# AnonymWriter/Iris-Style-Transfer

Hardware: NVIDIA B200
Metric: masked-NST image-steps/sec @640x400 VGG-19 (higher is better)
Workload: dtype bf16

## Files before the change

### include/isx.h

```cpp
#ifndef ISX_H_
#define ISX_H_

#include <stdint.h>

#ifdef __cplusplus
extern "C" {
#endif

#define ISX_VERSION 100

typedef uint16_t isx_bf16;
typedef void* isx_stream;

const char* isx_last_error(void);
int isx_version(void);
int isx_device_check(int device);

int isx_ipc_export(const void* ptr, void* handle64, int64_t* offset);
int isx_ipc_open(const void* handle64, void** base_out);
int isx_ipc_close(void* base);
int isx_copy_d2d_async(void* dst, const void* src, int64_t bytes, isx_stream stream);

typedef void* isx_handle;
int isx_create(int device, isx_handle* out);
int isx_destroy(isx_handle h);
int isx_make_current(isx_handle h);
int isx_sm_count(void);

int isx_pack_conv3x3_weights(const float* w_oihw, int Cout, int Cin, isx_bf16* w_fwd, isx_bf16* w_dgrad,
                             isx_stream stream);

int isx_conv1_1_fwd(const float* x, int xc, const float* mask, int mask_b, const float* w, const float* bias,
                    isx_bf16* out, int B, int H, int W, isx_stream stream);
int isx_pack_conv1_1_fwd(const float* w, isx_bf16* w0_fwd, isx_stream stream);
int isx_conv1_1_fwd_tc(const float* x, int xc, const float* mask, int mask_b, const isx_bf16* w0_fwd, const float* bias,
                       isx_bf16* out, int B, int H, int W, isx_stream stream);
int isx_conv1_1_dgrad(const isx_bf16* dy, const float* w, const float* mask, int mask_b, float* dx, int xc, int B,
                      int H, int W, isx_stream stream);

int isx_pack_conv1_1_dgrad(const float* w, isx_bf16* w0_dgrad, isx_stream stream);
int isx_conv1_1_dgrad_tc(const isx_bf16* dy, const isx_bf16* w0_dgrad, const float* mask, int mask_b, float* dx, int xc,
                         int B, int H, int W, isx_stream stream);

int isx_conv3x3_bias_relu_fwd(const isx_bf16* in, const isx_bf16* w_fwd, const float* bias, isx_bf16* out, int B,
                              int H, int W, int Cin, int Cout, int relu, int tile_cfg, isx_stream stream);

int isx_conv3x3_bias_relu_pool_fwd(const isx_bf16* in, const isx_bf16* w_fwd, const float* bias, isx_bf16* out,
                                   isx_bf16* pool_out, int B, int H, int W, int Cin, int Cout, int tile_cfg,
                                   isx_stream stream);
int isx_conv3x3_bias_relu_pool_idx_fwd(const isx_bf16* in, const isx_bf16* w_fwd, const float* bias, isx_bf16* out,
                                       isx_bf16* pool_out, uint8_t* pool_idx, int skip_out, int B, int H, int W, int Cin,
                                       int Cout, int tile_cfg, isx_stream stream);

int isx_conv3x3_dgrad(const isx_bf16* dy, const isx_bf16* w_dgrad, isx_bf16* dx, int B, int H, int W, int Cin,
                      int Cout, const isx_bf16* relu_act, const isx_bf16* add_grad, const float* aff_a,
                      const float* aff_b, int tile_cfg, isx_stream stream);

int isx_conv3x3_dgrad_gram(const isx_bf16* dy, const isx_bf16* w_dgrad, isx_bf16* dx, int B, int H, int W, int Cin,
                           int Cout, const isx_bf16* act_below, const isx_bf16* gram_D, isx_stream stream);

int isx_maxpool2x2_fwd(const isx_bf16* in, isx_bf16* out, int B, int H, int W, int C, isx_stream stream);
int isx_maxpool2x2_bwd(const isx_bf16* dy_pooled, const isx_bf16* act_prepool, isx_bf16* dx, int B, int H, int W,
                       int C, isx_stream stream);
int isx_maxpool2x2_fwd_idx(const isx_bf16* in, isx_bf16* out, uint8_t* idx, int B, int H, int W, int C, isx_stream stream);
int isx_maxpool2x2_bwd_idx(const isx_bf16* dy_pooled, const uint8_t* idx, isx_bf16* dx, int B, int H, int W, int C,
                           isx_stream stream);

int64_t isx_gram_workspace_bytes(int B, int HW, int C);
int isx_gram_fwd(const isx_bf16* feat, int B, int HW, int C, float inv_n, void* workspace, float* G_out,
                 const float* target, int target_b, double loss_scale, double* loss, float grad_scale,
                 isx_bf16* D_out, isx_stream stream);
int64_t isx_gram_mask_flags_bytes(int mask_b, int HW, int C);
int isx_gram_masked_fwd(const isx_bf16* feat, int B, int HW, int C, const float* m, int mask_b, void* flags_ws,
                        isx_bf16* fm2, float inv_n, void* workspace, float* G_out, const float* target, int target_b,
                        double loss_scale, double* loss, float grad_scale, isx_bf16* D_out, isx_stream stream);
int isx_gram_bwd(const isx_bf16* feat, const isx_bf16* D, isx_bf16* dF, int B, int H, int W, int C,
                 const isx_bf16* relu_act, isx_stream stream);

int isx_content_mse_fwd_bwd(const isx_bf16* pred, const isx_bf16* target, int target_b, isx_bf16* grad, int B,
                            int64_t per_image, double loss_scale, float grad_scale, double* loss, isx_stream stream);
int isx_mse_fwd_bwd(const isx_bf16* pred, const isx_bf16* target, int target_b, isx_bf16* grad, int B, int64_t per_image,
                    double loss_scale, float grad_scale, int relu_mask, double* loss, isx_stream stream);
int isx_channel_affine(const isx_bf16* feat, const float* a, const float* b, isx_bf16* out, int B, int64_t HW, int C,
                       int relu_mask, isx_stream stream);
int isx_bn_stats_fwd(const isx_bf16* feat, int B, int64_t HW, int C, double* sums, float* mean, float* std_,
                     const float* t_mean, const float* t_std, int target_b, double loss_scale, double grad_scale,
                     double* loss, float* aff_a, float* aff_b, isx_stream stream);
int isx_bn_stats_masked_fwd(const isx_bf16* feat, const float* m, int mask_b, int B, int64_t HW, int C, double* sums, float* mean,
                            float* std_, isx_stream stream);
int isx_mask_features(const isx_bf16* feat, const float* m, int mask_b, isx_bf16* fm, isx_bf16* fm2, int B, int64_t HW,
                      int C, isx_stream stream);
int isx_avgpool2x2_f32(const float* in, float* out, int B, int H, int W, isx_stream stream);
int isx_tap_add_mask(const isx_bf16* g, const isx_bf16* add, const float* aff_a, const float* aff_b,
                     const isx_bf16* act, isx_bf16* out, int B, int64_t HW, int C, isx_stream stream);

typedef struct {
  int32_t epochs;
  int32_t max_iter;
  int32_t max_eval;
  int32_t history;
  int32_t history_bf16;
  int32_t reserved_;
  double lr;
  double tolerance_grad;
  double tolerance_change;
  double c_weight, s_weight;
} isx_lbfgs_config;
int64_t isx_lbfgs_state_bytes(int P);
int64_t isx_lbfgs_mats_bytes(int P, int history);
int64_t isx_lbfgs_scratch_bytes(int P, int64_t N, int history);
int isx_lbfgs_init(void* state, int P, isx_stream stream);
int isx_lbfgs_tick(float* x, const float* grad, float* grad_prev, void* S, void* Y, void* state, void* mats,
                   void* scratch, const double* loss_c, const double* loss_s, int images_per_problem, int P,
                   int64_t N, const isx_lbfgs_config* cfg, double* hist_c, double* hist_s, int tick,
                   isx_stream stream);
int isx_lbfgs_done_flags(const void* state, int P, int32_t* done_out, isx_stream stream);
int isx_lbfgs_history_counts(const void* state, int P, int32_t* count_out, isx_stream stream);
int isx_clamp01(float* x, int64_t n, isx_stream stream);

#define ISX_MAX_TAPS 8
#define ISX_VGG19_CONVS 16
#define ISX_TAP_POOL0 16
#define ISX_VGG19_TAPS 21
typedef struct {
  int32_t B, H, W, xc;
  int32_t n_conv;
  int32_t style_mode;
  int32_t n_style;
  int32_t style_conv[ISX_MAX_TAPS];
  float style_w[ISX_MAX_TAPS];
  int32_t n_content;
  int32_t content_conv[ISX_MAX_TAPS];
  float content_w[ISX_MAX_TAPS];
  int32_t style_target_b;
  int32_t content_target_b;
  int32_t coupled;
  int32_t mask_b;
  int32_t style_mask_b;
  int32_t pred_unbatched;
  double c_weight, s_weight;
} isx_nst_config;

typedef struct {
  const float* w0;
  const isx_bf16* w0_fwd;
  const isx_bf16* w0_dgrad;
  const float* bias[ISX_VGG19_CONVS];
  const isx_bf16* w_fwd[ISX_VGG19_CONVS];
  const isx_bf16* w_dgrad[ISX_VGG19_CONVS];
  void* workspace;
  const isx_bf16* content_target[ISX_MAX_TAPS];
  const float* gram_target[ISX_MAX_TAPS];
  const float* bn_target_mean[ISX_MAX_TAPS];
  const float* bn_target_std[ISX_MAX_TAPS];
  const float* input_mask;
  const float* style_mask[ISX_MAX_TAPS];
} isx_nst_buffers;

int64_t isx_nst_workspace_bytes(const isx_nst_config* cfg);
int isx_nst_backward(const isx_nst_config* cfg, const isx_nst_buffers* bufs, const isx_bf16* const* feat_grads,
                     const isx_bf16* last_pool_grad, float* grad, isx_stream stream);
#define ISX_FWD_LAST_POOL 1
#define ISX_FWD_LEAN 2
int isx_nst_forward(const isx_nst_config* cfg, const isx_nst_buffers* bufs, const float* x, int flags,
                    isx_stream stream);
int isx_nst_feature(const isx_nst_config* cfg, const isx_nst_buffers* bufs, int kind, int idx, isx_bf16** ptr,
                    int32_t* h, int32_t* w, int32_t* c);
int isx_nst_prepare_style_masks(const isx_nst_config* cfg, const isx_nst_buffers* bufs, isx_stream stream);
int isx_nst_style_features(const isx_nst_config* cfg, const isx_nst_buffers* bufs, int want_stats, int want_gram,
                           float* out, int64_t ld, isx_stream stream);
int isx_nst_eval(const isx_nst_config* cfg, const isx_nst_buffers* bufs, const float* x, double* loss_c,
                 double* loss_s, float* grad, isx_stream stream);

int isx_mask_bbox(const float* x, const int64_t* seg, int label, int use_threshold, float threshold, uint8_t* mask,
                  float* xm, int32_t* bbox, int B, int H, int W, isx_stream stream);
int isx_mask_bbox_typed(const float* x, const void* seg, int seg_dtype, int label, int use_threshold, float threshold,
                        uint8_t* mask, float* xm, int32_t* bbox, int B, int H, int W, isx_stream stream);
int isx_resize_bilinear_aa(const float* src, int src_c, int SH, int SW, const int32_t* src_bbox, float* dst, int dst_c,
                           int DH, int DW, int B, isx_stream stream);
int isx_crop_resize_masked(const float* frames, const uint8_t* mask, const int32_t* bbox, float* dst, int dst_c, int DH,
                           int DW, int B, int H, int W, isx_stream stream);
int isx_composite(const float* new_iris, int src_c, int SH, int SW, float* frames, const uint8_t* mask,
                  const int32_t* bbox, int B, int H, int W, isx_stream stream);

int64_t isx_ritnet_transform_workspace_bytes(int B, int H, int W);
int isx_ritnet_transform(const float* x, const uint8_t* gamma_lut, const float* norm_lut, void* workspace, float* out, int B,
                         int H, int W, isx_stream stream);
int64_t isx_ritnet_param_floats(void);
int64_t isx_ritnet_workspace_bytes(int B, int H, int W);
int isx_ritnet_forward(const float* x, const float* params, const uint8_t* gamma_lut, const float* norm_lut, void* workspace,
                       int64_t* labels, float* logits, int B, int H, int W, isx_stream stream);
int isx_ritnet_forward_typed(const float* x, const float* params, const uint8_t* gamma_lut, const float* norm_lut,
                             void* workspace, void* labels, int label_dtype, float* logits, int B, int H, int W,
                             isx_stream stream);

int isx_linear_pack(const float* W, const float* bias, int N, int K, int Npad, isx_bf16* dst, isx_stream stream);
int isx_rows_pack(const float* src, int64_t ld_src, int M, int K, int Mpad, isx_bf16* dst, isx_stream stream);
int isx_pool7_flatten_pack(const isx_bf16* pool5, int B, int h, int w, int C, int Mpad, isx_bf16* dst, isx_stream stream);
int isx_linear_fwd(const isx_bf16* Xp, const isx_bf16* Wp, isx_bf16* outT, int Mpad, int Npad, int Kp, int relu, isx_stream stream);
int isx_transpose_pack(const isx_bf16* srcT, int N, int Mpad, int M, isx_bf16* dst, isx_stream stream);
int isx_transpose_out(const isx_bf16* srcT, int N, int Mpad, int M, float* dst, isx_stream stream);

int64_t isx_eye_landmarks_workspace_bytes(int B, int H, int W, int max_points);
int isx_eye_landmarks(const void* seg, int seg_dtype, int B, int H, int W, double epsilon, int max_points, void* workspace,
                      float* landmarks, int32_t* info, isx_stream stream);
int isx_gaze_head_fwd(const float* x, int64_t ld_x, int B, int in_dim, int hidden, int out_dim, const float* W1, const float* b1,
                      const float* W2, const float* b2, const float* W3, const float* b3, float* out, isx_stream stream);

int isx_pack_conv1x1_weights(const float* w, int Cout, int Cin, isx_bf16* w_out, isx_stream stream);
int isx_pack_resnet_stem_weights(const float* w, isx_bf16* w_out, isx_stream stream);
int isx_conv_bias_act_fwd(const isx_bf16* in, const isx_bf16* w, const float* bias, const isx_bf16* residual, isx_bf16* out,
                          int B, int H, int W, int Cin, int Cout, int k, int stride, int relu, isx_stream stream);
// ... 30 lines not shown
```

### iris-style-transfer_b200/csrc/api_ops.cu

```cuda
#include "../../include/isx.h"
#include "isx_common.cuh"
#include "isx_internal.h"
#include "isx_kernels.h"

using namespace isx;
typedef __nv_bfloat16 bf16;

static inline cudaStream_t S(isx_stream s) { return reinterpret_cast<cudaStream_t>(s); }
static inline const bf16* P(const isx_bf16* p) { return reinterpret_cast<const bf16*>(p); }
static inline bf16* P(isx_bf16* p) { return reinterpret_cast<bf16*>(p); }

static void decode_tile_cfg(int cfg, ConvArgs* a) {
  if (cfg > 0) {
    a->force_bn = cfg / 100;
    a->force_mt = (cfg % 100) / 10;
    a->force_stages = cfg % 10;
  }
}

extern "C" int isx_pack_conv3x3_weights(const float* w, int Cout, int Cin, isx_bf16* wf, isx_bf16* wd,
                                        isx_stream stream) {
  ISX_REQUIRE(w && (wf || wd) && Cout > 0 && Cin > 0, "isx_pack_conv3x3_weights: bad arguments");
  return pack_conv_weights(w, Cout, Cin, P(wf), P(wd), S(stream));
}

extern "C" int isx_conv1_1_fwd(const float* x, int xc, const float* mask, int mask_b, const float* w,
                               const float* bias, isx_bf16* out, int B, int H, int W, isx_stream stream) {
  ISX_REQUIRE(x && w && out && B > 0 && H > 0 && W > 0, "isx_conv1_1_fwd: bad arguments");
  ISX_REQUIRE(!mask || mask_b == 1 || mask_b == B, "isx_conv1_1_fwd: mask batch %d must be 1 or %d", mask_b, B);
  return conv1_1_fwd(x, xc, mask, mask_b, w, bias, P(out), B, H, W, S(stream));
}

extern "C" int isx_pack_conv1_1_fwd(const float* w, isx_bf16* w0_fwd, isx_stream stream) {
  ISX_REQUIRE(w && w0_fwd, "isx_pack_conv1_1_fwd: null pointer");
  return pack_w0_fwd(w, P(w0_fwd), S(stream));
}

extern "C" int isx_conv1_1_fwd_tc(const float* x, int xc, const float* mask, int mask_b, const isx_bf16* w0_fwd,
                                  const float* bias, isx_bf16* out, int B, int H, int W, isx_stream stream) {
  ISX_REQUIRE(x && w0_fwd && out && B > 0 && H > 0 && W > 0, "isx_conv1_1_fwd_tc: bad arguments");
  ISX_REQUIRE(!mask || mask_b == 1 || mask_b == B, "isx_conv1_1_fwd_tc: mask batch %d must be 1 or %d", mask_b, B);
  return conv1_1_fwd_tc(x, xc, mask, mask ? mask_b : 0, P(w0_fwd), bias, P(out), B, H, W, S(stream));
}

extern "C" int isx_pack_conv1_1_dgrad(const float* w, isx_bf16* w0_dgrad, isx_stream stream) {
  ISX_REQUIRE(w && w0_dgrad, "isx_pack_conv1_1_dgrad: null pointer");
  return pack_w0_dgrad(w, P(w0_dgrad), S(stream));
}

extern "C" int isx_conv1_1_dgrad_tc(const isx_bf16* dy, const isx_bf16* w0_dgrad, const float* mask, int mask_b,
                                    float* dx, int xc, int B, int H, int W, isx_stream stream) {
  ISX_REQUIRE(dy && w0_dgrad && dx && B > 0 && H > 0 && W > 0, "isx_conv1_1_dgrad_tc: bad arguments");
  ISX_REQUIRE(!mask || mask_b == 1 || mask_b == B, "isx_conv1_1_dgrad_tc: mask batch %d must be 1 or %d", mask_b, B);
  ConvArgs a;
  a.in = P(dy); a.weight = P(w0_dgrad); a.out = nullptr;
  a.B = B; a.H = H; a.W = W; a.Cin = 64; a.Cout = 16; a.ntaps = 9;
  a.dx_nchw = dx; a.xc = xc; a.in_mask = mask; a.mask_b = mask ? mask_b : 0;
  return conv_tc(a, S(stream));
}

extern "C" int isx_conv1_1_dgrad(const isx_bf16* dy, const float* w, const float* mask, int mask_b, float* dx, int xc,
                                 int B, int H, int W, isx_stream stream) {
  ISX_REQUIRE(dy && w && dx && B > 0 && H > 0 && W > 0, "isx_conv1_1_dgrad: bad arguments");
  ISX_REQUIRE(xc == 1 || xc == 3, "isx_conv1_1_dgrad: xc must be 1 or 3");
  return conv1_1_dgrad(P(dy), w, mask, mask_b, dx, xc, B, H, W, S(stream));
}

extern "C" int isx_conv3x3_bias_relu_fwd(const isx_bf16* in, const isx_bf16* w_fwd, const float* bias, isx_bf16* out,
                                         int B, int H, int W, int Cin, int Cout, int relu, int tile_cfg,
                                         isx_stream stream) {
  ISX_REQUIRE(in && w_fwd && out, "isx_conv3x3_bias_relu_fwd: null pointer");
  ConvArgs a;
  a.in = P(in); a.weight = P(w_fwd); a.out = P(out);
  a.B = B; a.H = H; a.W = W; a.Cin = Cin; a.Cout = Cout; a.ntaps = 9;
  a.bias = bias; a.relu = relu;
  decode_tile_cfg(tile_cfg, &a);
  return conv_tc(a, S(stream));
}

extern "C" int isx_conv3x3_bias_relu_pool_fwd(const isx_bf16* in, const isx_bf16* w_fwd, const float* bias, isx_bf16* out,
                                              isx_bf16* pool_out, int B, int H, int W, int Cin, int Cout, int tile_cfg,
                                              isx_stream stream) {
  ISX_REQUIRE(in && w_fwd && out && pool_out && H >= 2 && W >= 2, "isx_conv3x3_bias_relu_pool_fwd: bad arguments");
  ConvArgs a;
  a.in = P(in); a.weight = P(w_fwd); a.out = P(out); a.pool_out = P(pool_out);
  a.B = B; a.H = H; a.W = W; a.Cin = Cin; a.Cout = Cout; a.ntaps = 9;
  a.bias = bias; a.relu = 1;
  decode_tile_cfg(tile_cfg, &a);
  return conv_tc(a, S(stream));
}

extern "C" int isx_conv3x3_bias_relu_pool_idx_fwd(const isx_bf16* in, const isx_bf16* w_fwd, const float* bias, isx_bf16* out,
                                                  isx_bf16* pool_out, uint8_t* pool_idx, int skip_out, int B, int H, int W,
                                                  int Cin, int Cout, int tile_cfg, isx_stream stream) {
  ISX_REQUIRE(in && w_fwd && out && pool_out && pool_idx && H >= 2 && W >= 2, "isx_conv3x3_bias_relu_pool_idx_fwd: bad arguments");
  ConvArgs a;
  a.in = P(in); a.weight = P(w_fwd); a.out = P(out); a.pool_out = P(pool_out); a.pool_idx = pool_idx; a.skip_out = skip_out != 0;
  a.B = B; a.H = H; a.W = W; a.Cin = Cin; a.Cout = Cout; a.ntaps = 9;
  a.bias = bias; a.relu = 1;
  decode_tile_cfg(tile_cfg, &a);
  return conv_tc(a, S(stream));
}

extern "C" int isx_conv3x3_dgrad(const isx_bf16* dy, const isx_bf16* w_dgrad, isx_bf16* dx, int B, int H, int W,
                                 int Cin, int Cout, const isx_bf16* relu_act, const isx_bf16* add_grad,
                                 const float* aff_a, const float* aff_b, int tile_cfg, isx_stream stream) {
  ISX_REQUIRE(dy && w_dgrad && dx, "isx_conv3x3_dgrad: null pointer");
  ConvArgs a;
  a.in = P(dy); a.weight = P(w_dgrad); a.out = P(dx);
  a.B = B; a.H = H; a.W = W; a.Cin = Cout; a.Cout = Cin; a.ntaps = 9;
  a.mask_act = P(relu_act); a.add_buf = P(add_grad); a.aff_a = aff_a; a.aff_b = aff_b;
  decode_tile_cfg(tile_cfg, &a);
  return conv_tc(a, S(stream));
}

extern "C" int isx_conv3x3_dgrad_gram(const isx_bf16* dy, const isx_bf16* w_dgrad, isx_bf16* dx, int B, int H, int W,
                                      int Cin, int Cout, const isx_bf16* act_below, const isx_bf16* gram_D,
                                      isx_stream stream) {
  ISX_REQUIRE(dy && w_dgrad && dx && act_below && gram_D, "isx_conv3x3_dgrad_gram: null pointer");
  ConvArgs a;
  a.in = P(dy); a.weight = P(w_dgrad); a.out = P(dx);
  a.B = B; a.H = H; a.W = W; a.Cin = Cout; a.Cout = Cin; a.ntaps = 9;
  a.mask_act = P(act_below); a.gram_act = P(act_below); a.gram_D = P(gram_D);
  return conv_tc(a, S(stream));
}

extern "C" int isx_maxpool2x2_fwd(const isx_bf16* in, isx_bf16* out, int B, int H, int W, int C, isx_stream stream) {
  ISX_REQUIRE(in && out, "isx_maxpool2x2_fwd: null pointer");
  return maxpool_fwd(P(in), P(out), B, H, W, C, S(stream));
}

extern "C" int isx_maxpool2x2_bwd(const isx_bf16* dy, const isx_bf16* act, isx_bf16* dx, int B, int H, int W, int C,
                                  isx_stream stream) {
  ISX_REQUIRE(dy && act && dx, "isx_maxpool2x2_bwd: null pointer");
  return maxpool_bwd(P(dy), P(act), P(dx), B, H, W, C, S(stream));
}

extern "C" int isx_maxpool2x2_fwd_idx(const isx_bf16* in, isx_bf16* out, uint8_t* idx, int B, int H, int W, int C,
                                      isx_stream stream) {
  ISX_REQUIRE(in && idx, "isx_maxpool2x2_fwd_idx: null pointer");
  return maxpool_fwd_idx(P(in), P(out), idx, B, H, W, C, S(stream));
}

extern "C" int isx_maxpool2x2_bwd_idx(const isx_bf16* dy, const uint8_t* idx, isx_bf16* dx, int B, int H, int W, int C,
                                      isx_stream stream) {
  ISX_REQUIRE(dy && idx && dx, "isx_maxpool2x2_bwd_idx: null pointer");
  return maxpool_bwd_idx(P(dy), idx, P(dx), B, H, W, C, S(stream));
}

extern "C" int64_t isx_gram_workspace_bytes(int B, int HW, int C) {
  if (B <= 0 || HW <= 0 || C <= 0) return 0;
  return static_cast<int64_t>(gram_pick_splits(B, HW, C)) * B * C * C * 4;
}

extern "C" int isx_gram_fwd(const isx_bf16* feat, int B, int HW, int C, float inv_n, void* workspace, float* G_out,
                            const float* target, int target_b, double loss_scale, double* loss, float grad_scale,
                            isx_bf16* D_out, isx_stream stream) {
  ISX_REQUIRE(feat && workspace, "isx_gram_fwd: null pointer");
  ISX_REQUIRE(!target || target_b == 1 || target_b == B, "isx_gram_fwd: target batch %d must be 1 or %d", target_b, B);
  const int splits = gram_pick_splits(B, HW, C);
  int rc = gram_tc_partial(P(feat), B, HW, C, splits, static_cast<float*>(workspace), S(stream));
  if (rc) return rc;
  return gram_finalize(static_cast<const float*>(workspace), B, splits, C, inv_n, G_out, target, target_b, loss_scale,
                       loss, grad_scale, P(D_out), S(stream));
}

extern "C" int64_t isx_gram_mask_flags_bytes(int mask_b, int HW, int C) {
  if (mask_b <= 0 || HW <= 0 || C <= 0) return 0;
  return gram_mask_flags_bytes(mask_b, HW, C);
}

extern "C" int isx_gram_masked_fwd(const isx_bf16* feat, int B, int HW, int C, const float* m, int mask_b, void* flags_ws,
                                   isx_bf16* fm2, float inv_n, void* workspace, float* G_out, const float* target,
                                   int target_b, double loss_scale, double* loss, float grad_scale, isx_bf16* D_out,
                                   isx_stream stream) {
  ISX_REQUIRE(feat && m && flags_ws && workspace, "isx_gram_masked_fwd: null pointer");
  ISX_REQUIRE(mask_b == 1 || mask_b == B, "isx_gram_masked_fwd: mask batch %d must be 1 or %d", mask_b, B);
  ISX_REQUIRE(!target || target_b == 1 || target_b == B, "isx_gram_masked_fwd: target batch %d must be 1 or %d", target_b, B);
  int rc = gram_mask_flags(m, mask_b, HW, C, static_cast<uint8_t*>(flags_ws), S(stream));
  if (rc) return rc;
  ISX_REQUIRE(fm2 != nullptr, "isx_gram_masked_fwd: fm2 (bf16 [B,HW,C]) is required: the kernel stores F*m^2 while it scales the tiles");
  ISX_CHECK_CUDA(cudaMemsetAsync(fm2, 0, static_cast<size_t>(B) * HW * C * 2, S(stream)));
  GramMask gm;
  gm.m = m; gm.mask_b = mask_b; gm.kb_flags = static_cast<const uint8_t*>(flags_ws); gm.fm2 = P(fm2);
  const int splits = gram_pick_splits(B, HW, C);
  rc = gram_sym_partial(P(feat), B, HW, C, splits, static_cast<float*>(workspace), &gm, S(stream));
  if (rc) return rc;
  return gram_finalize(static_cast<const float*>(workspace), B, splits, C, inv_n, G_out, target, target_b, loss_scale,
                       loss, grad_scale, P(D_out), S(stream));
}

extern "C" int isx_gram_bwd(const isx_bf16* feat, const isx_bf16* D, isx_bf16* dF, int B, int H, int W, int C,
                            const isx_bf16* relu_act, isx_stream stream) {
  ISX_REQUIRE(feat && D && dF, "isx_gram_bwd: null pointer");
  ConvArgs a;
  a.in = P(feat); a.weight = P(D); a.out = P(dF);
  a.B = B; a.H = H; a.W = W; a.Cin = C; a.Cout = C; a.ntaps = 1;
  a.per_image_weights = true;
  a.mask_act = P(relu_act);
  return conv_tc(a, S(stream));
}

extern "C" int isx_content_mse_fwd_bwd(const isx_bf16* pred, const isx_bf16* target, int target_b, isx_bf16* grad,
                                       int B, int64_t per_image, double loss_scale, float grad_scale, double* loss,
                                       isx_stream stream) {
  ISX_REQUIRE(pred && target && loss, "isx_content_mse_fwd_bwd: null pointer");
  ISX_REQUIRE(target_b == 1 || target_b == B, "isx_content_mse_fwd_bwd: target batch %d must be 1 or %d", target_b, B);
  return content_mse(P(pred), P(target), target_b, P(grad), B, per_image, loss_scale, grad_scale, loss, S(stream));
}

extern "C" int isx_mse_fwd_bwd(const isx_bf16* pred, const isx_bf16* target, int target_b, isx_bf16* grad, int B,
                               int64_t per_image, double loss_scale, float grad_scale, int relu_mask, double* loss,
                               isx_stream stream) {
  ISX_REQUIRE(pred && target && loss, "isx_mse_fwd_bwd: null pointer");
  ISX_REQUIRE(target_b == 1 || target_b == B, "isx_mse_fwd_bwd: target batch %d must be 1 or %d", target_b, B);
  return content_mse(P(pred), P(target), target_b, P(grad), B, per_image, loss_scale, grad_scale, loss, S(stream), relu_mask);
}

extern "C" int isx_channel_affine(const isx_bf16* feat, const float* a, const float* b, isx_bf16* out, int B, int64_t HW, int C,
                                  int relu_mask, isx_stream stream) {
  ISX_REQUIRE(feat && a && b && out && C % 8 == 0, "isx_channel_affine: bad arguments");
  return tap_add_mask(nullptr, nullptr, a, b, P(feat), P(out), B, HW, C, S(stream), relu_mask);
}

extern "C" int isx_bn_stats_fwd(const isx_bf16* feat, int B, int64_t HW, int C, double* sums, float* mean, float* std_,
                                const float* t_mean, const float* t_std, int target_b, double loss_scale,
                                double grad_scale, double* loss, float* aff_a, float* aff_b, isx_stream stream) {
  ISX_REQUIRE(feat && sums, "isx_bn_stats_fwd: null pointer");
  ISX_REQUIRE(HW >= 2, "isx_bn_stats_fwd: unbiased std needs at least 2 pixels");
  ISX_CHECK_CUDA(cudaMemsetAsync(sums, 0, static_cast<size_t>(B) * C * 2 * sizeof(double), S(stream)));
  int rc = chan_sums(P(feat), B, HW, C, sums, S(stream));
  if (rc) return rc;
  return bn_finalize(sums, B, C, HW, mean, std_, t_mean, t_std, target_b, loss_scale, grad_scale, loss, aff_a, aff_b,
                     S(stream));
}

extern "C" int isx_bn_stats_masked_fwd(const isx_bf16* feat, const float* m, int mask_b, int B, int64_t HW, int C, double* sums,
                                       float* mean, float* std_, isx_stream stream) {
  ISX_REQUIRE(feat && m && sums && mean && std_, "isx_bn_stats_masked_fwd: null pointer");
  ISX_REQUIRE(mask_b == 1 || mask_b == B, "isx_bn_stats_masked_fwd: mask batch %d must be 1 or %d", mask_b, B);
  ISX_REQUIRE(HW >= 2, "isx_bn_stats_masked_fwd: unbiased std needs at least 2 pixels");
  ISX_CHECK_CUDA(cudaMemsetAsync(sums, 0, static_cast<size_t>(B) * C * 2 * sizeof(double), S(stream)));
  int rc = chan_sums(P(feat), B, HW, C, sums, S(stream), m, mask_b);
  if (rc) return rc;
  return bn_finalize(sums, B, C, HW, mean, std_, nullptr, nullptr, 1, 0.0, 0.0, nullptr, nullptr, nullptr, S(stream));
}

extern "C" int isx_mask_features(const isx_bf16* feat, const float* m, int mask_b, isx_bf16* fm, isx_bf16* fm2, int B,
                                 int64_t HW, int C, isx_stream stream) {
  ISX_REQUIRE(feat && m && fm && C % 8 == 0, "isx_mask_features: bad arguments");
  ISX_REQUIRE(mask_b == 1 || mask_b == B, "isx_mask_features: mask batch %d must be 1 or %d", mask_b, B);
  return mask_features(P(feat), m, mask_b, P(fm), P(fm2), B, HW, C, S(stream));
}

extern "C" int isx_avgpool2x2_f32(const float* in, float* out, int B, int H, int W, isx_stream stream) {
  ISX_REQUIRE(in && out && H >= 2 && W >= 2, "isx_avgpool2x2_f32: bad arguments");
  return avgpool2x2_f32(in, out, B, H, W, S(stream));
}

extern "C" int isx_tap_add_mask(const isx_bf16* g, const isx_bf16* add, const float* aff_a, const float* aff_b,
                                const isx_bf16* act, isx_bf16* out, int B, int64_t HW, int C, isx_stream stream) {
  ISX_REQUIRE(act && out, "isx_tap_add_mask: null pointer");
  return tap_add_mask(P(g), P(add), aff_a, aff_b, P(act), P(out), B, HW, C, S(stream));
}

static int IsxContext::*option_field(const char* name) {
  static const struct {
    const char* name;
    int IsxContext::*field;
  } kOptions[] = {
      {"c64", &IsxContext::opt_c64},
      {"halo2", &IsxContext::opt_halo2},
      {"tail_n", &IsxContext::opt_tail_n},
      {"sweep64", &IsxContext::opt_sweep64},
      {"smem_reserve_kb", &IsxContext::opt_smem_reserve_kb},
  };
  for (const auto& o : kOptions)
    if (strcmp(name, o.name) == 0) return o.field;
  return nullptr;
}

extern "C" int isx_set_option(const char* name, int value) {
  ISX_REQUIRE(name != nullptr, "isx_set_option: null name");
  int IsxContext::*field = option_field(name);
  ISX_REQUIRE(field != nullptr, "isx_set_option: unknown option '%s'", name);
  isx_ctx()->*field = value;
  return 0;
}

extern "C" int isx_get_option(const char* name, int* value) {
  ISX_REQUIRE(name != nullptr && value != nullptr, "isx_get_option: null pointer");
  int IsxContext::*field = option_field(name);
  ISX_REQUIRE(field != nullptr, "isx_get_option: unknown option '%s'", name);
  *value = isx_ctx()->*field;
  return 0;
}
```

### iris-style-transfer_b200/csrc/conv_c64.cu

```cuda
#include <algorithm>

#include "isx_common.cuh"
#include "isx_internal.h"
#include "isx_kernels.h"

namespace isx {

static constexpr int kC64Threads = 64 + 256;
static constexpr int kHalo = 18 * 16 * 128;
static constexpr int kTile = 128 * 128;

struct C64Params {
  int B, H, W, Cout;
  int tiles_x, tiles_y;
  long total_items;
  int halo_slots;
  int relu, fuse_pool, use_mask, use_gram;
  const float* bias;
  const __nv_bfloat16* add_buf;
  const float* aff_a;
  const float* aff_b;
  float* dx_nchw;
  int xc;
  const float* in_mask;
// ... 249 lines not shown
              const uint4 u = *reinterpret_cast<const uint4*>(mrow + chunk * 16);
              float a[8];
              float2 t;
              t = unpack_bf16x2(u.x); a[0] = t.x; a[1] = t.y;
              t = unpack_bf16x2(u.y); a[2] = t.x; a[3] = t.y;
              t = unpack_bf16x2(u.z); a[4] = t.x; a[5] = t.y;
              t = unpack_bf16x2(u.w); a[6] = t.x; a[7] = t.y;
              if (p.aff_a != nullptr && valid) {
                const float* pa = p.aff_a + static_cast<size_t>(b) * p.Cout + n + i;
                const float* pb = p.aff_b + static_cast<size_t>(b) * p.Cout + n + i;
#pragma unroll
                for (int j = 0; j < 8; ++j) f[i + j] += __ldg(pa + j) + __ldg(pb + j) * a[j];
              }
#pragma unroll
              for (int j = 0; j < 8; ++j) f[i + j] = a[j] > 0.f ? f[i + j] : 0.f;
            }
            __syncwarp();
            if (lane == 0) mbar_arrive(&act_empty[as]);
          }
          if (p.relu) {
#pragma unroll
            for (int i = 0; i < 32; ++i) f[i] = fmaxf(f[i], 0.f);
          }
          uint8_t* rowp = stg + row * 128;
#pragma unroll
          for (int c = 0; c < 4; ++c) {
            uint4 o;
            o.x = pack_bf16x2(f[c * 8 + 0], f[c * 8 + 1]);
            o.y = pack_bf16x2(f[c * 8 + 2], f[c * 8 + 3]);
            o.z = pack_bf16x2(f[c * 8 + 4], f[c * 8 + 5]);
            o.w = pack_bf16x2(f[c * 8 + 6], f[c * 8 + 7]);
            const int chunk = (h * 4 + c) ^ (row & 7);
            *reinterpret_cast<uint4*>(rowp + chunk * 16) = o;
          }
        }
        fence_proxy_async_smem();
        if (threadIdx.x == 64) tma_store_wait_read<0>();
        asm volatile("bar.sync 1, 256;" ::: "memory");
        if (threadIdx.x == 64 && !p.skip_out) {
          tma_store_4d(&tmO, stg, 0, x0, y0, b);
          tma_store_commit();
        }
        if (p.fuse_pool) {
          uint8_t* pst = smem + L.pstg + slot * 4096;
          const int item = threadIdx.x - 64;
          const int pr = item >> 3, chunk = item & 7;
          const int px = pr & 3, py = pr >> 2;
          const int r00 = (2 * py) * 8 + 2 * px;
          const int rr[4] = {r00, r00 + 1, r00 + 8, r00 + 9};
          uint4 u4[4];
#pragma unroll
          for (int k = 0; k < 4; ++k) u4[k] = *reinterpret_cast<const uint4*>(stg + rr[k] * 128 + ((chunk ^ (rr[k] & 7)) * 16));
          uint4 m4;
          uint2 codes;
          pool4_codes(u4, m4, codes);
          if (p.pool_idx != nullptr) {
            const int xp = (x0 >> 1) + px, yp = (y0 >> 1) + py;
            if (xp < (p.W >> 1) && yp < (p.H >> 1))
              *reinterpret_cast<uint2*>(p.pool_idx + ((static_cast<size_t>(b) * (p.H >> 1) + yp) * (p.W >> 1) + xp) * p.Cout +
                                        chunk * 8) = codes;
          }
          *reinterpret_cast<uint4*>(pst + pr * 128 + ((chunk ^ (pr & 7)) * 16)) = m4;
          fence_proxy_async_smem();
          asm volatile("bar.sync 1, 256;" ::: "memory");
          if (threadIdx.x == 64) {
            tma_store_4d(&tmP, pst, 0, x0 >> 1, y0 >> 1, b);
            tma_store_commit();
          }
        }
        ++gc;
      }
    }
    if (EPI == 0 && threadIdx.x == 64) tma_store_wait_all<0>();
    tc_fence_before();
  }
  __syncthreads();
  if (warp == 1) {
    tc_fence_after();
    tmem_dealloc<512>(tmem_base);
  }
}


template <int BN, int EPI>
static int launch_c64(const ConvArgs& a, cudaStream_t stream) {
  C64Params p;
  memset(&p, 0, sizeof(p));
  p.B = a.B; p.H = a.H; p.W = a.W; p.Cout = a.Cout;
  p.tiles_x = (a.W + 7) / 8;
  p.tiles_y = (a.H + 15) / 16;
  p.total_items = static_cast<long>(p.tiles_x) * p.tiles_y * a.B;
  ISX_REQUIRE(p.total_items < (1L << 31) - kNumSMs, "conv_c64: too many tiles");
  p.relu = a.relu; p.bias = a.bias; p.add_buf = a.add_buf; p.aff_a = a.aff_a; p.aff_b = a.aff_b;
  p.use_mask = (EPI == 0 && a.mask_act != nullptr) ? 1 : 0;
  p.use_gram = (EPI == 0 && a.gram_act != nullptr) ? 1 : 0;
  ISX_REQUIRE(!p.use_gram || a.gram_act == a.mask_act, "conv_c64: the fused Gram operand must be the ReLU-mask activation");
  p.fuse_pool = (EPI == 0 && a.pool_out != nullptr && a.H >= 2 && a.W >= 2) ? 1 : 0;
  p.pool_idx = p.fuse_pool ? a.pool_idx : nullptr;
  p.skip_out = (p.fuse_pool && a.pool_idx != nullptr && a.skip_out) ? 1 : 0;
  p.dx_nchw = a.dx_nchw; p.xc = a.xc; p.in_mask = a.in_mask; p.mask_b = a.mask_b;
  int hs = 4;
  C64Layout L = c64_layout<BN, EPI>(hs, p.use_mask, p.use_gram, p.fuse_pool);
  const int cap = (227 - std::max(0, std::min(isx_ctx()->opt_smem_reserve_kb, 22))) * 1024;
  while (hs > 2 && 1024 + L.total > cap) { --hs; L = c64_layout<BN, EPI>(hs, p.use_mask, p.use_gram, p.fuse_pool); }
  ISX_REQUIRE(1024 + L.total <= 227 * 1024, "conv_c64: %d B of shared memory exceed 227 KB", 1024 + L.total);
  p.halo_slots = hs;
  const size_t smem_bytes = std::max<size_t>(1024 + L.total, 204 * 1024);

  CUtensorMap tmA, tmW, tmO, tmM, tmD, tmP;
  {
    uint64_t dims[4] = {64, (uint64_t)a.W, (uint64_t)a.H, (uint64_t)a.B};
    uint64_t str[3] = {128, (uint64_t)a.W * 128, (uint64_t)a.H * a.W * 128};
    uint32_t box[4] = {64, 16, 18, 1};
    if (isx_make_tmap_bf16(&tmA, a.in, 4, dims, str, box, true)) return 3;
  }
  {
    uint64_t dims[2] = {64, (uint64_t)9 * a.Cout};
    uint64_t str[1] = {128};
    uint32_t box[2] = {64, (uint32_t)BN};
    if (isx_make_tmap_bf16(&tmW, a.weight, 2, dims, str, box, true)) return 3;
  }
  tmO = tmA; tmM = tmA; tmD = tmW; tmP = tmA;
  if (EPI == 0) {
    uint64_t dims[4] = {(uint64_t)a.Cout, (uint64_t)a.W, (uint64_t)a.H, (uint64_t)a.B};
    uint64_t str[3] = {(uint64_t)a.Cout * 2, (uint64_t)a.W * a.Cout * 2, (uint64_t)a.H * a.W * a.Cout * 2};
    uint32_t box[4] = {64, 8, 16, 1};
    if (isx_make_tmap_bf16(&tmO, a.out, 4, dims, str, box, true)) return 3;
    if (p.use_mask && isx_make_tmap_bf16(&tmM, a.mask_act, 4, dims, str, box, true)) return 3;
    if (p.use_gram) {
      uint64_t d2[2] = {(uint64_t)a.Cout, (uint64_t)a.Cout * a.B};
      uint64_t s2[1] = {(uint64_t)a.Cout * 2};
      uint32_t b2[2] = {64, (uint32_t)BN};
      if (isx_make_tmap_bf16(&tmD, a.gram_D, 2, d2, s2, b2, true)) return 3;
    }
    if (p.fuse_pool) {
      uint64_t dp[4] = {(uint64_t)a.Cout, (uint64_t)(a.W / 2), (uint64_t)(a.H / 2), (uint64_t)a.B};
      uint64_t sp[3] = {(uint64_t)a.Cout * 2, (uint64_t)(a.W / 2) * a.Cout * 2, (uint64_t)(a.H / 2) * (a.W / 2) * a.Cout * 2};
      uint32_t bp[4] = {64, 4, 8, 1};
      if (isx_make_tmap_bf16(&tmP, a.pool_out, 4, dp, sp, bp, true)) return 3;
    }
  }
  auto kern = conv_c64_kernel<BN, EPI>;
  ISX_CHECK_CUDA(cudaFuncSetAttribute(kern, cudaFuncAttributeMaxDynamicSharedMemorySize, (int)smem_bytes));
  const long grid = std::min<long>(p.total_items, kNumSMs);
  isx_prof_begin(ISX_PROF_CONV, 2.0 * (9 * 64 + (p.use_gram ? a.Cout : 0)) * a.Cout * static_cast<double>(a.B) * a.H * a.W, stream);
  kern<<<(unsigned)grid, kC64Threads, smem_bytes, stream>>>(tmA, tmW, tmO, tmM, tmD, tmP, p);
  isx_prof_end(ISX_PROF_CONV, stream);
  ISX_LAUNCH_CHECK();
  return 0;
}

bool conv_c64_applicable(const ConvArgs& a) {
  if (a.Cin != 64 || a.ntaps != 9 || a.per_image_weights || a.stride != 1) return false;
  if (a.dx_nchw != nullptr) return a.Cout == 16;
  if (a.Cout != 64) return false;
  if (a.gram_act != nullptr && a.gram_act != a.mask_act) return false;
  return true;
}

int conv_c64(const ConvArgs& a, cudaStream_t stream) {
  ISX_REQUIRE(conv_c64_applicable(a), "conv_c64: not applicable");
  if (a.dx_nchw != nullptr) return launch_c64<16, 1>(a, stream);
  return launch_c64<64, 0>(a, stream);
}

}
```

### iris-style-transfer_b200/csrc/conv_halo.cu

```cuda
#include <algorithm>

#include "isx_common.cuh"
#include "isx_internal.h"
#include "isx_kernels.h"

namespace isx {

static constexpr int kHaloThreads = 64 + 256;
static constexpr int kHaloSlot = 43 * 1024;
static constexpr int kSub = 128 * 128;

struct HaloParams {
  int B, H, W, Cin, Cout;
  int pairs_x, pairs_y, n_tiles;
  int total_items;
  int cin_blocks, extra_kb;
  int w_stages;
  int relu, fuse_pool, use_mask;
  const float* bias;
  const __nv_bfloat16* add_buf;
  const float* aff_a;
  const float* aff_b;
  uint8_t* pool_idx;
  int skip_out;
};

struct HaloLayout {
  int halo, w, act, stg, pstg, bars, total;
};
template <int BN>
__host__ __device__ inline HaloLayout halo_layout(int w_stages, int use_mask, int fuse_pool) {
  HaloLayout L;
  int off = 0;
  L.halo = off; off += 2 * kHaloSlot;
  L.w = off; off += w_stages * BN * 128;
  L.act = off; off += use_mask ? 2 * kSub : 0;
  L.stg = off; off += 2 * kSub;
  L.pstg = off; off += fuse_pool ? 2 * 4096 : 0;
  L.bars = off; off += 512;
  L.total = off;
  return L;
}

template <bool VERT>
struct ItemWalk {
  int b, r, stride, per_img, pairs_x, n_tiles;
  __device__ ItemWalk(int first, int stride_, int per_img_, int pairs_x_, int n_tiles_)
      : b(first / per_img_), r(first % per_img_), stride(stride_), per_img(per_img_), pairs_x(pairs_x_), n_tiles(n_tiles_) {}
  __device__ void next() {
    r += stride;
    while (r >= per_img) { r -= per_img; ++b; }
  }
  __device__ int nt() const { return r % n_tiles; }
  __device__ int x0() const { return ((r / n_tiles) % pairs_x) * (VERT ? 8 : 16); }
  __device__ int y0() const { return ((r / n_tiles) / pairs_x) * (VERT ? 32 : 16); }
};

template <int BN, bool VERT>
__global__ void __launch_bounds__(kHaloThreads, 1)
conv_halo_kernel(const __grid_constant__ CUtensorMap tmA, const __grid_constant__ CUtensorMap tmW,
                 const __grid_constant__ CUtensorMap tmO, const __grid_constant__ CUtensorMap tmM,
                 const __grid_constant__ CUtensorMap tmA2, const __grid_constant__ CUtensorMap tmD,
                 const __grid_constant__ CUtensorMap tmP, const HaloParams p) {
  constexpr int kPitch = VERT ? 10 : 18;
  constexpr int kPatchRows = VERT ? 34 : 18;
  constexpr int kHaloBytes = kPitch * kPatchRows * 128;
  constexpr int kMtOff = VERT ? 16 * kPitch * 128 : 8 * 128;
  constexpr int kWStage = BN * 128;
  constexpr int kNH = BN / 64;
  constexpr int kNSub = 2 * kNH;
  constexpr int kAccCols = 2 * BN;
  constexpr int kTmemCols = 2 * kAccCols;
  extern __shared__ uint8_t smem_raw[];
  uint8_t* smem = reinterpret_cast<uint8_t*>((reinterpret_cast<uintptr_t>(smem_raw) + 1023) & ~uintptr_t(1023));
  const HaloLayout L = halo_layout<BN>(p.w_stages, p.use_mask, p.fuse_pool);
  const int WS = p.w_stages;
  uint64_t* bars = reinterpret_cast<uint64_t*>(smem + L.bars);
  uint64_t* halo_full = bars;
  uint64_t* halo_empty = bars + 2;
  uint64_t* w_full = bars + 4;
  uint64_t* w_empty = bars + 12;
  uint64_t* act_full = bars + 20;
  uint64_t* tmem_full = bars + 22;
  uint64_t* tmem_empty = bars + 24;
  uint32_t* tmem_ptr_smem = reinterpret_cast<uint32_t*>(bars + 26);

  const int warp = threadIdx.x >> 5;
  const int lane = threadIdx.x & 31;

  if (warp == 0 && lane == 0) {
    tma_prefetch_desc(&tmA);
    tma_prefetch_desc(&tmW);
    tma_prefetch_desc(&tmO);
    if (p.use_mask) tma_prefetch_desc(&tmM);
    if (p.extra_kb > 0) { tma_prefetch_desc(&tmA2); tma_prefetch_desc(&tmD); }
    if (p.fuse_pool) tma_prefetch_desc(&tmP);
    for (int i = 0; i < 2; ++i) {
      mbar_init(&halo_full[i], 1);
      mbar_init(&halo_empty[i], 1);
      mbar_init(&act_full[i], 1);
      mbar_init(&tmem_full[i], 1);
      mbar_init(&tmem_empty[i], 8);
    }
    for (int i = 0; i < 8; ++i) { mbar_init(&w_full[i], 1); mbar_init(&w_empty[i], 1); }
    fence_barrier_init();
  }
  if (warp == 1) tmem_alloc<512>(tmem_ptr_smem);
  tc_fence_before();
  __syncthreads();
  tc_fence_after();
  const uint32_t tmem_base = *tmem_ptr_smem;
  const int per_img = p.pairs_x * p.pairs_y * p.n_tiles;
  const int n_my = (p.total_items - static_cast<int>(blockIdx.x) + static_cast<int>(gridDim.x) - 1) / static_cast<int>(gridDim.x);

  if (warp == 0) {
    if (lane == 0) {
      ItemWalk<VERT> it(blockIdx.x, gridDim.x, per_img, p.pairs_x, p.n_tiles);
      uint32_t hs = 0, hph = 0, ws = 0, wph = 0;
      for (int i = 0; i < n_my; ++i, it.next()) {
        const int b = it.b, x0 = it.x0(), y0 = it.y0(), n0 = it.nt() * BN;
        for (int c = 0; c < p.cin_blocks; ++c) {
          mbar_wait(&halo_empty[hs], hph ^ 1);
          mbar_arrive_expect_tx(&halo_full[hs], kHaloBytes);
          tma_load_4d(smem + L.halo + hs * kHaloSlot, &tmA, &halo_full[hs], c * 64, x0 - 1, y0 - 1, b);
          hs ^= 1;
          if (hs == 0) hph ^= 1;
          for (int tap = 0; tap < 9; ++tap) {
            mbar_wait(&w_empty[ws], wph ^ 1);
            mbar_arrive_expect_tx(&w_full[ws], kWStage);
            tma_load_2d(smem + L.w + ws * kWStage, &tmW, &w_full[ws], c * 64, tap * p.Cout + n0);
            if (++ws == static_cast<uint32_t>(WS)) { ws = 0; wph ^= 1; }
          }
        }
        for (int c2 = 0; c2 < p.extra_kb; ++c2) {
          mbar_wait(&halo_empty[hs], hph ^ 1);
          mbar_arrive_expect_tx(&halo_full[hs], 2 * kSub);
          uint8_t* slot = smem + L.halo + hs * kHaloSlot;
          tma_load_4d(slot, &tmA2, &halo_full[hs], c2 * 64, x0, y0, b);
          tma_load_4d(slot + kSub, &tmA2, &halo_full[hs], c2 * 64, VERT ? x0 : x0 + 8, VERT ? y0 + 16 : y0, b);
          hs ^= 1;
          if (hs == 0) hph ^= 1;
          mbar_wait(&w_empty[ws], wph ^ 1);
          mbar_arrive_expect_tx(&w_full[ws], kWStage);
          tma_load_2d(smem + L.w + ws * kWStage, &tmD, &w_full[ws], c2 * 64, b * p.Cout + n0);
          if (++ws == static_cast<uint32_t>(WS)) { ws = 0; wph ^= 1; }
        }
      }
    }
  } else if (warp == 1) {
    if (lane == 0) {
      constexpr uint32_t idesc = umma_idesc_bf16(128, BN, false, false);
      if (tmem_base != 0) {
        printf("isx: unexpected TMEM base %u (block %d)\n", tmem_base, blockIdx.x);
        __trap();
      }
      const uint64_t dh = umma_desc_sw128(smem_u32(smem + L.halo), 16, kPitch * 128);
      const uint64_t dp = umma_desc_sw128(smem_u32(smem + L.halo), 16, 1024);
      const uint64_t dw = umma_desc_sw128(smem_u32(smem + L.w), 16, 1024);
      const uint32_t h_lo0 = static_cast<uint32_t>(dh), h_hi = static_cast<uint32_t>(dh >> 32);
      const uint32_t p_hi = static_cast<uint32_t>(dp >> 32);
      const uint32_t w_lo0 = static_cast<uint32_t>(dw), w_hi = static_cast<uint32_t>(dw >> 32);
      uint32_t hs = 0, hph = 0, ws = 0, wph = 0, acc = 0, aph = 0, b_lo = w_lo0;
      bool w_ready = false, h_ready = false;
      auto next_stage = [&]() {
        b_lo += kWStage >> 4;
        if (++ws == static_cast<uint32_t>(WS)) { ws = 0; wph ^= 1; b_lo = w_lo0; }
      };
      for (int i = 0; i < n_my; ++i) {
        mbar_wait(&tmem_empty[acc], aph ^ 1);
        tc_fence_after();
        const uint32_t d_tm = acc * kAccCols;
        for (int c = 0; c < p.cin_blocks; ++c) {
          if (!h_ready) mbar_wait(&halo_full[hs], hph);
          h_ready = false;
          const uint32_t a_lo = h_lo0 + hs * (kHaloSlot >> 4);
#pragma unroll
          for (int tap = 0; tap < 9; ++tap) {
            const int ky = tap / 3, kx = tap - ky * 3;
            if (!w_ready) mbar_wait(&w_full[ws], wph);
            tc_fence_after();
            const uint32_t b_cur = b_lo;
            const uint32_t ws_cur = ws;
            next_stage();
            w_ready = mbar_try_wait(&w_full[ws], wph);
            if (tap == 8) h_ready = mbar_try_wait(&halo_full[hs ^ 1], hs == 1 ? hph ^ 1 : hph);
#pragma unroll
            for (int mt = 0; mt < 2; ++mt) {
#pragma unroll
              for (int k = 0; k < 4; ++k)
                umma_bf16_lohi(d_tm + mt * BN, a_lo + (((ky * kPitch + kx) * 128 + mt * kMtOff + k * 32) >> 4), h_hi,
                               b_cur + 2 * k, w_hi, idesc, (tap | k) != 0 ? 1u : (c != 0 ? 1u : 0u));
            }
            umma_commit(&w_empty[ws_cur]);
          }
          umma_commit(&halo_empty[hs]);
          hs ^= 1;
          if (hs == 0) hph ^= 1;
        }
        for (int c2 = 0; c2 < p.extra_kb; ++c2) {
          if (!h_ready) mbar_wait(&halo_full[hs], hph);
          h_ready = false;
          if (!w_ready) mbar_wait(&w_full[ws], wph);
          tc_fence_after();
          const uint32_t a_lo = h_lo0 + hs * (kHaloSlot >> 4);
          const uint32_t b_cur = b_lo;
          const uint32_t ws_cur = ws;
          next_stage();
          w_ready = mbar_try_wait(&w_full[ws], wph);
#pragma unroll
          for (int mt = 0; mt < 2; ++mt) {
#pragma unroll
            for (int k = 0; k < 4; ++k)
              umma_bf16_lohi(d_tm + mt * BN, a_lo + ((mt * kSub + k * 32) >> 4), p_hi, b_cur + 2 * k, w_hi, idesc, 1u);
          }
          umma_commit(&w_empty[ws_cur]);
          umma_commit(&halo_empty[hs]);
          hs ^= 1;
          if (hs == 0) hph ^= 1;
        }
        umma_commit(&tmem_full[acc]);
        acc ^= 1;
        if (acc == 0) aph ^= 1;
      }
    }
  } else {
    const int q = warp & 3;
    const int hsel = (warp - 2) >> 2;
    const int row = q * 32 + lane;
    const int tw = row & 7, th = row >> 3;
    const bool leader = threadIdx.x == 64;
    ItemWalk<VERT> it(blockIdx.x, gridDim.x, per_img, p.pairs_x, p.n_tiles);
    auto issue_mask_load = [&](const ItemWalk<VERT>& w, int s, uint32_t g) {
      const int mt = s / kNH, nh = s - mt * kNH;
      const uint32_t slot = g & 1;
      mbar_arrive_expect_tx(&act_full[slot], kSub);
      tma_load_4d(smem + L.act + slot * kSub, &tmM, &act_full[slot], w.nt() * BN + nh * 64,
                  w.x0() + (VERT ? 0 : 8 * mt), w.y0() + (VERT ? 16 * mt : 0), w.b);
    };
    uint32_t g = 0;
    if (p.use_mask && leader && n_my > 0) {
      issue_mask_load(it, 0, 0);
      issue_mask_load(it, 1, 1);
    }
    uint32_t acc = 0, aph = 0;
    for (int i = 0; i < n_my; ++i) {
      const int b = it.b, x0 = it.x0(), y0 = it.y0(), n0 = it.nt() * BN;
      ItemWalk<VERT> nxt = it;
      nxt.next();
      mbar_wait(&tmem_full[acc], aph);
      tc_fence_after();
#pragma unroll 1
      for (int s = 0; s < kNSub; ++s, ++g) {
        const int mt = s / kNH, nh = s - mt * kNH;
        const int xs = x0 + (VERT ? 0 : 8 * mt), ys = y0 + (VERT ? 16 * mt : 0);
        const int nc = n0 + nh * 64 + hsel * 32;
        const int x = xs + tw, y = ys + th;
        const bool valid = (x < p.W) && (y < p.H);
        const size_t pix = valid ? ((static_cast<size_t>(b) * p.H + y) * p.W + x) * p.Cout : 0;
        const uint32_t slot = g & 1;
        uint8_t* stg = smem + L.stg + slot * kSub;
        uint32_t v[32];
        tmem_ld_32x32(tmem_base + acc * kAccCols + mt * BN + nh * 64 + hsel * 32 + (static_cast<uint32_t>(q * 32) << 16), v);
        tmem_ld_wait();
        if (s == kNSub - 1) {
          tc_fence_before();
          __syncwarp();
          if (lane == 0) mbar_arrive(&tmem_empty[acc]);
        }
        float f[32];
#pragma unroll
        for (int j = 0; j < 32; ++j) f[j] = __uint_as_float(v[j]);
        if (p.bias != nullptr) {
#pragma unroll
          for (int j = 0; j < 32; j += 4) {
            const float4 bv = __ldg(reinterpret_cast<const float4*>(p.bias + nc + j));
            f[j] += bv.x; f[j + 1] += bv.y; f[j + 2] += bv.z; f[j + 3] += bv.w;
          }
        }
        if (p.add_buf != nullptr && valid) {
#pragma unroll
          for (int j = 0; j < 32; j += 8) {
            const uint4 u = __ldg(reinterpret_cast<const uint4*>(p.add_buf + pix + nc + j));
            float2 t;
            t = unpack_bf16x2(u.x); f[j] += t.x; f[j + 1] += t.y;
            t = unpack_bf16x2(u.y); f[j + 2] += t.x; f[j + 3] += t.y;
            t = unpack_bf16x2(u.z); f[j + 4] += t.x; f[j + 5] += t.y;
            t = unpack_bf16x2(u.w); f[j + 6] += t.x; f[j + 7] += t.y;
          }
        }
        if (p.use_mask) {
          mbar_wait(&act_full[slot], (g >> 1) & 1);
          const uint8_t* mrow = smem + L.act + slot * kSub + row * 128;
#pragma unroll
          for (int j = 0; j < 32; j += 8) {
            const int chunk = (hsel * 4 + (j >> 3)) ^ (row & 7);
            const uint4 u = *reinterpret_cast<const uint4*>(mrow + chunk * 16);
            float a[8];
            float2 t;
            t = unpack_bf16x2(u.x); a[0] = t.x; a[1] = t.y;
            t = unpack_bf16x2(u.y); a[2] = t.x; a[3] = t.y;
            t = unpack_bf16x2(u.z); a[4] = t.x; a[5] = t.y;
            t = unpack_bf16x2(u.w); a[6] = t.x; a[7] = t.y;
            if (p.aff_a != nullptr && valid) {
              const float* pa = p.aff_a + static_cast<size_t>(b) * p.Cout + nc + j;
              const float* pb = p.aff_b + static_cast<size_t>(b) * p.Cout + nc + j;
#pragma unroll
              for (int e = 0; e < 8; ++e) f[j + e] += __ldg(pa + e) + __ldg(pb + e) * a[e];
            }
#pragma unroll
            for (int e = 0; e < 8; ++e) f[j + e] = a[e] > 0.f ? f[j + e] : 0.f;
          }
        }
        if (p.relu) {
#pragma unroll
          for (int j = 0; j < 32; ++j) f[j] = fmaxf(f[j], 0.f);
        }
        uint8_t* rowp = stg + row * 128;
#pragma unroll
        for (int c = 0; c < 4; ++c) {
          uint4 o;
          o.x = pack_bf16x2(f[c * 8 + 0], f[c * 8 + 1]);
          o.y = pack_bf16x2(f[c * 8 + 2], f[c * 8 + 3]);
          o.z = pack_bf16x2(f[c * 8 + 4], f[c * 8 + 5]);
          o.w = pack_bf16x2(f[c * 8 + 6], f[c * 8 + 7]);
          const int chunk = (hsel * 4 + c) ^ (row & 7);
          *reinterpret_cast<uint4*>(rowp + chunk * 16) = o;
        }
        fence_proxy_async_smem();
        if (leader) tma_store_wait_read<0>();
        asm volatile("bar.sync 1, 256;" ::: "memory");
        const bool inside = xs < p.W && ys < p.H;
        if (leader) {
          if (inside && !p.skip_out) {
            tma_store_4d(&tmO, stg, n0 + nh * 64, xs, ys, b);
            tma_store_commit();
          }
          if (p.use_mask) {
            if (s + 2 < kNSub) issue_mask_load(it, s + 2, g + 2);
            else if (i + 1 < n_my) issue_mask_load(nxt, s + 2 - kNSub, g + 2);
          }
        }
        if (p.fuse_pool) {
          uint8_t* pst = smem + L.pstg + slot * 4096;
          const int item = threadIdx.x - 64;
          const int pr = item >> 3, chunk = item & 7;
          const int px = pr & 3, py = pr >> 2;
          const int r00 = (2 * py) * 8 + 2 * px;
          const int rr[4] = {r00, r00 + 1, r00 + 8, r00 + 9};
          uint4 u4[4];
#pragma unroll
          for (int k = 0; k < 4; ++k) u4[k] = *reinterpret_cast<const uint4*>(stg + rr[k] * 128 + ((chunk ^ (rr[k] & 7)) * 16));
          uint4 m4;
          uint2 codes;
          pool4_codes(u4, m4, codes);
          if (p.pool_idx != nullptr) {
            const int xp = (xs >> 1) + px, yp = (ys >> 1) + py;
            if (xp < (p.W >> 1) && yp < (p.H >> 1))
              *reinterpret_cast<uint2*>(p.pool_idx + ((static_cast<size_t>(b) * (p.H >> 1) + yp) * (p.W >> 1) + xp) * p.Cout +
                                        n0 + nh * 64 + chunk * 8) = codes;
          }
          *reinterpret_cast<uint4*>(pst + pr * 128 + ((chunk ^ (pr & 7)) * 16)) = m4;
          fence_proxy_async_smem();
          asm volatile("bar.sync 1, 256;" ::: "memory");
          if (leader && inside) {
            tma_store_4d(&tmP, pst, n0 + nh * 64, xs >> 1, ys >> 1, b);
            tma_store_commit();
          }
        }
      }
      it = nxt;
      acc ^= 1;
      if (acc == 0) aph ^= 1;
    }
    if (leader) tma_store_wait_all<0>();
    tc_fence_before();
  }
  __syncthreads();
  if (warp == 1) {
    tc_fence_after();
    tmem_dealloc<512>(tmem_base);
  }
}


template <int BN, bool VERT>
static int launch_halo(const ConvArgs& a, cudaStream_t stream) {
  HaloParams p;
  memset(&p, 0, sizeof(p));
  p.B = a.B; p.H = a.H; p.W = a.W; p.Cin = a.Cin; p.Cout = a.Cout;
  p.pairs_x = VERT ? (a.W + 7) / 8 : (a.W + 15) / 16;
  p.pairs_y = VERT ? (a.H + 31) / 32 : (a.H + 15) / 16;
  p.n_tiles = a.Cout / BN;
  const long total = static_cast<long>(p.pairs_x) * p.pairs_y * p.n_tiles * a.B;
  ISX_REQUIRE(total < (1L << 31) - kNumSMs, "conv_halo: too many work items");
  p.total_items = static_cast<int>(total);
  p.cin_blocks = a.Cin / 64;
  p.extra_kb = a.gram_act != nullptr ? a.Cout / 64 : 0;
  p.relu = a.relu; p.bias = a.bias; p.add_buf = a.add_buf; p.aff_a = a.aff_a; p.aff_b = a.aff_b;
  p.use_mask = a.mask_act != nullptr ? 1 : 0;
  p.fuse_pool = (a.pool_out != nullptr && a.H >= 2 && a.W >= 2) ? 1 : 0;
  p.pool_idx = p.fuse_pool ? a.pool_idx : nullptr;
  p.skip_out = (p.fuse_pool && a.pool_idx != nullptr && a.skip_out) ? 1 : 0;
  int ws = 6;
  HaloLayout L = halo_layout<BN>(ws, p.use_mask, p.fuse_pool);
  const int cap = (227 - std::max(0, std::min(isx_ctx()->opt_smem_reserve_kb, 22))) * 1024;
  while (ws > 2 && 1024 + L.total > cap) { --ws; L = halo_layout<BN>(ws, p.use_mask, p.fuse_pool); }
  ISX_REQUIRE(1024 + L.total <= 227 * 1024, "conv_halo: %d B of shared memory exceed 227 KB", 1024 + L.total);
  p.w_stages = ws;
  const size_t smem_bytes = std::max<size_t>(1024 + L.total, 204 * 1024);

  CUtensorMap tmA, tmW, tmO, tmM, tmA2, tmD, tmP;
  {
    uint64_t dims[4] = {(uint64_t)a.Cin, (uint64_t)a.W, (uint64_t)a.H, (uint64_t)a.B};
    uint64_t str[3] = {(uint64_t)a.Cin * 2, (uint64_t)a.W * a.Cin * 2, (uint64_t)a.H * a.W * a.Cin * 2};
    uint32_t box[4] = {64, VERT ? 10u : 18u, VERT ? 34u : 18u, 1};
    if (isx_make_tmap_bf16(&tmA, a.in, 4, dims, str, box, true)) return 3;
  }
  {
    uint64_t dims[2] = {(uint64_t)a.Cin, (uint64_t)9 * a.Cout};
    uint64_t str[1] = {(uint64_t)a.Cin * 2};
    uint32_t box[2] = {64, (uint32_t)BN};
    if (isx_make_tmap_bf16(&tmW, a.weight, 2, dims, str, box, true)) return 3;
  }
  {
    uint64_t dims[4] = {(uint64_t)a.Cout, (uint64_t)a.W, (uint64_t)a.H, (uint64_t)a.B};
    uint64_t str[3] = {(uint64_t)a.Cout * 2, (uint64_t)a.W * a.Cout * 2, (uint64_t)a.H * a.W * a.Cout * 2};
    uint32_t box[4] = {64, 8, 16, 1};
    if (isx_make_tmap_bf16(&tmO, a.out, 4, dims, str, box, true)) return 3;
    tmM = tmO; tmA2 = tmO;
    if (p.use_mask && isx_make_tmap_bf16(&tmM, a.mask_act, 4, dims, str, box, true)) return 3;
    if (p.extra_kb > 0 && isx_make_tmap_bf16(&tmA2, a.gram_act, 4, dims, str, box, true)) return 3;
  }
  tmD = tmW; tmP = tmO;
  if (p.extra_kb > 0) {
    uint64_t d2[2] = {(uint64_t)a.Cout, (uint64_t)a.Cout * a.B};
    uint64_t s2[1] = {(uint64_t)a.Cout * 2};
    uint32_t b2[2] = {64, (uint32_t)BN};
    if (isx_make_tmap_bf16(&tmD, a.gram_D, 2, d2, s2, b2, true)) return 3;
  }
  if (p.fuse_pool) {
    uint64_t dp[4] = {(uint64_t)a.Cout, (uint64_t)(a.W / 2), (uint64_t)(a.H / 2), (uint64_t)a.B};
    uint64_t sp[3] = {(uint64_t)a.Cout * 2, (uint64_t)(a.W / 2) * a.Cout * 2, (uint64_t)(a.H / 2) * (a.W / 2) * a.Cout * 2};
    uint32_t bp[4] = {64, 4, 8, 1};
    if (isx_make_tmap_bf16(&tmP, a.pool_out, 4, dp, sp, bp, true)) return 3;
  }
  auto kern = conv_halo_kernel<BN, VERT>;
  ISX_CHECK_CUDA(cudaFuncSetAttribute(kern, cudaFuncAttributeMaxDynamicSharedMemorySize, (int)smem_bytes));
  const int grid = std::min<int>(p.total_items, kNumSMs);
  isx_prof_begin(ISX_PROF_CONV, 2.0 * (9.0 * a.Cin + (p.extra_kb ? a.Cout : 0)) * a.Cout * static_cast<double>(a.B) * a.H * a.W, stream);
  kern<<<(unsigned)grid, kHaloThreads, smem_bytes, stream>>>(tmA, tmW, tmO, tmM, tmA2, tmD, tmP, p);
  isx_prof_end(ISX_PROF_CONV, stream);
  ISX_LAUNCH_CHECK();
  return 0;
}

static double pair_efficiency(int H, int W, int pw, int ph) {
  const double cw = static_cast<double>((W + pw - 1) / pw) * pw, ch = static_cast<double>((H + ph - 1) / ph) * ph;
  return (static_cast<double>(W) / cw) * (static_cast<double>(H) / ch);
}

bool conv_halo_applicable(const ConvArgs& a) {
  if (a.ntaps != 9 || a.per_image_weights || a.dx_nchw != nullptr || a.stride != 1) return false;
  if (a.Cin % 64 != 0 || a.Cout % 64 != 0) return false;
  if (a.out == nullptr) return false;
  return true;
}

int conv_halo_pick(const ConvArgs& a) {
  const double eh = pair_efficiency(a.H, a.W, 16, 16), ev = pair_efficiency(a.H, a.W, 8, 32);
  return ev > eh ? 2 : 1;
}
double conv_halo_efficiency(const ConvArgs& a) {
  return std::max(pair_efficiency(a.H, a.W, 16, 16), pair_efficiency(a.H, a.W, 8, 32));
}

int conv_halo(const ConvArgs& a, cudaStream_t stream) {
  ISX_REQUIRE(conv_halo_applicable(a), "conv_halo: not applicable");
  const bool vert = conv_halo_pick(a) == 2;
  if (a.Cout % 128 == 0) return vert ? launch_halo<128, true>(a, stream) : launch_halo<128, false>(a, stream);
  return vert ? launch_halo<64, true>(a, stream) : launch_halo<64, false>(a, stream);
}

}
```

### iris-style-transfer_b200/csrc/conv_sweep.cu

```cuda
#include <algorithm>

#include "isx_common.cuh"
#include "isx_internal.h"
#include "isx_kernels.h"

namespace isx {

static constexpr int kSwThreads = 64 + 256;
static constexpr int kSwPatch = 17 * 1024;
static constexpr int kSwPatchBytes = 130 * 128;
static constexpr int kSwTile = 128 * 128;
static constexpr int kSwWBytes = 9 * 64 * 128;
static constexpr int kSwMaxCtas = 160;

struct SweepParams {
  int B, H, W;
  int U, V;
  int u_is_y;
  int u_tiles;
  long total_cols;
  int cut_b[kSwMaxCtas + 1], cut_t[kSwMaxCtas + 1], cut_v[kSwMaxCtas + 1];
  int patch_slots;
  int relu, fuse_pool, use_mask, use_gram, skip_out;
  const float* bias;
// ... 393 lines not shown
              t = unpack_bf16x2(w4.x); a[0] = t.x; a[1] = t.y;
              t = unpack_bf16x2(w4.y); a[2] = t.x; a[3] = t.y;
              t = unpack_bf16x2(w4.z); a[4] = t.x; a[5] = t.y;
              t = unpack_bf16x2(w4.w); a[6] = t.x; a[7] = t.y;
              const float* pa = p.aff_a + static_cast<size_t>(J.b) * 64 + n + e;
              const float* pb = p.aff_b + static_cast<size_t>(J.b) * 64 + n + e;
#pragma unroll
              for (int j = 0; j < 8; ++j) f[e + j] += __ldg(pa + j) + __ldg(pb + j) * a[j];
            }
          }
          ++at;
        }
        if (p.relu) {
#pragma unroll
          for (int e = 0; e < 32; ++e) f[e] = fmaxf(f[e], 0.f);
        }
        if (regpool) {
          uint32_t w[16];
#pragma unroll
          for (int e = 0; e < 16; ++e) w[e] = pack_bf16x2(f[2 * e], f[2 * e + 1]);
          if ((vo & 1) == 0) {
#pragma unroll
            for (int e = 0; e < 16; ++e) prevw[e] = w[e];
            continue;
          }
          const bool odd = (lane & 1) != 0;
          uint32_t r0p[8], r1p[8], r0c[8], r1c[8];
#pragma unroll
          for (int i = 0; i < 8; ++i) {
            const uint32_t my_p = odd ? prevw[8 + i] : prevw[i], send_p = odd ? prevw[i] : prevw[8 + i];
            const uint32_t my_c = odd ? w[8 + i] : w[i], send_c = odd ? w[i] : w[8 + i];
            const uint32_t got_p = __shfl_xor_sync(0xffffffffu, send_p, 1);
            const uint32_t got_c = __shfl_xor_sync(0xffffffffu, send_c, 1);
            r0p[i] = odd ? got_p : my_p; r1p[i] = odd ? my_p : got_p;
            r0c[i] = odd ? got_c : my_c; r1c[i] = odd ? my_c : got_c;
          }
          uint8_t* pst = smem + L.pstg + ((static_cast<uint32_t>(vo) >> 1) & 1) * 8192;
          const int pr = row >> 1;
          const int up = (J.u0 >> 1) + pr, vp = vo >> 1;
          const int xp = p.u_is_y ? vp : up, yp = p.u_is_y ? up : vp;
          const bool pvalid = xp < (p.W >> 1) && yp < (p.H >> 1);
          uint32_t cw[4];
#pragma unroll
          for (int h2 = 0; h2 < 2; ++h2) {
            uint4 u4[4];
            u4[0] = make_uint4(r0p[4 * h2], r0p[4 * h2 + 1], r0p[4 * h2 + 2], r0p[4 * h2 + 3]);
            u4[3] = make_uint4(r1c[4 * h2], r1c[4 * h2 + 1], r1c[4 * h2 + 2], r1c[4 * h2 + 3]);
            const uint4 a = make_uint4(r0c[4 * h2], r0c[4 * h2 + 1], r0c[4 * h2 + 2], r0c[4 * h2 + 3]);
            const uint4 bq = make_uint4(r1p[4 * h2], r1p[4 * h2 + 1], r1p[4 * h2 + 2], r1p[4 * h2 + 3]);
            u4[1] = p.u_is_y ? a : bq;
            u4[2] = p.u_is_y ? bq : a;
            uint4 m4;
            uint2 codes;
            pool4_codes(u4, m4, codes);
            cw[2 * h2] = codes.x; cw[2 * h2 + 1] = codes.y;
            const int chunk = hsel * 4 + (odd ? 2 : 0) + h2;
            *reinterpret_cast<uint4*>(pst + pr * 128 + ((chunk ^ (pr & 7)) * 16)) = m4;
          }
          if (p.pool_idx != nullptr && pvalid)
            *reinterpret_cast<uint4*>(p.pool_idx + ((static_cast<size_t>(J.b) * (p.H >> 1) + yp) * (p.W >> 1) + xp) * 64 + hsel * 32 +
                                      (odd ? 16 : 0)) = make_uint4(cw[0], cw[1], cw[2], cw[3]);
          fence_proxy_async_smem();
          if (leader) tma_store_wait_read<0>();
          asm volatile("bar.sync 1, 256;" ::: "memory");
          if (leader) {
            tma_store_4d(&tmP, pst, 0, J.u0 >> 1, vo >> 1, J.b);
            tma_store_commit();
          }
          continue;
        }
        uint8_t* rowp = stg + row * 128;
#pragma unroll
        for (int c = 0; c < 4; ++c) {
          uint4 o;
          o.x = pack_bf16x2(f[c * 8 + 0], f[c * 8 + 1]) & keep[c * 4 + 0];
          o.y = pack_bf16x2(f[c * 8 + 2], f[c * 8 + 3]) & keep[c * 4 + 1];
          o.z = pack_bf16x2(f[c * 8 + 4], f[c * 8 + 5]) & keep[c * 4 + 2];
          o.w = pack_bf16x2(f[c * 8 + 6], f[c * 8 + 7]) & keep[c * 4 + 3];
          const int chunk = (hsel * 4 + c) ^ (row & 7);
          *reinterpret_cast<uint4*>(rowp + chunk * 16) = o;
        }
        fence_proxy_async_smem();
        if (leader) {
          tma_store_wait_read<0>();
          if (act_held != 0xffffffffu) { mbar_arrive(&act_empty[act_held]); act_held = 0xffffffffu; }
        }
        asm volatile("bar.sync 1, 256;" ::: "memory");
        if (leader && !p.skip_out) {
          tma_store_4d(&tmO, stg, 0, J.u0, vo, J.b);
          tma_store_commit();
        }
        if (leader && p.use_mask) act_held = as;
        if (p.fuse_pool && (vo & 1)) {
          const uint8_t* s0 = smem + L.stg;
          const uint8_t* s1 = smem + L.stg + kSwTile;
          uint8_t* pst = smem + L.pstg + ((static_cast<uint32_t>(vo) >> 1) & 1) * 8192;
#pragma unroll
          for (int rep = 0; rep < 2; ++rep) {
            const int item = static_cast<int>(threadIdx.x) - 64 + rep * 256;
            const int pr = item >> 3, chunk = item & 7;
            const int r0 = 2 * pr, r1 = 2 * pr + 1;
            const int o0 = r0 * 128 + ((chunk ^ (r0 & 7)) * 16), o1 = r1 * 128 + ((chunk ^ (r1 & 7)) * 16);
            uint4 u4[4];
            u4[0] = *reinterpret_cast<const uint4*>(s0 + o0);
            u4[3] = *reinterpret_cast<const uint4*>(s1 + o1);
            if (p.u_is_y) {
              u4[1] = *reinterpret_cast<const uint4*>(s1 + o0);
              u4[2] = *reinterpret_cast<const uint4*>(s0 + o1);
            } else {
              u4[1] = *reinterpret_cast<const uint4*>(s0 + o1);
              u4[2] = *reinterpret_cast<const uint4*>(s1 + o0);
            }
            uint4 m4;
            uint2 codes;
            pool4_codes(u4, m4, codes);
            if (p.pool_idx != nullptr) {
              const int up = (J.u0 >> 1) + pr, vp = vo >> 1;
              const int xp = p.u_is_y ? vp : up, yp = p.u_is_y ? up : vp;
              if (xp < (p.W >> 1) && yp < (p.H >> 1))
                *reinterpret_cast<uint2*>(p.pool_idx + ((static_cast<size_t>(J.b) * (p.H >> 1) + yp) * (p.W >> 1) + xp) * 64 +
                                          chunk * 8) = codes;
            }
            *reinterpret_cast<uint4*>(pst + pr * 128 + ((chunk ^ (pr & 7)) * 16)) = m4;
          }
          fence_proxy_async_smem();
          asm volatile("bar.sync 1, 256;" ::: "memory");
          if (leader) {
            tma_store_4d(&tmP, pst, 0, J.u0 >> 1, vo >> 1, J.b);
            tma_store_commit();
          }
        }
      }
    }
    if (leader) {
      tma_store_wait_all<0>();
      if (act_held != 0xffffffffu) mbar_arrive(&act_empty[act_held]);
    }
    tc_fence_before();
  }
  __syncthreads();
  if (warp == 1) {
    tc_fence_after();
    tmem_dealloc<512>(tmem_base);
  }
}

static double strip_efficiency(int n) { return static_cast<double>(n) / (((n + 127) / 128) * 128); }

bool conv_sweep_applicable(const ConvArgs& a) {
  if (a.Cin != 64 || a.Cout != 64 || a.ntaps != 9 || a.per_image_weights || a.dx_nchw != nullptr || a.stride != 1) return false;
  if (a.out == nullptr) return false;
  if (a.gram_act != nullptr && a.gram_act != a.mask_act) return false;
  if (a.aff_a != nullptr && a.mask_act == nullptr) return false;
  return true;
}
double conv_sweep_efficiency(const ConvArgs& a) { return std::max(strip_efficiency(a.H), strip_efficiency(a.W)); }

int conv_sweep(const ConvArgs& a, cudaStream_t stream) {
  ISX_REQUIRE(conv_sweep_applicable(a), "conv_sweep: not applicable");
  SweepParams p;
  memset(&p, 0, sizeof(p));
  p.B = a.B; p.H = a.H; p.W = a.W;
  p.u_is_y = strip_efficiency(a.H) > strip_efficiency(a.W) ? 1 : 0;
  p.U = p.u_is_y ? a.H : a.W;
  p.V = p.u_is_y ? a.W : a.H;
  p.u_tiles = (p.U + 127) / 128;
  p.total_cols = static_cast<long>(a.B) * p.u_tiles * p.V;
  p.relu = a.relu; p.bias = a.bias; p.add_buf = a.add_buf; p.aff_a = a.aff_a; p.aff_b = a.aff_b;
  p.use_mask = a.mask_act != nullptr ? 1 : 0;
  p.use_gram = a.gram_act != nullptr ? 1 : 0;
  p.fuse_pool = (a.pool_out != nullptr && a.H >= 2 && a.W >= 2) ? 1 : 0;
  p.pool_idx = p.fuse_pool ? a.pool_idx : nullptr;
  p.skip_out = (p.fuse_pool && a.pool_idx != nullptr && a.skip_out) ? 1 : 0;
  int ps = 6;
  SweepLayout L = sweep_layout(ps, p.use_mask, p.use_gram, p.fuse_pool);
  while (ps > 2 && 1024 + L.total > 227 * 1024) { --ps; L = sweep_layout(ps, p.use_mask, p.use_gram, p.fuse_pool); }
  ISX_REQUIRE(1024 + L.total <= 227 * 1024, "conv_sweep: %d B of shared memory exceed 227 KB", 1024 + L.total);
  p.patch_slots = ps;
  const size_t smem_bytes = std::max<size_t>(1024 + L.total, 204 * 1024);

  const uint64_t su = (p.u_is_y ? static_cast<uint64_t>(a.W) : 1ull) * 128, sv = (p.u_is_y ? 1ull : static_cast<uint64_t>(a.W)) * 128;
  const uint64_t sb = static_cast<uint64_t>(a.H) * a.W * 128;
  CUtensorMap tmA, tmW, tmO, tmM, tmD, tmP;
  {
    uint64_t dims[4] = {64, (uint64_t)p.U, (uint64_t)p.V, (uint64_t)a.B};
    uint64_t str[3] = {su, sv, sb};
    uint32_t box[4] = {64, 130, 1, 1};
    if (isx_make_tmap_bf16(&tmA, a.in, 4, dims, str, box, true)) return 3;
    uint32_t box2[4] = {64, 128, 1, 1};
    if (isx_make_tmap_bf16(&tmO, a.out, 4, dims, str, box2, true)) return 3;
    tmM = tmO;
    if (p.use_mask && isx_make_tmap_bf16(&tmM, a.mask_act, 4, dims, str, box2, true)) return 3;
  }
  {
    uint64_t dims[2] = {64, (uint64_t)9 * 64};
    uint64_t str[1] = {128};
    uint32_t box[2] = {64, 64};
    if (isx_make_tmap_bf16(&tmW, a.weight, 2, dims, str, box, true)) return 3;
  }
  tmD = tmW; tmP = tmO;
  if (p.use_gram) {
    uint64_t d2[2] = {64, (uint64_t)64 * a.B};
    uint64_t s2[1] = {128};
    uint32_t b2[2] = {64, 64};
    if (isx_make_tmap_bf16(&tmD, a.gram_D, 2, d2, s2, b2, true)) return 3;
  }
  if (p.fuse_pool) {
    const int Hp = a.H / 2, Wp = a.W / 2;
    uint64_t dp[4] = {64, (uint64_t)(p.u_is_y ? Hp : Wp), (uint64_t)(p.u_is_y ? Wp : Hp), (uint64_t)a.B};
    uint64_t sp[3] = {(p.u_is_y ? static_cast<uint64_t>(Wp) : 1ull) * 128, (p.u_is_y ? 1ull : static_cast<uint64_t>(Wp)) * 128,
                      static_cast<uint64_t>(Hp) * Wp * 128};
    uint32_t bp[4] = {64, 64, 1, 1};
    if (isx_make_tmap_bf16(&tmP, a.pool_out, 4, dp, sp, bp, true)) return 3;
  }
  ISX_CHECK_CUDA(cudaFuncSetAttribute(conv_sweep64_kernel, cudaFuncAttributeMaxDynamicSharedMemorySize, (int)smem_bytes));
  const long grid = std::max<long>(1, std::min<long>(p.total_cols / 16, std::min<long>(kNumSMs, kSwMaxCtas)));
  for (long k = 0; k <= grid; ++k) {
    long f = k >= grid ? p.total_cols : k * p.total_cols / grid;
    long sw = f / p.V;
    const long v = k >= grid ? 0 : ((f - sw * p.V) & ~1L);
    p.cut_b[k] = static_cast<int>(sw / p.u_tiles);
    p.cut_t[k] = static_cast<int>(sw % p.u_tiles);
    p.cut_v[k] = static_cast<int>(v);
  }
  isx_prof_begin(ISX_PROF_CONV, 2.0 * (9 * 64 + (p.use_gram ? 64 : 0)) * 64 * static_cast<double>(a.B) * a.H * a.W, stream);
  conv_sweep64_kernel<<<(unsigned)grid, kSwThreads, smem_bytes, stream>>>(tmA, tmW, tmO, tmM, tmD, tmP, p);
  isx_prof_end(ISX_PROF_CONV, stream);
  ISX_LAUNCH_CHECK();
  return 0;
}

}
```

### iris-style-transfer_b200/csrc/conv_tc.cu

```cuda
#include "isx_common.cuh"
#include "isx_internal.h"
#include "isx_kernels.h"

namespace isx {

struct ConvParams {
  int B, H, W, Cin, Cout;
  int ntaps;
  int stride;
  int TW, TH, TB;
  int tiles_x, tiles_y, tiles_b;
  int n_tiles;
  int w_rows_per_image;
  int extra_kb;
  int stages;
  int relu;
  const float* bias;
  const __nv_bfloat16* mask_act;
  const __nv_bfloat16* add_buf;
  const float* aff_a;
  const float* aff_b;
  int fuse_pool;
  uint8_t* pool_idx;
  int skip_out;
// ... 175 lines not shown
      tma_load_4d(scratch + (gi & 1) * kATileBytes, &tmM, &epi_bar[gi & 1], n0 + g_ * 64, x0[mt_], y0[mt_], b0[mt_]);
    };
    if (use_mask && threadIdx.x == 64) {
      issue_mask_load(0);
      if (NG > 1) issue_mask_load(1);
    }
#pragma unroll 1
    for (int mt = 0; mt < MT; ++mt) {
      const int x = x0[mt] + tw, y = y0[mt] + th, b = b0[mt] + tb;
      const bool valid = (x < p.W) && (y < p.H) && (b < p.B);
      const size_t pix = valid ? ((static_cast<size_t>(b) * p.H + y) * p.W + x) * p.Cout : 0;
#pragma unroll 1
      for (int g = 0; g < BN / 64; ++g) {
        const int gi = mt * (BN / 64) + g;
        uint8_t* stg = smem + gi * kATileBytes;
        const uint8_t* mrow = scratch + (gi & 1) * kATileBytes + row * 128;
        if (use_mask) mbar_wait(&epi_bar[gi & 1], (gi >> 1) & 1);
        {
          const int h = hsel;
          const int nloc = g * 64 + h * 32;
          uint32_t v[32];
          tmem_ld_32x32(tmem_base + (static_cast<uint32_t>(q * 32) << 16) + mt * BN + nloc, v);
          tmem_ld_wait();
          float f[32];
#pragma unroll
          for (int i = 0; i < 32; ++i) f[i] = __uint_as_float(v[i]);
          const int n = n0 + nloc;
          if (p.bias != nullptr) {
#pragma unroll
            for (int i = 0; i < 32; i += 4) {
              const float4 bv = __ldg(reinterpret_cast<const float4*>(p.bias + n + i));
              f[i] += bv.x; f[i + 1] += bv.y; f[i + 2] += bv.z; f[i + 3] += bv.w;
            }
          }
          if (p.add_buf != nullptr && valid) {
#pragma unroll
            for (int i = 0; i < 32; i += 8) {
              const uint4 u = __ldg(reinterpret_cast<const uint4*>(p.add_buf + pix + n + i));
              float2 t;
              t = unpack_bf16x2(u.x); f[i] += t.x; f[i + 1] += t.y;
              t = unpack_bf16x2(u.y); f[i + 2] += t.x; f[i + 3] += t.y;
              t = unpack_bf16x2(u.z); f[i + 4] += t.x; f[i + 5] += t.y;
              t = unpack_bf16x2(u.w); f[i + 6] += t.x; f[i + 7] += t.y;
            }
          }
          if (use_mask) {
#pragma unroll
            for (int i = 0; i < 32; i += 8) {
              const int chunk = (h * 4 + (i >> 3)) ^ (row & 7);
              const uint4 u = *reinterpret_cast<const uint4*>(mrow + chunk * 16);
              float a[8];
              float2 t;
              t = unpack_bf16x2(u.x); a[0] = t.x; a[1] = t.y;
              t = unpack_bf16x2(u.y); a[2] = t.x; a[3] = t.y;
              t = unpack_bf16x2(u.z); a[4] = t.x; a[5] = t.y;
              t = unpack_bf16x2(u.w); a[6] = t.x; a[7] = t.y;
              if (p.aff_a != nullptr && valid) {
                const float* pa = p.aff_a + static_cast<size_t>(b) * p.Cout + n + i;
                const float* pb = p.aff_b + static_cast<size_t>(b) * p.Cout + n + i;
#pragma unroll
                for (int j = 0; j < 8; ++j) f[i + j] += __ldg(pa + j) + __ldg(pb + j) * a[j];
              }
#pragma unroll
              for (int j = 0; j < 8; ++j) f[i + j] = a[j] > 0.f ? f[i + j] : 0.f;
            }
          }
          if (p.relu) {
#pragma unroll
            for (int i = 0; i < 32; ++i) f[i] = fmaxf(f[i], 0.f);
          }
          uint8_t* rowp = stg + row * 128;
#pragma unroll
          for (int c = 0; c < 4; ++c) {
            uint4 o;
            o.x = pack_bf16x2(f[c * 8 + 0], f[c * 8 + 1]);
            o.y = pack_bf16x2(f[c * 8 + 2], f[c * 8 + 3]);
            o.z = pack_bf16x2(f[c * 8 + 4], f[c * 8 + 5]);
            o.w = pack_bf16x2(f[c * 8 + 6], f[c * 8 + 7]);
            const int chunk = (h * 4 + c) ^ (row & 7);
            *reinterpret_cast<uint4*>(rowp + chunk * 16) = o;
          }
        }
        fence_proxy_async_smem();
        asm volatile("bar.sync 1, 256;" ::: "memory");
        if (threadIdx.x == 64) {
          if (!p.skip_out) {
            tma_store_4d(&tmO, stg, n0 + g * 64, x0[mt], y0[mt], b0[mt]);
            tma_store_commit();
          }
          if (use_mask && gi + 2 < NG) issue_mask_load(gi + 2);
        }
        if (p.fuse_pool) {
          uint8_t* pst = smem + (NG + (use_mask ? 2 : 0)) * kATileBytes + gi * 4096;
          const int twp = p.TW >> 1, thp = p.TH >> 1;
          const int et = threadIdx.x - 64;
          {
            const int item = et;
            const int pr = item >> 3, chunk = item & 7;
            const int px = pr % twp, py = (pr / twp) % thp, pb = pr / (twp * thp);
            const int r00 = (pb * p.TH + 2 * py) * p.TW + 2 * px;
            const int rr[4] = {r00, r00 + 1, r00 + p.TW, r00 + p.TW + 1};
            uint4 u4[4];
#pragma unroll
            for (int k = 0; k < 4; ++k) u4[k] = *reinterpret_cast<const uint4*>(stg + rr[k] * 128 + ((chunk ^ (rr[k] & 7)) * 16));
            uint4 m4;
            uint2 codes;
            pool4_codes(u4, m4, codes);
            if (p.pool_idx != nullptr) {
              const int xp = (x0[mt] >> 1) + px, yp = (y0[mt] >> 1) + py, bp = b0[mt] + pb;
              if (xp < (p.W >> 1) && yp < (p.H >> 1) && bp < p.B)
                *reinterpret_cast<uint2*>(p.pool_idx + ((static_cast<size_t>(bp) * (p.H >> 1) + yp) * (p.W >> 1) + xp) * p.Cout +
                                          n0 + g * 64 + chunk * 8) = codes;
            }
            *reinterpret_cast<uint4*>(pst + pr * 128 + ((chunk ^ (pr & 7)) * 16)) = m4;
          }
          fence_proxy_async_smem();
          asm volatile("bar.sync 1, 256;" ::: "memory");
          if (threadIdx.x == 64) {
            tma_store_4d(&tmP, pst, n0 + g * 64, x0[mt] >> 1, y0[mt] >> 1, b0[mt]);
            tma_store_commit();
          }
        }
      }
    }
    }
    if (EPI == 0 && threadIdx.x == 64) tma_store_wait_all<0>();
    tc_fence_before();
  }
  __syncthreads();
  if (warp == 1) {
    tc_fence_after();
    tmem_dealloc<kTmemCols>(tmem_base);
  }
}

static void choose_patch(int B, int H, int W, bool one_image_per_tile, int* TW, int* TH, int* TB) {
  long best = -1;
  for (int tw = 128; tw >= 1; tw >>= 1) {
    for (int th = 128 / tw; th >= 1; th >>= 1) {
      int tb = 128 / (tw * th);
      if (one_image_per_tile && tb != 1) continue;
      if (tw > 256 || th > 256 || tb > 256) continue;
      long padded = static_cast<long>((W + tw - 1) / tw * tw) * ((H + th - 1) / th * th) * ((B + tb - 1) / tb * tb);
      if (best < 0 || padded < best) {
        best = padded;
        *TW = tw; *TH = th; *TB = tb;
      }
    }
  }
}

template <int BN, int MT, int EPI = 0>
static int launch_conv(const ConvArgs& a, int stages_override, cudaStream_t stream) {
  ConvParams p;
  memset(&p, 0, sizeof(p));
  const int Ho = (a.H + a.stride - 1) / a.stride, Wo = (a.W + a.stride - 1) / a.stride;
  p.B = a.B; p.H = Ho; p.W = Wo; p.Cin = a.Cin; p.Cout = a.Cout; p.ntaps = a.ntaps; p.stride = a.stride;
  const bool per_image = a.per_image_weights || a.gram_act != nullptr;
  choose_patch(a.B, Ho, Wo, per_image, &p.TW, &p.TH, &p.TB);
  p.tiles_x = (Wo + p.TW - 1) / p.TW;
  p.tiles_y = (Ho + p.TH - 1) / p.TH;
  p.tiles_b = (a.B + p.TB - 1) / p.TB;
  p.n_tiles = a.Cout / BN;
  p.w_rows_per_image = a.per_image_weights ? a.Cout : 0;
  p.relu = a.relu; p.bias = a.bias; p.mask_act = a.mask_act; p.add_buf = a.add_buf;
  p.aff_a = a.aff_a; p.aff_b = a.aff_b;
  p.dx_nchw = a.dx_nchw; p.xc = a.xc; p.in_mask = a.in_mask; p.mask_b = a.mask_b;
  p.extra_kb = a.gram_act != nullptr ? a.Cout / 64 : 0;
  if (per_image && MT != 1)
    ISX_REQUIRE(p.TB == 1 && (p.tiles_x * p.tiles_y) % MT == 0, "per-image weights: an odd tile count per image needs MT = 1");

  constexpr int kStageBytes = MT * kATileBytes + BN * 128;
  const bool fuse_pool = EPI == 0 && a.pool_out != nullptr && p.TW % 2 == 0 && p.TH % 2 == 0 &&
                         a.H >= 2 && a.W >= 2;
  p.fuse_pool = fuse_pool ? 1 : 0;
  p.pool_idx = fuse_pool ? a.pool_idx : nullptr;
  p.skip_out = (fuse_pool && a.pool_idx != nullptr && a.skip_out) ? 1 : 0;
  const int epi_bytes = (MT * (BN / 64) + (a.mask_act ? 2 : 0)) * kATileBytes + (fuse_pool ? MT * (BN / 64) * 4096 : 0);
  int stages;
  size_t ring_bytes;
  stages = stages_override > 0 ? stages_override : (200 * 1024) / kStageBytes;
  if (stages > 8) stages = 8;
  if (stages < 2) stages = 2;
  while (stages * kStageBytes < epi_bytes) ++stages;
  ring_bytes = static_cast<size_t>(stages) * kStageBytes;
  p.stages = stages;
  const size_t smem_bytes = 1024 + ring_bytes + 256;
  ISX_REQUIRE(smem_bytes <= 227 * 1024, "conv_tc: %zu B of shared memory exceed 227 KB", smem_bytes);

  CUtensorMap tmA, tmB, tmO, tmM, tmA2, tmB2, tmP;
  {
    uint64_t dims[4] = {(uint64_t)a.Cin, (uint64_t)a.W, (uint64_t)a.H, (uint64_t)a.B};
    uint64_t str[3] = {(uint64_t)a.Cin * 2, (uint64_t)a.W * a.Cin * 2, (uint64_t)a.H * a.W * a.Cin * 2};
    uint32_t box[4] = {64, (uint32_t)(p.TW * a.stride), (uint32_t)(p.TH * a.stride), (uint32_t)p.TB};
    const uint32_t es[4] = {1, (uint32_t)a.stride, (uint32_t)a.stride, 1};
    if (isx_make_tmap_bf16(&tmA, a.in, 4, dims, str, box, true, es)) return 3;
  }
  {
    uint64_t rows = (uint64_t)a.ntaps * a.Cout * (a.per_image_weights ? a.B : 1);
    uint64_t dims[2] = {(uint64_t)a.Cin, rows};
    uint64_t str[1] = {(uint64_t)a.Cin * 2};
    uint32_t box[2] = {64, (uint32_t)BN};
    if (isx_make_tmap_bf16(&tmB, a.weight, 2, dims, str, box, true)) return 3;
  }
  if (EPI == 0) {
    uint64_t dims[4] = {(uint64_t)a.Cout, (uint64_t)Wo, (uint64_t)Ho, (uint64_t)a.B};
    uint64_t str[3] = {(uint64_t)a.Cout * 2, (uint64_t)Wo * a.Cout * 2, (uint64_t)Ho * Wo * a.Cout * 2};
    uint32_t box[4] = {64, (uint32_t)p.TW, (uint32_t)p.TH, (uint32_t)p.TB};
    if (isx_make_tmap_bf16(&tmO, a.out, 4, dims, str, box, true)) return 3;
  } else {
    tmO = tmA;
  }
  tmM = tmO; tmA2 = tmA; tmB2 = tmB; tmP = tmO;
  if (fuse_pool) {
    uint64_t dims[4] = {(uint64_t)a.Cout, (uint64_t)(a.W / 2), (uint64_t)(a.H / 2), (uint64_t)a.B};
    uint64_t str[3] = {(uint64_t)a.Cout * 2, (uint64_t)(a.W / 2) * a.Cout * 2, (uint64_t)(a.H / 2) * (a.W / 2) * a.Cout * 2};
    uint32_t box[4] = {64, (uint32_t)(p.TW / 2), (uint32_t)(p.TH / 2), (uint32_t)p.TB};
    if (isx_make_tmap_bf16(&tmP, a.pool_out, 4, dims, str, box, true)) return 3;
  }
  if (EPI == 0 && a.mask_act != nullptr) {
    uint64_t dims[4] = {(uint64_t)a.Cout, (uint64_t)a.W, (uint64_t)a.H, (uint64_t)a.B};
    uint64_t str[3] = {(uint64_t)a.Cout * 2, (uint64_t)a.W * a.Cout * 2, (uint64_t)a.H * a.W * a.Cout * 2};
    uint32_t box[4] = {64, (uint32_t)p.TW, (uint32_t)p.TH, (uint32_t)p.TB};
    if (isx_make_tmap_bf16(&tmM, a.mask_act, 4, dims, str, box, true)) return 3;
  }
  if (a.gram_act != nullptr) {
    uint64_t dims[4] = {(uint64_t)a.Cout, (uint64_t)a.W, (uint64_t)a.H, (uint64_t)a.B};
    uint64_t str[3] = {(uint64_t)a.Cout * 2, (uint64_t)a.W * a.Cout * 2, (uint64_t)a.H * a.W * a.Cout * 2};
    uint32_t box[4] = {64, (uint32_t)p.TW, (uint32_t)p.TH, (uint32_t)p.TB};
    if (isx_make_tmap_bf16(&tmA2, a.gram_act, 4, dims, str, box, true)) return 3;
    uint64_t dims2[2] = {(uint64_t)a.Cout, (uint64_t)a.Cout * a.B};
    uint64_t str2[1] = {(uint64_t)a.Cout * 2};
    uint32_t box2[2] = {64, (uint32_t)BN};
    if (isx_make_tmap_bf16(&tmB2, a.gram_D, 2, dims2, str2, box2, true)) return 3;
  }
  const long sp_tiles = static_cast<long>(p.tiles_x) * p.tiles_y * p.tiles_b;
  long grid = ((sp_tiles + MT - 1) / MT) * p.n_tiles;
  auto kern = conv_tc_kernel<BN, MT, EPI>;
  ISX_CHECK_CUDA(cudaFuncSetAttribute(kern, cudaFuncAttributeMaxDynamicSharedMemorySize, (int)smem_bytes));
  isx_prof_begin(ISX_PROF_CONV,
                 2.0 * (a.ntaps * a.Cin + (a.gram_act ? a.Cout : 0)) * a.Cout * static_cast<double>(a.B) * Ho * Wo, stream);
  kern<<<(unsigned)grid, kConvThreads, smem_bytes, stream>>>(tmA, tmB, tmO, tmM, tmA2, tmB2, tmP, p);
  isx_prof_end(ISX_PROF_CONV, stream);
  ISX_LAUNCH_CHECK();
  if (a.pool_out != nullptr && !fuse_pool) {
    if (a.pool_idx != nullptr) return maxpool_fwd_idx(a.out, a.pool_out, a.pool_idx, a.B, a.H, a.W, a.Cout, stream);
    return maxpool_fwd(a.out, a.pool_out, a.B, a.H, a.W, a.Cout, stream);
  }
  return 0;
}

int conv_tc(const ConvArgs& a_in, cudaStream_t stream) {
  ConvArgs a = a_in;
  ISX_REQUIRE(a.stride == 1 || (a.stride == 2 && a.pool_out == nullptr && a.mask_act == nullptr && a.gram_act == nullptr &&
                                a.dx_nchw == nullptr && !a.per_image_weights),
              "conv_tc: stride %d (stride 2 is the plain forward conv: no pool, mask, image gradient or per-image weights)",
              a.stride);
  if (a.dx_nchw != nullptr && isx_ctx()->opt_tail_n > 0 && isx_ctx()->opt_c64 < 2 && a.force_bn == 0 &&
      a.Cin == 64 && a.Cout == 16 && a.ntaps == 9)
    return conv1_1_tail_n(a.in, a.weight, a.in_mask, a.mask_b, a.dx_nchw, a.xc, a.B, a.H, a.W, stream);
  if (isx_ctx()->opt_sweep64 > 0 && a.force_bn == 0 && !a.generic_only && conv_sweep_applicable(a)) {
    const long strips = static_cast<long>(a.B) * ((std::max(a.H, a.W) + 127) / 128) * std::min(a.H, a.W);
    if (isx_ctx()->opt_sweep64 >= 2 ||
        (conv_sweep_efficiency(a) >= 0.85 && strips >= 64L * kNumSMs && std::min(a.H, a.W) >= 16))
      return conv_sweep(a, stream);
  }
  if (isx_ctx()->opt_c64 > 0 && a.force_bn == 0 && !a.generic_only && conv_c64_applicable(a) &&
      (isx_ctx()->opt_c64 >= 2 || (a.dx_nchw == nullptr && static_cast<long>(a.B) * ((a.H + 15) / 16) * ((a.W + 7) / 8) >= kNumSMs)))
    return conv_c64(a, stream);
  if (isx_ctx()->opt_halo2 > 0 && a.force_bn == 0 && !a.generic_only && conv_halo_applicable(a)) {
    const long items = static_cast<long>(a.B) * ((a.H + 15) / 16) * ((a.W + 15) / 16) * (a.Cout / (a.Cout % 128 == 0 ? 128 : 64));
    if (isx_ctx()->opt_halo2 >= 2 || (items >= 2 * kNumSMs && conv_halo_efficiency(a) >= 0.85)) return conv_halo(a, stream);
  }
  if (a.dx_nchw != nullptr) {
    ISX_REQUIRE(a.Cin == 64 && a.Cout == 16 && a.ntaps == 9, "conv_tc: image-gradient mode needs Cin 64, Cout 16 (padded)");
    ISX_REQUIRE(a.xc == 1 || a.xc == 3, "conv_tc: xc must be 1 or 3");
    const long pix_tiles = (static_cast<long>(a.B) * a.H * a.W + 127) / 128;
    if (a.force_mt == 1 || pix_tiles < 4 * kNumSMs) return launch_conv<16, 1, 1>(a, a.force_stages ? a.force_stages : 3, stream);
    return launch_conv<16, 2, 1>(a, a.force_stages ? a.force_stages : 2, stream);
  }
  ISX_REQUIRE(a.Cin % 64 == 0 && a.Cout % 64 == 0, "conv_tc: Cin=%d / Cout=%d must be multiples of 64", a.Cin, a.Cout);
  ISX_REQUIRE(a.ntaps == 9 || a.ntaps == 1, "conv_tc: ntaps must be 9 or 1");
  ISX_REQUIRE(a.B > 0 && a.H > 0 && a.W > 0, "conv_tc: empty input");
  ISX_REQUIRE((a.aff_a == nullptr) || (a.mask_act != nullptr), "conv_tc: affine tap gradient needs the activation");
  ISX_REQUIRE((a.gram_act == nullptr) || (a.gram_D != nullptr && !a.per_image_weights), "conv_tc: bad fused-Gram arguments");
  int bn = a.force_bn, mt = a.force_mt;
  int st = a.force_stages;
  if (bn == 0) {
    bn = a.Cout % 256 == 0 ? 256 : (a.Cout % 128 == 0 ? 128 : 64);
    mt = (bn == 256 || a.per_image_weights) ? 1 : 2;
    if (st == 0) st = 2;
    const long pix_tiles = (static_cast<long>(a.B) * ((a.H + a.stride - 1) / a.stride) * ((a.W + a.stride - 1) / a.stride) + 127) / 128;
    auto ctas = [&](int BN_, int MT_) { return ((pix_tiles + MT_ - 1) / MT_) * (a.Cout / BN_); };
    if (ctas(bn, mt) < 2 * kNumSMs && mt == 2) mt = 1;
    if (ctas(bn, mt) < 2 * kNumSMs && bn == 256) bn = 128;
    if (a.gram_act != nullptr && mt == 2) {
      int tw, th, tb;
      choose_patch(a.B, a.H, a.W, true, &tw, &th, &tb);
      if ((((a.W + tw - 1) / tw) * ((a.H + th - 1) / th)) % 2 != 0) mt = 1;
    }
  }
  if (mt == 0) mt = 1;
#define ISX_CONV_CASE(BN_, MT_) \
  if (bn == BN_ && mt == MT_) return launch_conv<BN_, MT_>(a, st, stream);
  ISX_CONV_CASE(64, 1) ISX_CONV_CASE(64, 2) ISX_CONV_CASE(128, 1) ISX_CONV_CASE(128, 2)
  ISX_CONV_CASE(256, 1) ISX_CONV_CASE(256, 2)
#undef ISX_CONV_CASE
  ISX_REQUIRE(false, "conv_tc: unsupported tile BN=%d MT=%d", bn, mt);
}

}
```

### iris-style-transfer_b200/csrc/elementwise.cu

```cuda
#include <algorithm>

#include "isx_common.cuh"
#include "isx_internal.h"
#include "isx_kernels.h"

namespace isx {

__constant__ float c_mean[3] = {0.485f, 0.456f, 0.406f};
__constant__ float c_std[3] = {0.229f, 0.224f, 0.225f};

__global__ void pack_w_kernel(const float* __restrict__ w, int Cout, int Cin, __nv_bfloat16* __restrict__ wf,
                              __nv_bfloat16* __restrict__ wd) {
  const long n = static_cast<long>(Cout) * Cin * 9;
  for (long i = blockIdx.x * static_cast<long>(blockDim.x) + threadIdx.x; i < n;
       i += static_cast<long>(gridDim.x) * blockDim.x) {
    const int tap = i % 9;
    const int ci = (i / 9) % Cin;
    const int co = i / (9L * Cin);
    const __nv_bfloat16 v = __float2bfloat16_rn(w[i]);
    if (wf) wf[(static_cast<long>(tap) * Cout + co) * Cin + ci] = v;
    if (wd) wd[(static_cast<long>(8 - tap) * Cin + ci) * Cout + co] = v;
  }
}

// ... 133 lines not shown
  } else {
    dx[static_cast<long>(b) * hw + off] = a0 + a1 + a2;
  }
}

int conv1_1_dgrad(const __nv_bfloat16* dy, const float* w, const float* mask, int mask_b, float* dx, int xc, int B,
                  int H, int W, cudaStream_t s) {
  const long npix = static_cast<long>(B) * H * W;
  conv1_1_dgrad_kernel<<<static_cast<unsigned>((npix + 127) / 128), 128, 0, s>>>(dy, w, mask, mask_b, dx, xc, B, H, W);
  ISX_LAUNCH_CHECK();
  return 0;
}

__device__ __forceinline__ void unpack8(const uint4& u, float (&f)[8]) {
  float2 t;
  t = unpack_bf16x2(u.x); f[0] = t.x; f[1] = t.y;
  t = unpack_bf16x2(u.y); f[2] = t.x; f[3] = t.y;
  t = unpack_bf16x2(u.z); f[4] = t.x; f[5] = t.y;
  t = unpack_bf16x2(u.w); f[6] = t.x; f[7] = t.y;
}
__device__ __forceinline__ uint4 pack8(const float (&f)[8]) {
  uint4 o;
  o.x = pack_bf16x2(f[0], f[1]); o.y = pack_bf16x2(f[2], f[3]);
  o.z = pack_bf16x2(f[4], f[5]); o.w = pack_bf16x2(f[6], f[7]);
  return o;
}

__global__ void maxpool_fwd_kernel(const __nv_bfloat16* __restrict__ in, __nv_bfloat16* __restrict__ out, int B, int H,
                                   int W, int C) {
  const int Ho = H / 2, Wo = W / 2, C8 = C / 8;
  const long n = static_cast<long>(B) * Ho * Wo * C8;
  for (long i = blockIdx.x * static_cast<long>(blockDim.x) + threadIdx.x; i < n;
       i += static_cast<long>(gridDim.x) * blockDim.x) {
    const int c8 = i % C8;
    const int xo = (i / C8) % Wo;
    const int yo = (i / (static_cast<long>(C8) * Wo)) % Ho;
    const int b = i / (static_cast<long>(C8) * Wo * Ho);
    const __nv_bfloat16* p = in + ((static_cast<long>(b) * H + 2 * yo) * W + 2 * xo) * C + c8 * 8;
    float a[8], t[8];
    unpack8(__ldg(reinterpret_cast<const uint4*>(p)), a);
    unpack8(__ldg(reinterpret_cast<const uint4*>(p + C)), t);
#pragma unroll
    for (int j = 0; j < 8; ++j) a[j] = t[j] > a[j] ? t[j] : a[j];
    unpack8(__ldg(reinterpret_cast<const uint4*>(p + static_cast<long>(W) * C)), t);
#pragma unroll
    for (int j = 0; j < 8; ++j) a[j] = t[j] > a[j] ? t[j] : a[j];
    unpack8(__ldg(reinterpret_cast<const uint4*>(p + static_cast<long>(W) * C + C)), t);
#pragma unroll
    for (int j = 0; j < 8; ++j) a[j] = t[j] > a[j] ? t[j] : a[j];
    *reinterpret_cast<uint4*>(out + ((static_cast<long>(b) * Ho + yo) * Wo + xo) * C + c8 * 8) = pack8(a);
  }
}

int maxpool_fwd(const __nv_bfloat16* in, __nv_bfloat16* out, int B, int H, int W, int C, cudaStream_t s) {
  ISX_REQUIRE(C % 8 == 0 && H >= 2 && W >= 2, "maxpool: bad shape H=%d W=%d C=%d", H, W, C);
  const long n = static_cast<long>(B) * (H / 2) * (W / 2) * (C / 8);
  const int blocks = static_cast<int>(std::min<long>((n + 255) / 256, static_cast<long>(isx_num_sms()) * 16));
  maxpool_fwd_kernel<<<blocks, 256, 0, s>>>(in, out, B, H, W, C);
  ISX_LAUNCH_CHECK();
  return 0;
}

__global__ void maxpool_bwd_kernel(const __nv_bfloat16* __restrict__ dy, const __nv_bfloat16* __restrict__ act,
                                   __nv_bfloat16* __restrict__ dx, int B, int H, int W, int C) {
  const int Ho = H / 2, Wo = W / 2, C8 = C / 8;
  const long n = static_cast<long>(B) * Ho * Wo * C8;
  for (long i = blockIdx.x * static_cast<long>(blockDim.x) + threadIdx.x; i < n;
       i += static_cast<long>(gridDim.x) * blockDim.x) {
    const int c8 = i % C8;
    const int xo = (i / C8) % Wo;
    const int yo = (i / (static_cast<long>(C8) * Wo)) % Ho;
    const int b = i / (static_cast<long>(C8) * Wo * Ho);
    const long base = ((static_cast<long>(b) * H + 2 * yo) * W + 2 * xo) * C + c8 * 8;
    const long offs[4] = {0, C, static_cast<long>(W) * C, static_cast<long>(W) * C + C};
    float a[4][8], g[8];
#pragma unroll
    for (int k = 0; k < 4; ++k) unpack8(__ldg(reinterpret_cast<const uint4*>(act + base + offs[k])), a[k]);
    unpack8(__ldg(reinterpret_cast<const uint4*>(dy + ((static_cast<long>(b) * Ho + yo) * Wo + xo) * C + c8 * 8)), g);
    float o[4][8];
#pragma unroll
    for (int j = 0; j < 8; ++j) {
      int arg = 0;
      float m = a[0][j];
#pragma unroll
      for (int k = 1; k < 4; ++k)
        if (a[k][j] > m) { m = a[k][j]; arg = k; }
#pragma unroll
      for (int k = 0; k < 4; ++k) o[k][j] = (k == arg && m > 0.f) ? g[j] : 0.f;
    }
#pragma unroll
    for (int k = 0; k < 4; ++k) *reinterpret_cast<uint4*>(dx + base + offs[k]) = pack8(o[k]);
  }
}

int maxpool_bwd(const __nv_bfloat16* dy, const __nv_bfloat16* act, __nv_bfloat16* dx, int B, int H, int W, int C,
                cudaStream_t s) {
  ISX_REQUIRE(C % 8 == 0 && H >= 2 && W >= 2, "maxpool_bwd: bad shape H=%d W=%d C=%d", H, W, C);
  if ((H & 1) || (W & 1))
    ISX_CHECK_CUDA(cudaMemsetAsync(dx, 0, static_cast<size_t>(B) * H * W * C * 2, s));
  const long n = static_cast<long>(B) * (H / 2) * (W / 2) * (C / 8);
  const int blocks = static_cast<int>(std::min<long>((n + 255) / 256, static_cast<long>(isx_num_sms()) * 16));
  maxpool_bwd_kernel<<<blocks, 256, 0, s>>>(dy, act, dx, B, H, W, C);
  ISX_LAUNCH_CHECK();
  return 0;
}

__global__ void maxpool_fwd_idx_kernel(const __nv_bfloat16* __restrict__ in, __nv_bfloat16* __restrict__ out,
                                       uint8_t* __restrict__ idx, int B, int H, int W, int C) {
  const int Ho = H / 2, Wo = W / 2, C8 = C / 8;
  const long n = static_cast<long>(B) * Ho * Wo * C8;
  for (long i = blockIdx.x * static_cast<long>(blockDim.x) + threadIdx.x; i < n;
       i += static_cast<long>(gridDim.x) * blockDim.x) {
    const int c8 = i % C8;
    const int xo = (i / C8) % Wo;
    const int yo = (i / (static_cast<long>(C8) * Wo)) % Ho;
    const int b = i / (static_cast<long>(C8) * Wo * Ho);
    const __nv_bfloat16* p = in + ((static_cast<long>(b) * H + 2 * yo) * W + 2 * xo) * C + c8 * 8;
    uint4 u[4];
    u[0] = __ldg(reinterpret_cast<const uint4*>(p));
    u[1] = __ldg(reinterpret_cast<const uint4*>(p + C));
    u[2] = __ldg(reinterpret_cast<const uint4*>(p + static_cast<long>(W) * C));
    u[3] = __ldg(reinterpret_cast<const uint4*>(p + static_cast<long>(W) * C + C));
    uint4 m4;
    uint2 codes;
    pool4_codes(u, m4, codes);
    const long o = ((static_cast<long>(b) * Ho + yo) * Wo + xo) * C + c8 * 8;
    if (out != nullptr) *reinterpret_cast<uint4*>(out + o) = m4;
    *reinterpret_cast<uint2*>(idx + o) = codes;
  }
}

int maxpool_fwd_idx(const __nv_bfloat16* in, __nv_bfloat16* out, uint8_t* idx, int B, int H, int W, int C, cudaStream_t s) {
  ISX_REQUIRE(C % 8 == 0 && H >= 2 && W >= 2, "maxpool: bad shape H=%d W=%d C=%d", H, W, C);
  const long n = static_cast<long>(B) * (H / 2) * (W / 2) * (C / 8);
  const int blocks = static_cast<int>(std::min<long>((n + 255) / 256, static_cast<long>(isx_num_sms()) * 16));
  maxpool_fwd_idx_kernel<<<blocks, 256, 0, s>>>(in, out, idx, B, H, W, C);
  ISX_LAUNCH_CHECK();
  return 0;
}

__global__ void maxpool_bwd_idx_kernel(const __nv_bfloat16* __restrict__ dy, const uint8_t* __restrict__ idx,
                                       __nv_bfloat16* __restrict__ dx, int B, int H, int W, int C) {
  const int Ho = H / 2, Wo = W / 2, C8 = C / 8;
  const long n = static_cast<long>(B) * Ho * Wo * C8;
  for (long i = blockIdx.x * static_cast<long>(blockDim.x) + threadIdx.x; i < n;
       i += static_cast<long>(gridDim.x) * blockDim.x) {
    const int c8 = i % C8;
    const int xo = (i / C8) % Wo;
    const int yo = (i / (static_cast<long>(C8) * Wo)) % Ho;
    const int b = i / (static_cast<long>(C8) * Wo * Ho);
    const long po = ((static_cast<long>(b) * Ho + yo) * Wo + xo) * C + c8 * 8;
    const uint4 g = __ldg(reinterpret_cast<const uint4*>(dy + po));
    const uint2 cd = __ldg(reinterpret_cast<const uint2*>(idx + po));
    const uint32_t gw[4] = {g.x, g.y, g.z, g.w};
    const uint32_t c16[4] = {__byte_perm(cd.x, 0u, 0x4140), __byte_perm(cd.x, 0u, 0x4342), __byte_perm(cd.y, 0u, 0x4140),
                             __byte_perm(cd.y, 0u, 0x4342)};
    const long base = ((static_cast<long>(b) * H + 2 * yo) * W + 2 * xo) * C + c8 * 8;
    const long offs[4] = {0, C, static_cast<long>(W) * C, static_cast<long>(W) * C + C};
#pragma unroll
    for (int k = 0; k < 4; ++k) {
      uint32_t o[4];
#pragma unroll
      for (int e = 0; e < 4; ++e) {
        const uint32_t d = c16[e] ^ (static_cast<uint32_t>(k) * 0x00010001u);
        const uint32_t keep = ((d & 0x0000FFFFu) ? 0u : 0x0000FFFFu) | ((d & 0xFFFF0000u) ? 0u : 0xFFFF0000u);
        o[e] = gw[e] & keep;
      }
      *reinterpret_cast<uint4*>(dx + base + offs[k]) = make_uint4(o[0], o[1], o[2], o[3]);
    }
  }
}

int maxpool_bwd_idx(const __nv_bfloat16* dy, const uint8_t* idx, __nv_bfloat16* dx, int B, int H, int W, int C,
                    cudaStream_t s) {
  ISX_REQUIRE(C % 8 == 0 && H >= 2 && W >= 2, "maxpool_bwd: bad shape H=%d W=%d C=%d", H, W, C);
  if ((H & 1) || (W & 1))
    ISX_CHECK_CUDA(cudaMemsetAsync(dx, 0, static_cast<size_t>(B) * H * W * C * 2, s));
  const long n = static_cast<long>(B) * (H / 2) * (W / 2) * (C / 8);
  const int blocks = static_cast<int>(std::min<long>((n + 255) / 256, static_cast<long>(isx_num_sms()) * 16));
  maxpool_bwd_idx_kernel<<<blocks, 256, 0, s>>>(dy, idx, dx, B, H, W, C);
  ISX_LAUNCH_CHECK();
  return 0;
}

__global__ void mask_features_kernel(const __nv_bfloat16* __restrict__ f, const float* __restrict__ m, int mask_b,
                                     __nv_bfloat16* __restrict__ fm, __nv_bfloat16* __restrict__ fm2, long HW, int C8,
                                     long n8) {
  for (long i = blockIdx.x * static_cast<long>(blockDim.x) + threadIdx.x; i < n8;
       i += static_cast<long>(gridDim.x) * blockDim.x) {
    const long pix = i / C8;
    const long b = pix / HW, pp = pix - b * HW;
    const float mv = __ldg(m + (mask_b > 1 ? b : 0) * HW + pp);
    float a[8], o1[8], o2[8];
    unpack8(__ldg(reinterpret_cast<const uint4*>(f) + i), a);
#pragma unroll
    for (int j = 0; j < 8; ++j) { o1[j] = a[j] * mv; o2[j] = o1[j] * mv; }
    reinterpret_cast<uint4*>(fm)[i] = pack8(o1);
    if (fm2) reinterpret_cast<uint4*>(fm2)[i] = pack8(o2);
  }
}

int mask_features(const __nv_bfloat16* f, const float* m, int mask_b, __nv_bfloat16* fm, __nv_bfloat16* fm2, int B,
                  long HW, int C, cudaStream_t s) {
  const long n8 = static_cast<long>(B) * HW * C / 8;
  const int blocks = static_cast<int>(std::min<long>((n8 + 255) / 256, static_cast<long>(isx_num_sms()) * 16));
  mask_features_kernel<<<blocks, 256, 0, s>>>(f, m, mask_b, fm, fm2, HW, C / 8, n8);
  ISX_LAUNCH_CHECK();
  return 0;
}

__global__ void avgpool2x2_f32_kernel(const float* __restrict__ in, float* __restrict__ out, int B, int H, int W) {
  const int Ho = H / 2, Wo = W / 2;
  const long n = static_cast<long>(B) * Ho * Wo;
  for (long i = blockIdx.x * static_cast<long>(blockDim.x) + threadIdx.x; i < n;
       i += static_cast<long>(gridDim.x) * blockDim.x) {
    const int xo = i % Wo;
    const int yo = (i / Wo) % Ho;
    const long b = i / (static_cast<long>(Wo) * Ho);
    const float* p = in + (b * H + 2 * yo) * W + 2 * xo;
    out[i] = (p[0] + p[1] + p[W] + p[W + 1]) * 0.25f;
  }
}

int avgpool2x2_f32(const float* in, float* out, int B, int H, int W, cudaStream_t s) {
  const long n = static_cast<long>(B) * (H / 2) * (W / 2);
  const int blocks = static_cast<int>(std::min<long>((n + 255) / 256, static_cast<long>(isx_num_sms()) * 8));
  avgpool2x2_f32_kernel<<<blocks, 256, 0, s>>>(in, out, B, H, W);
  ISX_LAUNCH_CHECK();
  return 0;
}

__global__ void tap_add_mask_kernel(const __nv_bfloat16* __restrict__ g, const __nv_bfloat16* __restrict__ add,
                                    const float* __restrict__ aff_a, const float* __restrict__ aff_b,
                                    const __nv_bfloat16* __restrict__ act, __nv_bfloat16* __restrict__ out, long n8,
                                    int C, long per_image8, int relu_mask) {
  for (long i = blockIdx.x * static_cast<long>(blockDim.x) + threadIdx.x; i < n8;
       i += static_cast<long>(gridDim.x) * blockDim.x) {
    float a[8], v[8], t[8];
    unpack8(__ldg(reinterpret_cast<const uint4*>(act) + i), a);
    if (g) unpack8(__ldg(reinterpret_cast<const uint4*>(g) + i), v);
    else {
#pragma unroll
      for (int j = 0; j < 8; ++j) v[j] = 0.f;
    }
    if (add) {
      unpack8(__ldg(reinterpret_cast<const uint4*>(add) + i), t);
#pragma unroll
      for (int j = 0; j < 8; ++j) v[j] += t[j];
    }
    if (aff_a) {
      const int c = (i * 8) % C;
      const long b = i / per_image8;
#pragma unroll
      for (int j = 0; j < 8; ++j) v[j] += aff_a[b * C + c + j] + aff_b[b * C + c + j] * a[j];
    }
#pragma unroll
    for (int j = 0; j < 8; ++j) v[j] = (!relu_mask || a[j] > 0.f) ? v[j] : 0.f;
    reinterpret_cast<uint4*>(out)[i] = pack8(v);
  }
}

__global__ void masked_affine_grad_kernel(const __nv_bfloat16* __restrict__ f, const float* __restrict__ m, int mask_b,
                                          const float* __restrict__ aff_a, const float* __restrict__ aff_b,
                                          __nv_bfloat16* __restrict__ out, long HW, int C, long n8) {
  const int C8 = C / 8;
  for (long i = blockIdx.x * static_cast<long>(blockDim.x) + threadIdx.x; i < n8; i += static_cast<long>(gridDim.x) * blockDim.x) {
    const long pix = i / C8;
    const long b = pix / HW, pp = pix - b * HW;
    const int c = static_cast<int>(i % C8) * 8;
    const float mv = __ldg(m + (mask_b > 1 ? b : 0) * HW + pp);
    float a[8], o[8];
    unpack8(__ldg(reinterpret_cast<const uint4*>(f) + i), a);
#pragma unroll
    for (int j = 0; j < 8; ++j) o[j] = mv * (aff_a[b * C + c + j] + aff_b[b * C + c + j] * (mv * a[j]));
    reinterpret_cast<uint4*>(out)[i] = pack8(o);
  }
}

int masked_affine_grad(const __nv_bfloat16* f, const float* m, int mask_b, const float* aff_a, const float* aff_b,
                       __nv_bfloat16* out, int B, long HW, int C, cudaStream_t s) {
  const long n8 = static_cast<long>(B) * HW * C / 8;
  const int blocks = static_cast<int>(std::min<long>((n8 + 255) / 256, static_cast<long>(isx_num_sms()) * 16));
  masked_affine_grad_kernel<<<blocks, 256, 0, s>>>(f, m, mask_b, aff_a, aff_b, out, HW, C, n8);
  ISX_LAUNCH_CHECK();
  return 0;
}

int tap_add_mask(const __nv_bfloat16* g, const __nv_bfloat16* add, const float* aff_a, const float* aff_b,
                 const __nv_bfloat16* act, __nv_bfloat16* out, int B, long HW, int C, cudaStream_t s, int relu_mask) {
  const long n8 = static_cast<long>(B) * HW * C / 8;
  const int blocks = static_cast<int>(std::min<long>((n8 + 255) / 256, static_cast<long>(isx_num_sms()) * 16));
  tap_add_mask_kernel<<<blocks, 256, 0, s>>>(g, add, aff_a, aff_b, act, out, n8, C, HW * C / 8, relu_mask);
  ISX_LAUNCH_CHECK();
  return 0;
}

__global__ void __launch_bounds__(256)
gram_finalize_kernel(const float* __restrict__ partial, int splits, int C, float inv_n, float* __restrict__ G_out,
                     const float* __restrict__ target, int target_b, double loss_scale, double* __restrict__ loss,
                     float grad_scale, __nv_bfloat16* __restrict__ D_out, float* __restrict__ triu, long triu_ld) {
  __shared__ float sg[32][33];
  __shared__ double red[8];
  const int b = blockIdx.y;
  const int nt = C >> 5;
  int tr = 0, rem = blockIdx.x;
  while (rem >= nt - tr) { rem -= nt - tr; ++tr; }
  const int tc = tr + rem;
  const int tx = threadIdx.x & 31, ty = threadIdx.x >> 5;
  const long cc = static_cast<long>(C) * C;
  const float* pb = partial + static_cast<long>(b) * splits * cc;
  const float* tb = target ? target + (target_b > 1 ? b : 0) * cc : nullptr;
  float d2 = 0.f;
  float g[4];
#pragma unroll
  for (int k = 0; k < 4; ++k) {
    const int r = tr * 32 + ty + 8 * k, c = tc * 32 + tx;
    const long o = static_cast<long>(r) * C + c;
    float acc = __ldg(pb + o);
    for (int s = 1; s < splits; ++s) acc += __ldg(pb + s * cc + o);
    g[k] = acc * inv_n;
    sg[ty + 8 * k][tx] = g[k];
    if (G_out) G_out[b * cc + o] = g[k];
// ... 216 lines not shown
```

### iris-style-transfer_b200/csrc/isx_common.cuh

```cuda
#pragma once
#include <cuda.h>
#include <cuda_bf16.h>
#include <cuda_runtime.h>
#include <stdint.h>
#include <stdio.h>
#include <string.h>

void isx_set_error(const char* fmt, ...);

#define ISX_CHECK_CUDA(expr)                                                              \
  do {                                                                                    \
    cudaError_t _e = (expr);                                                              \
    if (_e != cudaSuccess) {                                                              \
      isx_set_error("%s:%d: %s -> %s", __FILE__, __LINE__, #expr, cudaGetErrorString(_e)); \
      return 1;                                                                           \
    }                                                                                     \
  } while (0)

#define ISX_REQUIRE(cond, ...)   \
  do {                           \
    if (!(cond)) {               \
      isx_set_error(__VA_ARGS__); \
      return 2;                  \
    }                            \
  } while (0)

struct IsxProfiler;
struct IsxContext {
  int device = 0;
  int num_sms = 148;
  int opt_c64 = 1;
  int opt_halo2 = 1;
  int opt_tail_n = 1;
  int opt_smem_reserve_kb = 0;
  int opt_sweep64 = 1;
  unsigned long long launches = 0;
  IsxProfiler* prof = nullptr;
};
IsxContext* isx_ctx();
inline int isx_num_sms() { return isx_ctx()->num_sms; }

#define ISX_LAUNCH_CHECK()               \
  do {                                   \
    ++isx_ctx()->launches;               \
    ISX_CHECK_CUDA(cudaGetLastError());  \
  } while (0)

void isx_prof_begin(int family, double work, cudaStream_t s);
void isx_prof_end(int family, cudaStream_t s);
enum { ISX_PROF_CONV = 0, ISX_PROF_GRAM = 1, ISX_PROF_LBFGS = 2, ISX_PROF_PLANES = 3, ISX_PROF_FAMILIES = 4 };

int isx_make_tmap_bf16(CUtensorMap* out, const void* base, int rank, const uint64_t* dims,
                       const uint64_t* strides_bytes, const uint32_t* box, bool swizzle128,
                       const uint32_t* elem_strides = nullptr);

#ifdef __CUDACC__
namespace isx {

#define kNumSMs (isx_num_sms())

__device__ __forceinline__ uint32_t smem_u32(const void* p) {
  return static_cast<uint32_t>(__cvta_generic_to_shared(p));
}
__device__ __forceinline__ uint32_t lane_id() { return threadIdx.x & 31; }

__device__ __forceinline__ bool elect_one() {
  uint32_t pred = 0;
  asm volatile(
      "{\n\t.reg .pred P;\n\t.reg .b32 R;\n\t"
      "elect.sync R|P, 0xffffffff;\n\t"
      "selp.u32 %0, 1, 0, P;\n\t}"
      : "=r"(pred));
  return pred != 0;
}

__device__ __forceinline__ void mbar_init(uint64_t* bar, uint32_t count) {
  asm volatile("mbarrier.init.shared::cta.b64 [%0], %1;" ::"r"(smem_u32(bar)), "r"(count));
}
__device__ __forceinline__ void fence_barrier_init() {
  asm volatile("fence.mbarrier_init.release.cluster;" ::: "memory");
}
__device__ __forceinline__ void fence_proxy_async_smem() {
  asm volatile("fence.proxy.async.shared::cta;" ::: "memory");
}
__device__ __forceinline__ void mbar_arrive_expect_tx(uint64_t* bar, uint32_t bytes) {
  asm volatile("mbarrier.arrive.expect_tx.shared::cta.b64 _, [%0], %1;" ::"r"(smem_u32(bar)), "r"(bytes)
               : "memory");
}
__device__ __forceinline__ void mbar_arrive(uint64_t* bar) {
  asm volatile("mbarrier.arrive.shared::cta.b64 _, [%0];" ::"r"(smem_u32(bar)) : "memory");
}
__device__ __forceinline__ bool mbar_try_wait(uint64_t* bar, uint32_t parity) {
  uint32_t ok;
  asm volatile(
      "{\n\t.reg .pred P;\n\t"
      "mbarrier.try_wait.parity.shared::cta.b64 P, [%1], %2;\n\t"
      "selp.u32 %0, 1, 0, P;\n\t}"
      : "=r"(ok)
      : "r"(smem_u32(bar)), "r"(parity)
      : "memory");
  return ok != 0;
}
__device__ __forceinline__ void mbar_wait(uint64_t* bar, uint32_t parity) {
  uint32_t spins = 0;
  while (!mbar_try_wait(bar, parity)) {
    if (++spins > (1u << 26)) {
      printf("isx: mbarrier wait timed out (block %d,%d thread %d)\n", blockIdx.x, blockIdx.y, threadIdx.x);
      __trap();
    }
  }
}

__device__ __forceinline__ void mbar_wait2(uint64_t* bar_a, uint32_t parity_a, uint64_t* bar_b, uint32_t parity_b) {
  bool a = mbar_try_wait(bar_a, parity_a);
  bool b = mbar_try_wait(bar_b, parity_b);
  if (!a) mbar_wait(bar_a, parity_a);
  if (!b) mbar_wait(bar_b, parity_b);
}

__device__ __forceinline__ void tma_prefetch_desc(const CUtensorMap* m) {
  asm volatile("prefetch.tensormap [%0];" ::"l"(reinterpret_cast<uint64_t>(m)) : "memory");
}
__device__ __forceinline__ void tma_load_2d(void* smem, const CUtensorMap* m, uint64_t* bar, int c0, int c1) {
  asm volatile(
      "cp.async.bulk.tensor.2d.shared::cluster.global.mbarrier::complete_tx::bytes [%0], [%1, {%3, %4}], [%2];"
      ::"r"(smem_u32(smem)), "l"(reinterpret_cast<uint64_t>(m)), "r"(smem_u32(bar)), "r"(c0), "r"(c1)
      : "memory");
}
__device__ __forceinline__ void tma_load_3d(void* smem, const CUtensorMap* m, uint64_t* bar, int c0, int c1, int c2) {
  asm volatile(
      "cp.async.bulk.tensor.3d.shared::cluster.global.mbarrier::complete_tx::bytes [%0], [%1, {%3, %4, %5}], [%2];"
      ::"r"(smem_u32(smem)), "l"(reinterpret_cast<uint64_t>(m)), "r"(smem_u32(bar)), "r"(c0), "r"(c1), "r"(c2)
      : "memory");
}
__device__ __forceinline__ void tma_load_4d(void* smem, const CUtensorMap* m, uint64_t* bar, int c0, int c1, int c2,
                                            int c3) {
  asm volatile(
      "cp.async.bulk.tensor.4d.shared::cluster.global.mbarrier::complete_tx::bytes [%0], [%1, {%3, %4, %5, %6}], [%2];"
      ::"r"(smem_u32(smem)), "l"(reinterpret_cast<uint64_t>(m)), "r"(smem_u32(bar)), "r"(c0), "r"(c1), "r"(c2),
      "r"(c3)
      : "memory");
}
__device__ __forceinline__ void tma_store_4d(const CUtensorMap* m, const void* smem, int c0, int c1, int c2, int c3) {
  asm volatile("cp.async.bulk.tensor.4d.global.shared::cta.bulk_group [%0, {%2, %3, %4, %5}], [%1];" ::"l"(
                   reinterpret_cast<uint64_t>(m)),
               "r"(smem_u32(smem)), "r"(c0), "r"(c1), "r"(c2), "r"(c3)
               : "memory");
}
__device__ __forceinline__ void tma_store_commit() { asm volatile("cp.async.bulk.commit_group;" ::: "memory"); }
template <int N>
__device__ __forceinline__ void tma_store_wait_read() {
  asm volatile("cp.async.bulk.wait_group.read %0;" ::"n"(N) : "memory");
}
template <int N>
__device__ __forceinline__ void tma_store_wait_all() {
  asm volatile("cp.async.bulk.wait_group %0;" ::"n"(N) : "memory");
}

template <int kCols>
__device__ __forceinline__ void tmem_alloc(uint32_t* dst_smem) {
  asm volatile("tcgen05.alloc.cta_group::1.sync.aligned.shared::cta.b32 [%0], %1;" ::"r"(smem_u32(dst_smem)),
               "n"(kCols)
               : "memory");
  asm volatile("tcgen05.relinquish_alloc_permit.cta_group::1.sync.aligned;" ::: "memory");
}
template <int kCols>
__device__ __forceinline__ void tmem_dealloc(uint32_t taddr) {
  asm volatile("tcgen05.dealloc.cta_group::1.sync.aligned.b32 %0, %1;" ::"r"(taddr), "n"(kCols) : "memory");
}
__device__ __forceinline__ void tc_fence_before() { asm volatile("tcgen05.fence::before_thread_sync;" ::: "memory"); }
__device__ __forceinline__ void tc_fence_after() { asm volatile("tcgen05.fence::after_thread_sync;" ::: "memory"); }

__device__ __forceinline__ void umma_bf16(uint32_t tmem_d, uint64_t desc_a, uint64_t desc_b, uint32_t idesc,
                                          uint32_t accumulate) {
  asm volatile(
      "{\n\t.reg .pred p;\n\t"
      "setp.ne.b32 p, %4, 0;\n\t"
      "tcgen05.mma.cta_group::1.kind::f16 [%0], %1, %2, %3, p;\n\t}"
      ::"r"(tmem_d), "l"(desc_a), "l"(desc_b), "r"(idesc), "r"(accumulate)
      : "memory");
}
__device__ __forceinline__ void umma_bf16_lohi(uint32_t tmem_d, uint32_t a_lo, uint32_t a_hi, uint32_t b_lo, uint32_t b_hi,
                                               uint32_t idesc, uint32_t accumulate) {
  asm volatile(
      "{\n\t.reg .pred p;\n\t.reg .b64 da, db;\n\t"
      "mov.b64 da, {%1, %2};\n\tmov.b64 db, {%3, %4};\n\t"
      "setp.ne.b32 p, %6, 0;\n\t"
      "tcgen05.mma.cta_group::1.kind::f16 [%0], da, db, %5, p;\n\t}"
      ::"r"(tmem_d), "r"(a_lo), "r"(a_hi), "r"(b_lo), "r"(b_hi), "r"(idesc), "r"(accumulate)
      : "memory");
}
__device__ __forceinline__ void umma_commit(uint64_t* bar) {
  asm volatile("tcgen05.commit.cta_group::1.mbarrier::arrive::one.shared::cluster.b64 [%0];" ::"r"(smem_u32(bar))
               : "memory");
}
__device__ __forceinline__ void tmem_ld_32x32(uint32_t taddr, uint32_t (&v)[32]) {
  asm volatile(
      "tcgen05.ld.sync.aligned.32x32b.x32.b32 "
      "{%0, %1, %2, %3, %4, %5, %6, %7, %8, %9, %10, %11, %12, %13, %14, %15, "
      "%16, %17, %18, %19, %20, %21, %22, %23, %24, %25, %26, %27, %28, %29, %30, %31}, [%32];"
      : "=r"(v[0]), "=r"(v[1]), "=r"(v[2]), "=r"(v[3]), "=r"(v[4]), "=r"(v[5]), "=r"(v[6]), "=r"(v[7]), "=r"(v[8]),
        "=r"(v[9]), "=r"(v[10]), "=r"(v[11]), "=r"(v[12]), "=r"(v[13]), "=r"(v[14]), "=r"(v[15]), "=r"(v[16]),
        "=r"(v[17]), "=r"(v[18]), "=r"(v[19]), "=r"(v[20]), "=r"(v[21]), "=r"(v[22]), "=r"(v[23]), "=r"(v[24]),
        "=r"(v[25]), "=r"(v[26]), "=r"(v[27]), "=r"(v[28]), "=r"(v[29]), "=r"(v[30]), "=r"(v[31])
      : "r"(taddr)
      : "memory");
}
__device__ __forceinline__ void tmem_ld_32x16(uint32_t taddr, uint32_t (&v)[16]) {
  asm volatile(
      "tcgen05.ld.sync.aligned.32x32b.x16.b32 "
      "{%0, %1, %2, %3, %4, %5, %6, %7, %8, %9, %10, %11, %12, %13, %14, %15}, [%16];"
      : "=r"(v[0]), "=r"(v[1]), "=r"(v[2]), "=r"(v[3]), "=r"(v[4]), "=r"(v[5]), "=r"(v[6]), "=r"(v[7]), "=r"(v[8]),
        "=r"(v[9]), "=r"(v[10]), "=r"(v[11]), "=r"(v[12]), "=r"(v[13]), "=r"(v[14]), "=r"(v[15])
      : "r"(taddr)
      : "memory");
}
__device__ __forceinline__ void tmem_ld_wait() { asm volatile("tcgen05.wait::ld.sync.aligned;" ::: "memory"); }

__device__ __forceinline__ uint64_t umma_desc_sw128(uint32_t smem_addr, uint32_t lbo_bytes, uint32_t sbo_bytes,
                                                   uint32_t base_offset = 0) {
  uint64_t d = 0;
  d |= static_cast<uint64_t>(base_offset & 7) << 49;
  d |= static_cast<uint64_t>((smem_addr & 0x3FFFF) >> 4);
  d |= static_cast<uint64_t>((lbo_bytes >> 4) & 0x3FFF) << 16;
  d |= static_cast<uint64_t>((sbo_bytes >> 4) & 0x3FFF) << 32;
  d |= 1ull << 46;
  d |= 2ull << 61;
  return d;
}
__host__ __device__ constexpr uint32_t umma_idesc_bf16(int M, int N, bool a_mn_major, bool b_mn_major) {
  return (1u << 4)
         | (1u << 7)
         | (1u << 10)
         | ((a_mn_major ? 1u : 0u) << 15)
         | ((b_mn_major ? 1u : 0u) << 16)
         | (static_cast<uint32_t>(N >> 3) << 17)
         | (static_cast<uint32_t>(M >> 4) << 24);
}

__device__ __forceinline__ uint32_t pack_bf16x2(float a, float b) {
  __nv_bfloat162 h = __floats2bfloat162_rn(a, b);
  return *reinterpret_cast<uint32_t*>(&h);
}
__device__ __forceinline__ float2 unpack_bf16x2(uint32_t u) {
  __nv_bfloat162 h = *reinterpret_cast<__nv_bfloat162*>(&u);
  return __bfloat1622float2(h);
}
__device__ __forceinline__ void pool4_codes(const uint4 (&u)[4], uint4& m4, uint2& codes) {
  uint32_t cw[4];
  const __nv_bfloat162 zero2 = __floats2bfloat162_rn(0.f, 0.f);
#pragma unroll
  for (int e = 0; e < 4; ++e) {
    __nv_bfloat162 m = reinterpret_cast<const __nv_bfloat162*>(&u[0])[e];
    uint32_t code = 0u;
#pragma unroll
    for (int k = 1; k < 4; ++k) {
      const __nv_bfloat162 a = reinterpret_cast<const __nv_bfloat162*>(&u[k])[e];
      const uint32_t gt = __hgt2_mask(a, m);
      m = __hmax2(m, a);
      code = (code & ~gt) | (gt & (static_cast<uint32_t>(k) * 0x00010001u));
    }
    const uint32_t z = __hle2_mask(m, zero2);
    cw[e] = (code & ~z) | (z & 0x00040004u);
    reinterpret_cast<__nv_bfloat162*>(&m4)[e] = m;
  }
  codes.x = __byte_perm(cw[0], cw[1], 0x6420);
  codes.y = __byte_perm(cw[2], cw[3], 0x6420);
}

__device__ __forceinline__ float warp_sum(float v) {
#pragma unroll
  for (int o = 16; o > 0; o >>= 1) v += __shfl_xor_sync(0xffffffffu, v, o);
  return v;
}
__device__ __forceinline__ double warp_sum(double v) {
#pragma unroll
  for (int o = 16; o > 0; o >>= 1) v += __shfl_xor_sync(0xffffffffu, v, o);
  return v;
}
__device__ __forceinline__ float warp_max(float v) {
#pragma unroll
  for (int o = 16; o > 0; o >>= 1) v = fmaxf(v, __shfl_xor_sync(0xffffffffu, v, o));
  return v;
}

}
#endif
```

### iris-style-transfer_b200/csrc/isx_internal.h

```cpp
#pragma once
#include <cuda_bf16.h>
#include <cuda_runtime.h>
#include <stdint.h>

namespace isx {

struct ConvArgs {
  const __nv_bfloat16* in = nullptr;
  const __nv_bfloat16* weight = nullptr;
  __nv_bfloat16* out = nullptr;
  int B = 0, H = 0, W = 0, Cin = 0, Cout = 0, ntaps = 9;
  int stride = 1;
  bool per_image_weights = false;
  const float* bias = nullptr;
  int relu = 0;
  __nv_bfloat16* pool_out = nullptr;
  uint8_t* pool_idx = nullptr;
  bool skip_out = false;
  const __nv_bfloat16* mask_act = nullptr;
  const __nv_bfloat16* add_buf = nullptr;
  const float* aff_a = nullptr;
  const float* aff_b = nullptr;
  int force_bn = 0, force_mt = 0, force_stages = 0;
  bool generic_only = false;
  const __nv_bfloat16* gram_act = nullptr;
  const __nv_bfloat16* gram_D = nullptr;
  float* dx_nchw = nullptr;
  int xc = 3;
  const float* in_mask = nullptr;
  int mask_b = 0;
};
int conv_tc(const ConvArgs& a, cudaStream_t stream);
bool conv_c64_applicable(const ConvArgs& a);
int conv_c64(const ConvArgs& a, cudaStream_t stream);
bool conv_sweep_applicable(const ConvArgs& a);
double conv_sweep_efficiency(const ConvArgs& a);
int conv_sweep(const ConvArgs& a, cudaStream_t stream);
int conv1_1_tail_n(const __nv_bfloat16* dy, const __nv_bfloat16* wd, const float* mask, int mask_b, float* dx, int xc,
                   int B, int H, int W, cudaStream_t stream);
bool conv_halo_applicable(const ConvArgs& a);
double conv_halo_efficiency(const ConvArgs& a);
int conv_halo(const ConvArgs& a, cudaStream_t stream);

int gram_tc_partial(const __nv_bfloat16* feat, int B, int HW, int C, int splits, float* partial,
                    cudaStream_t stream);
int gram_pick_splits(int B, int HW, int C);
struct GramMask {
  const float* m;
  int mask_b;
  const uint8_t* kb_flags;
  __nv_bfloat16* fm2;
};
int gram_sym_partial(const __nv_bfloat16* feat, int B, int HW, int C, int splits, float* partial, const GramMask* mask,
                     cudaStream_t stream, float* csum = nullptr);
int gram_mask_flags_bytes(int mask_b, int HW, int C);
int gram_mask_flags(const float* m, int mask_b, int HW, int C, uint8_t* flags, cudaStream_t stream);

}
```

### iris-style-transfer_b200/csrc/nst_engine.cu

```cuda
#include <vector>

#include "../../include/isx.h"
#include "isx_common.cuh"
#include "isx_internal.h"
#include "isx_kernels.h"
#include "lbfgs_state.h"

using namespace isx;
typedef __nv_bfloat16 bf16;

static inline cudaStream_t S(isx_stream s) { return reinterpret_cast<cudaStream_t>(s); }

static const int kCout[16] = {64, 64, 128, 128, 256, 256, 256, 256, 512, 512, 512, 512, 512, 512, 512, 512};
static const int kCin[16] = {3, 64, 64, 128, 128, 256, 256, 256, 256, 512, 512, 512, 512, 512, 512, 512};
static const int kLevel[16] = {0, 0, 1, 1, 2, 2, 2, 2, 3, 3, 3, 3, 4, 4, 4, 4};
static inline bool pool_after(int i) { return i == 1 || i == 3 || i == 7 || i == 11 || i == 15; }
static const int kConvBefore[5] = {1, 3, 7, 11, 15};
static inline int pool_index(int conv) { return conv == 1 ? 0 : conv == 3 ? 1 : conv == 7 ? 2 : conv == 11 ? 3 : 4; }
static inline bool tap_is_pool(int id) { return id >= ISX_TAP_POOL0; }
static inline int tap_conv(int id) { return tap_is_pool(id) ? kConvBefore[id - ISX_TAP_POOL0] : id; }
static inline int tap_level(int id) { return tap_is_pool(id) ? id - ISX_TAP_POOL0 + 1 : kLevel[id]; }
static inline int tap_C(int id) { return kCout[tap_conv(id)]; }

namespace {
// ... 133 lines not shown
  if (!cfg || make_layout(cfg, &L)) return -1;
  return static_cast<int64_t>(L.total);
}

extern "C" int isx_nst_forward(const isx_nst_config* c, const isx_nst_buffers* b, const float* x, int flags,
                               isx_stream stream) {
  ISX_REQUIRE(c && b && x && b->workspace, "isx_nst_forward: null pointer");
  Layout L;
  if (int rc = make_layout(c, &L)) return rc;
  cudaStream_t s = S(stream);
  const bool with_last_pool = (flags & ISX_FWD_LAST_POOL) != 0, lean = (flags & ISX_FWD_LEAN) != 0;
  for (int i = 0; i < c->n_conv; ++i) {
    const bool want_pool = pool_after(i) && (i + 1 < c->n_conv || with_last_pool || pool_tapped(c, pool_index(i)));
    if (int rc = run_conv_fwd(c, b, L, i, x, want_pool && i > 0, s, lean)) return rc;
    if (want_pool && i == 0) {
      const int lv = kLevel[i];
      if (int rc = maxpool_fwd(at(b, L.act[i]), at(b, L.pool[lv]), c->B, L.H[lv], L.W[lv], kCout[i], s)) return rc;
    }
  }
  return 0;
}

extern "C" int isx_nst_feature(const isx_nst_config* c, const isx_nst_buffers* b, int kind, int idx, isx_bf16** ptr,
                               int32_t* h, int32_t* w, int32_t* ch) {
  ISX_REQUIRE(c && b && ptr && h && w && ch, "isx_nst_feature: null pointer");
  Layout L;
  if (int rc = make_layout(c, &L)) return rc;
  if (kind == 0) {
    ISX_REQUIRE(idx >= 0 && idx < c->n_conv, "isx_nst_feature: conv %d not computed (n_conv=%d)", idx, c->n_conv);
    *ptr = reinterpret_cast<isx_bf16*>(at(b, L.act[idx]));
    *h = L.H[kLevel[idx]]; *w = L.W[kLevel[idx]]; *ch = kCout[idx];
  } else {
    const int conv_before[5] = {1, 3, 7, 11, 15};
    ISX_REQUIRE(idx >= 0 && idx < 5 && conv_before[idx] < c->n_conv, "isx_nst_feature: pool %d not computed", idx);
    *ptr = reinterpret_cast<isx_bf16*>(at(b, L.pool[idx]));
    *h = L.H[idx + 1]; *w = L.W[idx + 1]; *ch = kCout[conv_before[idx]];
  }
  return 0;
}

namespace {
struct TapSrc {
  const bf16* add = nullptr;
  const float* aa = nullptr;
  const float* ab = nullptr;
  const bf16* gram_D = nullptr;
  const bf16* gram_A = nullptr;
  bool add_is_masked = false;
  bool any() const { return add || aa || gram_D; }
};

int run_backward(const isx_nst_config* c, const isx_nst_buffers* b, const Layout& L, const TapSrc* src,
                 const bf16* last_pool_grad, float* grad, cudaStream_t s) {
  const int B = c->B;
  auto pool_src = [&](int conv) -> const TapSrc* {
    if (!pool_after(conv)) return nullptr;
    const TapSrc& ps = src[ISX_TAP_POOL0 + pool_index(conv)];
    return ps.any() ? &ps : nullptr;
  };
  int deepest = c->n_conv - 1;
  if (!last_pool_grad)
    while (deepest > 0 && !src[deepest].any() && !pool_src(deepest)) --deepest;
  bf16* ping = at(b, L.gradA);
  bf16* pong = at(b, L.gradB);
  bf16* tapbuf = at(b, L.tapbuf);
  const bf16* gm = nullptr;
  auto gram_1x1 = [&](int id, bf16* out, bool mask) -> int {
    const int lv = tap_level(id);
    ConvArgs a;
    a.in = src[id].gram_A; a.weight = src[id].gram_D; a.out = out;
    a.B = B; a.H = L.H[lv]; a.W = L.W[lv]; a.Cin = tap_C(id); a.Cout = tap_C(id); a.ntaps = 1; a.per_image_weights = true;
    a.mask_act = mask ? at(b, tap_off(L, id)) : nullptr;
    return conv_tc(a, s);
  };
  auto pool_bwd = [&](const bf16* dy, int lv, int conv, bf16* dx) -> int {
    return maxpool_bwd_idx(dy, atb(b, L.pidx[lv]), dx, B, L.H[lv], L.W[lv], kCout[conv], s);
  };
  auto pool_combine = [&](int k, const bf16* g, bf16* out) -> int {
    const int id = ISX_TAP_POOL0 + k, lv = k + 1, C = tap_C(id);
    const long HW = static_cast<long>(L.H[lv]) * L.W[lv];
    const TapSrc& t = src[id];
    const bf16* add2 = t.add;
    if (t.gram_D) {
      if (int rc = gram_1x1(id, tapbuf, false)) return rc;
      if (t.add)
        if (int rc = tap_add_mask(t.add, tapbuf, nullptr, nullptr, at(b, L.pool[k]), tapbuf, B, HW, C, s, 0)) return rc;
      add2 = tapbuf;
    }
    return tap_add_mask(g, add2, t.aa, t.ab, at(b, L.pool[k]), out, B, HW, C, s, 0);
  };
  {
    const int i = deepest, lv = kLevel[i], C = kCout[i];
    const long HW = static_cast<long>(L.H[lv]) * L.W[lv];
    const TapSrc& t = src[i];
    const bf16* up = nullptr;
    const bf16* pg = last_pool_grad;
    if (pool_src(i)) {
      if (int rc = pool_combine(pool_index(i), pg, ping)) return rc;
      pg = ping;
    }
    if (pg) {
      if (int rc = pool_bwd(pg, lv, i, pong)) return rc;
      up = pong;
    }
    ISX_REQUIRE(up || t.any(), "nst backward: conv %d carries no gradient", i);
    if (up && !t.any()) {
      gm = up;
    } else if (!up && t.add && !t.aa && !t.gram_D) {
      if (t.add_is_masked) {
        gm = t.add;
      } else {
        if (int rc = tap_add_mask(t.add, nullptr, nullptr, nullptr, at(b, L.act[i]), ping, B, HW, C, s)) return rc;
        gm = ping;
      }
    } else if (!up && !t.add && !t.aa && t.gram_D) {
      if (int rc = gram_1x1(i, ping, true)) return rc;
      gm = ping;
    } else {
      const bf16* add2 = nullptr;
      if (t.gram_D) {
        if (int rc = gram_1x1(i, tapbuf, false)) return rc;
        add2 = tapbuf;
      }
      const bf16* g1 = up ? up : t.add;
      if (up && t.add && add2) {
        if (int rc = tap_add_mask(t.add, tapbuf, nullptr, nullptr, at(b, L.act[i]), tapbuf, B, HW, C, s)) return rc;
      } else if (up && t.add) {
        add2 = t.add;
      }
      if (int rc = tap_add_mask(g1, add2, t.aa, t.ab, at(b, L.act[i]), ping, B, HW, C, s)) return rc;
      gm = ping;
    }
  }
  for (int i = deepest; i >= 1; --i) {
    const int lv = kLevel[i];
    const int j = i - 1;
    const int lvj = kLevel[j];
    const int Cj = kCout[j];
    const long HWj = static_cast<long>(L.H[lvj]) * L.W[lvj];
    const TapSrc& t = src[j];
    const bool through_pool = pool_after(j);
    ConvArgs a;
    a.in = gm; a.weight = reinterpret_cast<const bf16*>(b->w_dgrad[i]);
    ISX_REQUIRE(b->w_dgrad[i] != nullptr, "nst: packed dgrad weights of conv %d missing", i);
    a.B = B; a.H = L.H[lv]; a.W = L.W[lv]; a.Cin = kCout[i]; a.Cout = kCin[i]; a.ntaps = 9;
    a.out = (gm == ping) ? pong : ping;
    bf16* other = (a.out == ping) ? pong : ping;
    if (!through_pool) {
      a.mask_act = at(b, L.act[j]); a.add_buf = t.add; a.aff_a = t.aa; a.aff_b = t.ab;
      if (t.gram_D) { a.gram_act = t.gram_A; a.gram_D = t.gram_D; }
      if (int rc = conv_tc(a, s)) return rc;
      gm = a.out;
    } else {
      if (int rc = conv_tc(a, s)) return rc;
      if (pool_src(j))
        if (int rc = pool_combine(pool_index(j), a.out, a.out)) return rc;
      if (int rc = pool_bwd(a.out, lvj, j, other)) return rc;
      gm = other;
      if (t.any()) {
        const bf16* add2 = t.add;
        if (t.gram_D) {
          if (int rc = gram_1x1(j, tapbuf, false)) return rc;
          if (t.add) {
            if (int rc = tap_add_mask(t.add, tapbuf, nullptr, nullptr, at(b, L.act[j]), tapbuf, B, HWj, Cj, s)) return rc;
          }
          add2 = tapbuf;
        }
        if (int rc = tap_add_mask(other, add2, t.aa, t.ab, at(b, L.act[j]), a.out, B, HWj, Cj, s)) return rc;
        gm = a.out;
      }
    }
  }
  if (b->w0_dgrad != nullptr) {
    ConvArgs a;
    a.in = gm; a.weight = reinterpret_cast<const bf16*>(b->w0_dgrad);
    a.B = B; a.H = L.H[0]; a.W = L.W[0]; a.Cin = 64; a.Cout = 16; a.ntaps = 9;
    a.dx_nchw = grad; a.xc = c->xc; a.in_mask = c->mask_b ? b->input_mask : nullptr; a.mask_b = c->mask_b;
    return conv_tc(a, s);
  }
  return conv1_1_dgrad(gm, b->w0, c->mask_b ? b->input_mask : nullptr, c->mask_b, grad, c->xc, B, L.H[0], L.W[0], s);
}
}

extern "C" int isx_nst_eval(const isx_nst_config* c, const isx_nst_buffers* b, const float* x, double* loss_c,
                            double* loss_s, float* grad, isx_stream stream) {
  ISX_REQUIRE(c && b && x && loss_c && loss_s && grad && b->workspace, "isx_nst_eval: null pointer");
  ISX_REQUIRE(c->n_style + c->n_content > 0, "isx_nst_eval: no loss taps");
  ISX_REQUIRE(c->style_mask_b == 0 || c->style_mask_b == 1 || c->style_mask_b == c->B, "isx_nst_eval: style mask batch %d", c->style_mask_b);
  Layout L;
  if (int rc = make_layout(c, &L)) return rc;
  cudaStream_t s = S(stream);
  const int B = c->B;
  const int deepest = c->n_conv - 1;
  const bool last_pool_tapped = pool_after(deepest) && pool_tapped(c, pool_index(deepest));
  ISX_REQUIRE(style_tap_of(c, deepest) >= 0 || content_tap_of(c, deepest) >= 0 || last_pool_tapped,
              "isx_nst_eval: conv %d is not tapped", deepest);
  ISX_CHECK_CUDA(cudaMemsetAsync(loss_c, 0, sizeof(double) * B, s));
  ISX_CHECK_CUDA(cudaMemsetAsync(loss_s, 0, sizeof(double) * B, s));

  auto tap_losses = [&](int id) -> int {
    const int lv = tap_level(id);
    const int C = tap_C(id);
    const long HW = static_cast<long>(L.H[lv]) * L.W[lv];
    const bf16* act = at(b, tap_off(L, id));
    const int st = style_tap_of(c, id);
    if (st >= 0) {
      const double w = c->style_w[st];
      if (c->style_mode == 0) {
        ISX_REQUIRE(b->gram_target[st], "nst: Gram target %d missing", st);
        const double inv_n = 1.0 / ((c->pred_unbatched ? 1.0 : static_cast<double>(C)) * HW);
        GramMask gm;
        if (c->style_mask_b > 0) {
          ISX_REQUIRE(b->style_mask[st], "nst: style mask %d missing", st);
          gm.m = b->style_mask[st]; gm.mask_b = c->style_mask_b;
          gm.kb_flags = reinterpret_cast<const uint8_t*>(at(b, L.kbflags[st]));
          gm.fm2 = at(b, L.fm2[st]);
        }
        const int splits = gram_pick_splits(B, static_cast<int>(HW), C);
        int rc = gram_sym_partial(act, B, static_cast<int>(HW), C, splits, atf(b, L.gram_ws), c->style_mask_b > 0 ? &gm : nullptr, s);
        if (rc) return rc;
        rc = gram_finalize(atf(b, L.gram_ws), B, splits, C, static_cast<float>(inv_n), nullptr, b->gram_target[st],
                           c->style_target_b, 0.25 * w, loss_s, static_cast<float>(c->s_weight * w * inv_n), at(b, L.D[st]), s);
        if (rc) return rc;
      } else {
        ISX_REQUIRE(b->bn_target_mean[st] && b->bn_target_std[st], "nst: BN target %d missing", st);
        ISX_REQUIRE(HW >= 2, "nst: unbiased std needs >= 2 pixels at tap %d", id);
        double* sums = reinterpret_cast<double*>(static_cast<char*>(b->workspace) + L.sums);
        ISX_CHECK_CUDA(cudaMemsetAsync(sums, 0, sizeof(double) * B * C * 2, s));
        const float* m = nullptr;
        if (c->style_mask_b > 0) {
          ISX_REQUIRE(b->style_mask[st], "nst: style mask %d missing", st);
          m = b->style_mask[st];
        }
        int rc = chan_sums(act, B, HW, C, sums, s, m, c->style_mask_b);
        if (rc) return rc;
        rc = bn_finalize(sums, B, C, HW, nullptr, nullptr, b->bn_target_mean[st], b->bn_target_std[st],
                         c->style_target_b, w / C, c->s_weight * w / C, loss_s, atf(b, L.aff_a[st]), atf(b, L.aff_b[st]), s);
        if (rc) return rc;
        if (m)
          if (int rc2 = masked_affine_grad(act, m, c->style_mask_b, atf(b, L.aff_a[st]), atf(b, L.aff_b[st]), at(b, L.fm2[st]), B, HW, C, s)) return rc2;
      }
    }
    const int ct = content_tap_of(c, id);
    if (ct >= 0) {
      ISX_REQUIRE(b->content_target[ct], "nst: content target %d missing", ct);
      const long per_image = HW * C;
      const double denom = static_cast<double>(per_image) * (c->coupled ? B : 1);
      int rc = content_mse(act, reinterpret_cast<const bf16*>(b->content_target[ct]), c->content_target_b,
                           at(b, L.cgrad[ct]), B, per_image, 0.5 * c->content_w[ct] / denom,
                           static_cast<float>(c->c_weight * c->content_w[ct] / denom), loss_c, s);
      if (rc) return rc;
    }
    return 0;
  };

  for (int i = 0; i < c->n_conv; ++i) {
    const bool want_pool = pool_after(i) && (i + 1 < c->n_conv || pool_tapped(c, pool_index(i)));
    if (int rc = run_conv_fwd(c, b, L, i, x, want_pool, s, true)) return rc;
    if (int rc = tap_losses(i)) return rc;
    if (want_pool && pool_tapped(c, pool_index(i)))
      if (int rc = tap_losses(ISX_TAP_POOL0 + pool_index(i))) return rc;
  }

  TapSrc src[ISX_VGG19_TAPS];
  for (int id = 0; id < ISX_VGG19_TAPS; ++id) {
    if (tap_conv(id) >= c->n_conv) continue;
    const int st = style_tap_of(c, id), ct = content_tap_of(c, id);
    if (ct >= 0) { src[id].add = at(b, L.cgrad[ct]); src[id].add_is_masked = true; }
    if (st >= 0 && c->style_mode == 0) {
      src[id].gram_D = at(b, L.D[st]);
      src[id].gram_A = c->style_mask_b > 0 ? at(b, L.fm2[st]) : at(b, tap_off(L, id));
    } else if (st >= 0 && c->style_mask_b > 0) {
      if (src[id].add) {
        const long HWt = static_cast<long>(L.H[tap_level(id)]) * L.W[tap_level(id)];
        if (int rc = tap_add_mask(src[id].add, at(b, L.fm2[st]), nullptr, nullptr, at(b, tap_off(L, id)), at(b, L.fm2[st]), B, HWt,
                                  tap_C(id), s, 0)) return rc;
      }
      src[id].add = at(b, L.fm2[st]);
      src[id].add_is_masked = false;
    } else if (st >= 0) {
      src[id].aa = atf(b, L.aff_a[st]);
      src[id].ab = atf(b, L.aff_b[st]);
    }
  }
  return run_backward(c, b, L, src, nullptr, grad, s);
}

extern "C" int isx_nst_prepare_style_masks(const isx_nst_config* c, const isx_nst_buffers* b, isx_stream stream) {
  ISX_REQUIRE(c && b && b->workspace, "isx_nst_prepare_style_masks: null pointer");
  ISX_REQUIRE(c->style_mask_b == 1 || c->style_mask_b == c->B, "isx_nst_prepare_style_masks: style mask batch %d", c->style_mask_b);
  Layout L;
  if (int rc = make_layout(c, &L)) return rc;
  cudaStream_t s = S(stream);
  if (c->style_mode != 0) return 0;
  for (int t = 0; t < c->n_style; ++t) {
    const int i = c->style_conv[t];
    const int C = tap_C(i);
    const int HW = L.H[tap_level(i)] * L.W[tap_level(i)];
    ISX_REQUIRE(b->style_mask[t], "isx_nst_prepare_style_masks: style mask %d missing", t);
    ISX_CHECK_CUDA(cudaMemsetAsync(at(b, L.fm2[t]), 0, static_cast<size_t>(c->B) * HW * C * 2, s));
    if (int rc = gram_mask_flags(b->style_mask[t], c->style_mask_b, HW, C, reinterpret_cast<uint8_t*>(at(b, L.kbflags[t])), s))
      return rc;
  }
  return 0;
}

extern "C" int isx_nst_style_features(const isx_nst_config* c, const isx_nst_buffers* b, int want_stats, int want_gram,
                                      float* out, int64_t ld, isx_stream stream) {
  ISX_REQUIRE(c && b && out && b->workspace, "isx_nst_style_features: null pointer");
  ISX_REQUIRE(want_stats || want_gram, "isx_nst_style_features: nothing to extract");
  Layout L;
  if (int rc = make_layout(c, &L)) return rc;
  cudaStream_t s = S(stream);
  const int B = c->B;
  int64_t need = 0;
  for (int t = 0; t < c->n_style; ++t) {
    const int64_t C = tap_C(c->style_conv[t]);
    need += (want_stats ? 2 * C : 0) + (want_gram ? C * (C + 1) / 2 : 0);
  }
  ISX_REQUIRE(ld >= need, "isx_nst_style_features: row stride %lld < feature dimension %lld", (long long)ld, (long long)need);
  int64_t stat_off[ISX_MAX_TAPS], gram_off[ISX_MAX_TAPS], off = 0;
  for (int t = 0; t < c->n_style; ++t) { stat_off[t] = off; if (want_stats) off += 2 * tap_C(c->style_conv[t]); }
// ... 101 lines not shown
```

Measured before the change: 2084.

## Fuse max-unpool backward into halo conv dgrad epilogue

Adds an UNPOOL template variant of the halo conv kernel that scatters the dgrad output directly into the 2x-upsampled pre-pool gradient using the stored pool indices. The NST backward pass uses it at pool boundaries when the halo path applies, which removes a separate maxpool backward kernel and the write and reread of the pooled-resolution dgrad. Costs include extra index loads, uncoalesced 4-way scattered stores from the epilogue, and more template instantiations. A scratch profiling script is also added.

```diff
diff --git a/include/isx.h b/include/isx.h
--- a/include/isx.h
+++ b/include/isx.h
@@ -58,6 +58,9 @@
 
 int isx_conv3x3_dgrad_gram(const isx_bf16* dy, const isx_bf16* w_dgrad, isx_bf16* dx, int B, int H, int W, int Cin,
                            int Cout, const isx_bf16* act_below, const isx_bf16* gram_D, isx_stream stream);
+
+int isx_conv3x3_dgrad_unpool(const isx_bf16* dy, const isx_bf16* w_dgrad, const uint8_t* idx, isx_bf16* dx, int B, int H,
+                             int W, int Cin, int Cout, isx_stream stream);
 
 int isx_maxpool2x2_fwd(const isx_bf16* in, isx_bf16* out, int B, int H, int W, int C, isx_stream stream);
 int isx_maxpool2x2_bwd(const isx_bf16* dy_pooled, const isx_bf16* act_prepool, isx_bf16* dx, int B, int H, int W,
diff --git a/iris-style-transfer_b200/csrc/api_ops.cu b/iris-style-transfer_b200/csrc/api_ops.cu
--- a/iris-style-transfer_b200/csrc/api_ops.cu
+++ b/iris-style-transfer_b200/csrc/api_ops.cu
@@ -111,6 +111,18 @@
   a.B = B; a.H = H; a.W = W; a.Cin = Cout; a.Cout = Cin; a.ntaps = 9;
   a.mask_act = P(relu_act); a.add_buf = P(add_grad); a.aff_a = aff_a; a.aff_b = aff_b;
   decode_tile_cfg(tile_cfg, &a);
+  return conv_tc(a, S(stream));
+}
+
+extern "C" int isx_conv3x3_dgrad_unpool(const isx_bf16* dy, const isx_bf16* w_dgrad, const uint8_t* idx, isx_bf16* dx, int B,
+                                        int H, int W, int Cin, int Cout, isx_stream stream) {
+  ISX_REQUIRE(dy && w_dgrad && idx && dx, "isx_conv3x3_dgrad_unpool: null pointer");
+  ConvArgs a;
+  a.in = P(dy); a.weight = P(w_dgrad); a.out = P(dx);
+  a.B = B; a.H = H; a.W = W; a.Cin = Cout; a.Cout = Cin; a.ntaps = 9;
+  a.unpool_idx = idx;
+  ISX_REQUIRE(B > 0 && H > 0 && W > 0 && conv_halo_unpool_applicable(a, 2 * H, 2 * W),
+              "isx_conv3x3_dgrad_unpool: B=%d %dx%d Cin=%d Cout=%d is not a halo-patch call", B, H, W, Cin, Cout);
   return conv_tc(a, S(stream));
 }
 
@@ -273,6 +285,7 @@
       {"halo2", &IsxContext::opt_halo2},
       {"tail_n", &IsxContext::opt_tail_n},
       {"sweep64", &IsxContext::opt_sweep64},
+      {"unpool", &IsxContext::opt_unpool},
       {"smem_reserve_kb", &IsxContext::opt_smem_reserve_kb},
   };
   for (const auto& o : kOptions)
diff --git a/iris-style-transfer_b200/csrc/conv_c64.cu b/iris-style-transfer_b200/csrc/conv_c64.cu
--- a/iris-style-transfer_b200/csrc/conv_c64.cu
+++ b/iris-style-transfer_b200/csrc/conv_c64.cu
@@ -425,6 +425,7 @@
 
 bool conv_c64_applicable(const ConvArgs& a) {
   if (a.Cin != 64 || a.ntaps != 9 || a.per_image_weights || a.stride != 1) return false;
+  if (a.unpool_idx != nullptr) return false;
   if (a.dx_nchw != nullptr) return a.Cout == 16;
   if (a.Cout != 64) return false;
   if (a.gram_act != nullptr && a.gram_act != a.mask_act) return false;
diff --git a/iris-style-transfer_b200/csrc/conv_halo.cu b/iris-style-transfer_b200/csrc/conv_halo.cu
--- a/iris-style-transfer_b200/csrc/conv_halo.cu
+++ b/iris-style-transfer_b200/csrc/conv_halo.cu
@@ -23,6 +23,8 @@
   const float* aff_b;
   uint8_t* pool_idx;
   int skip_out;
+  const uint8_t* unpool_idx;
+  __nv_bfloat16* unpool_out;
 };
 
 struct HaloLayout {
@@ -56,7 +58,7 @@
   __device__ int y0() const { return ((r / n_tiles) / pairs_x) * (VERT ? 32 : 16); }
 };
 
-template <int BN, bool VERT>
+template <int BN, bool VERT, bool UNPOOL>
 __global__ void __launch_bounds__(kHaloThreads, 1)
 conv_halo_kernel(const __grid_constant__ CUtensorMap tmA, const __grid_constant__ CUtensorMap tmW,
                  const __grid_constant__ CUtensorMap tmO, const __grid_constant__ CUtensorMap tmM,
@@ -238,10 +240,25 @@
                   w.x0() + (VERT ? 0 : 8 * mt), w.y0() + (VERT ? 16 * mt : 0), w.b);
     };
     uint32_t g = 0;
-    if (p.use_mask && leader && n_my > 0) {
+    if (!UNPOOL && p.use_mask && leader && n_my > 0) {
       issue_mask_load(it, 0, 0);
       issue_mask_load(it, 1, 1);
     }
+    const int ut = static_cast<int>(threadIdx.x) - 64;
+    uint2 ucode[4];
+    auto load_codes = [&](const ItemWalk<VERT>& w, int s) {
+      const int mt = s / kNH, nh = s - mt * kNH;
+      const int xs = w.x0() + (VERT ? 0 : 8 * mt), ys = w.y0() + (VERT ? 16 * mt : 0);
+#pragma unroll
+      for (int u = 0; u < 4; ++u) {
+        const int r = u * 32 + (ut >> 3), x = xs + (r & 7), y = ys + (r >> 3);
+        ucode[u] = make_uint2(0u, 0u);
+        if (x < p.W && y < p.H)
+          ucode[u] = __ldg(reinterpret_cast<const uint2*>(p.unpool_idx + ((static_cast<size_t>(w.b) * p.H + y) * p.W + x) * p.Cout +
+                                                            w.nt() * BN + nh * 64 + (ut & 7) * 8));
+      }
+    };
+    if (UNPOOL && n_my > 0) load_codes(it, 0);
     uint32_t acc = 0, aph = 0;
     for (int i = 0; i < n_my; ++i) {
       const int b = it.b, x0 = it.x0(), y0 = it.y0(), n0 = it.nt() * BN;
@@ -270,14 +287,14 @@
         float f[32];
 #pragma unroll
         for (int j = 0; j < 32; ++j) f[j] = __uint_as_float(v[j]);
-        if (p.bias != nullptr) {
+        if (!UNPOOL && p.bias != nullptr) {
 #pragma unroll
           for (int j = 0; j < 32; j += 4) {
             const float4 bv = __ldg(reinterpret_cast<const float4*>(p.bias + nc + j));
             f[j] += bv.x; f[j + 1] += bv.y; f[j + 2] += bv.z; f[j + 3] += bv.w;
           }
         }
-        if (p.add_buf != nullptr && valid) {
+        if (!UNPOOL && p.add_buf != nullptr && valid) {
 #pragma unroll
           for (int j = 0; j < 32; j += 8) {
             const uint4 u = __ldg(reinterpret_cast<const uint4*>(p.add_buf + pix + nc + j));
@@ -288,7 +305,7 @@
             t = unpack_bf16x2(u.w); f[j + 6] += t.x; f[j + 7] += t.y;
           }
         }
-        if (p.use_mask) {
+        if (!UNPOOL && p.use_mask) {
           mbar_wait(&act_full[slot], (g >> 1) & 1);
           const uint8_t* mrow = smem + L.act + slot * kSub + row * 128;
 #pragma unroll
@@ -311,7 +328,7 @@
             for (int e = 0; e < 8; ++e) f[j + e] = a[e] > 0.f ? f[j + e] : 0.f;
           }
         }
-        if (p.relu) {
+        if (!UNPOOL && p.relu) {
 #pragma unroll
           for (int j = 0; j < 32; ++j) f[j] = fmaxf(f[j], 0.f);
         }
@@ -335,12 +352,31 @@
             tma_store_4d(&tmO, stg, n0 + nh * 64, xs, ys, b);
             tma_store_commit();
           }
-          if (p.use_mask) {
+          if (!UNPOOL && p.use_mask) {
             if (s + 2 < kNSub) issue_mask_load(it, s + 2, g + 2);
             else if (i + 1 < n_my) issue_mask_load(nxt, s + 2 - kNSub, g + 2);
           }
         }
-        if (p.fuse_pool) {
+        if (UNPOOL) {
+#pragma unroll
+          for (int u = 0; u < 4; ++u) {
+            const int r = u * 32 + (ut >> 3), chunk = ut & 7, x = xs + (r & 7), y = ys + (r >> 3);
+            if (x < p.W && y < p.H) {
+              uint4 o[4];
+              unpool4_codes(*reinterpret_cast<const uint4*>(stg + r * 128 + ((chunk ^ (r & 7)) * 16)), ucode[u], o);
+              __nv_bfloat16* dst = p.unpool_out + ((static_cast<size_t>(b) * (2 * p.H) + 2 * y) * (2 * p.W) + 2 * x) * p.Cout +
+                                   n0 + nh * 64 + chunk * 8;
+              const size_t row2 = static_cast<size_t>(2 * p.W) * p.Cout;
+              *reinterpret_cast<uint4*>(dst) = o[0];
+              *reinterpret_cast<uint4*>(dst + p.Cout) = o[1];
+              *reinterpret_cast<uint4*>(dst + row2) = o[2];
+              *reinterpret_cast<uint4*>(dst + row2 + p.Cout) = o[3];
+            }
+          }
+          if (s + 1 < kNSub) load_codes(it, s + 1);
+          else if (i + 1 < n_my) load_codes(nxt, 0);
+        }
+        if (!UNPOOL && p.fuse_pool) {
           uint8_t* pst = smem + L.pstg + slot * 4096;
           const int item = threadIdx.x - 64;
           const int pr = item >> 3, chunk = item & 7;
@@ -383,7 +419,7 @@
 }
 
 
-template <int BN, bool VERT>
+template <int BN, bool VERT, bool UNPOOL>
 static int launch_halo(const ConvArgs& a, cudaStream_t stream) {
   HaloParams p;
   memset(&p, 0, sizeof(p));
@@ -400,7 +436,8 @@
   p.use_mask = a.mask_act != nullptr ? 1 : 0;
   p.fuse_pool = (a.pool_out != nullptr && a.H >= 2 && a.W >= 2) ? 1 : 0;
   p.pool_idx = p.fuse_pool ? a.pool_idx : nullptr;
-  p.skip_out = (p.fuse_pool && a.pool_idx != nullptr && a.skip_out) ? 1 : 0;
+  p.skip_out = ((p.fuse_pool && a.pool_idx != nullptr && a.skip_out) || UNPOOL) ? 1 : 0;
+  p.unpool_idx = a.unpool_idx; p.unpool_out = a.out;
   int ws = 6;
   HaloLayout L = halo_layout<BN>(ws, p.use_mask, p.fuse_pool);
   const int cap = (227 - std::max(0, std::min(isx_ctx()->opt_smem_reserve_kb, 22))) * 1024;
@@ -444,7 +481,7 @@
     uint32_t bp[4] = {64, 4, 8, 1};
     if (isx_make_tmap_bf16(&tmP, a.pool_out, 4, dp, sp, bp, true)) return 3;
   }
-  auto kern = conv_halo_kernel<BN, VERT>;
+  auto kern = conv_halo_kernel<BN, VERT, UNPOOL>;
   ISX_CHECK_CUDA(cudaFuncSetAttribute(kern, cudaFuncAttributeMaxDynamicSharedMemorySize, (int)smem_bytes));
   const int grid = std::min<int>(p.total_items, kNumSMs);
   isx_prof_begin(ISX_PROF_CONV, 2.0 * (9.0 * a.Cin + (p.extra_kb ? a.Cout : 0)) * a.Cout * static_cast<double>(a.B) * a.H * a.W, stream);
@@ -477,8 +514,15 @@
 int conv_halo(const ConvArgs& a, cudaStream_t stream) {
   ISX_REQUIRE(conv_halo_applicable(a), "conv_halo: not applicable");
   const bool vert = conv_halo_pick(a) == 2;
-  if (a.Cout % 128 == 0) return vert ? launch_halo<128, true>(a, stream) : launch_halo<128, false>(a, stream);
-  return vert ? launch_halo<64, true>(a, stream) : launch_halo<64, false>(a, stream);
-}
-
-}
+  if (a.unpool_idx != nullptr) {
+    ISX_REQUIRE(a.bias == nullptr && !a.relu && a.pool_out == nullptr && a.mask_act == nullptr && a.add_buf == nullptr &&
+                    a.aff_a == nullptr && a.gram_act == nullptr,
+                "conv_halo: the unpool epilogue applies no bias, ReLU, pool, mask, map, affine or Gram term");
+    if (a.Cout % 128 == 0) return vert ? launch_halo<128, true, true>(a, stream) : launch_halo<128, false, true>(a, stream);
+    return vert ? launch_halo<64, true, true>(a, stream) : launch_halo<64, false, true>(a, stream);
+  }
+  if (a.Cout % 128 == 0) return vert ? launch_halo<128, true, false>(a, stream) : launch_halo<128, false, false>(a, stream);
+  return vert ? launch_halo<64, true, false>(a, stream) : launch_halo<64, false, false>(a, stream);
+}
+
+}
diff --git a/iris-style-transfer_b200/csrc/conv_sweep.cu b/iris-style-transfer_b200/csrc/conv_sweep.cu
--- a/iris-style-transfer_b200/csrc/conv_sweep.cu
+++ b/iris-style-transfer_b200/csrc/conv_sweep.cu
@@ -569,6 +569,7 @@
   if (a.out == nullptr) return false;
   if (a.gram_act != nullptr && a.gram_act != a.mask_act) return false;
   if (a.aff_a != nullptr && a.mask_act == nullptr) return false;
+  if (a.unpool_idx != nullptr) return false;
   return true;
 }
 double conv_sweep_efficiency(const ConvArgs& a) { return std::max(strip_efficiency(a.H), strip_efficiency(a.W)); }
diff --git a/iris-style-transfer_b200/csrc/conv_tc.cu b/iris-style-transfer_b200/csrc/conv_tc.cu
--- a/iris-style-transfer_b200/csrc/conv_tc.cu
+++ b/iris-style-transfer_b200/csrc/conv_tc.cu
@@ -351,6 +351,7 @@
 
 template <int BN, int MT, int EPI = 0>
 static int launch_conv(const ConvArgs& a, int stages_override, cudaStream_t stream) {
+  ISX_REQUIRE(a.unpool_idx == nullptr, "conv_tc: the generic kernel has no unpool epilogue");
   ConvParams p;
   memset(&p, 0, sizeof(p));
   const int Ho = (a.H + a.stride - 1) / a.stride, Wo = (a.W + a.stride - 1) / a.stride;
@@ -449,27 +450,55 @@
   return 0;
 }
 
+namespace {
+enum class ConvPath { kTailN, kSweep, kC64, kHalo, kGeneric };
+
+ConvPath conv_path(const ConvArgs& a) {
+  if (a.dx_nchw != nullptr && isx_ctx()->opt_tail_n > 0 && isx_ctx()->opt_c64 < 2 && a.force_bn == 0 &&
+      a.Cin == 64 && a.Cout == 16 && a.ntaps == 9)
+    return ConvPath::kTailN;
+  if (isx_ctx()->opt_sweep64 > 0 && a.force_bn == 0 && !a.generic_only && conv_sweep_applicable(a)) {
+    const long strips = static_cast<long>(a.B) * ((std::max(a.H, a.W) + 127) / 128) * std::min(a.H, a.W);
+    if (isx_ctx()->opt_sweep64 >= 2 ||
+        (conv_sweep_efficiency(a) >= 0.85 && strips >= 64L * kNumSMs && std::min(a.H, a.W) >= 16))
+      return ConvPath::kSweep;
+  }
+  if (isx_ctx()->opt_c64 > 0 && a.force_bn == 0 && !a.generic_only && conv_c64_applicable(a) &&
+      (isx_ctx()->opt_c64 >= 2 || (a.dx_nchw == nullptr && static_cast<long>(a.B) * ((a.H + 15) / 16) * ((a.W + 7) / 8) >= kNumSMs)))
+    return ConvPath::kC64;
+  if (isx_ctx()->opt_halo2 > 0 && a.force_bn == 0 && !a.generic_only && conv_halo_applicable(a)) {
+    const long items = static_cast<long>(a.B) * ((a.H + 15) / 16) * ((a.W + 15) / 16) * (a.Cout / (a.Cout % 128 == 0 ? 128 : 64));
+    if (isx_ctx()->opt_halo2 >= 2 || (items >= 2 * kNumSMs && conv_halo_efficiency(a) >= 0.85)) return ConvPath::kHalo;
+  }
+  return ConvPath::kGeneric;
+}
+}
+
+bool conv_halo_unpool_applicable(const ConvArgs& a_in, int H_pre, int W_pre) {
+  ConvArgs a = a_in;
+  a.unpool_idx = nullptr;
+  if (H_pre != 2 * a.H || W_pre != 2 * a.W || a.ntaps != 9 || a.bias != nullptr || a.relu || a.pool_out != nullptr ||
+      a.mask_act != nullptr || a.add_buf != nullptr || a.aff_a != nullptr || a.gram_act != nullptr)
+    return false;
+  return conv_path(a) == ConvPath::kHalo;
+}
+
 int conv_tc(const ConvArgs& a_in, cudaStream_t stream) {
   ConvArgs a = a_in;
   ISX_REQUIRE(a.stride == 1 || (a.stride == 2 && a.pool_out == nullptr && a.mask_act == nullptr && a.gram_act == nullptr &&
                                 a.dx_nchw == nullptr && !a.per_image_weights),
               "conv_tc: stride %d (stride 2 is the plain forward conv: no pool, mask, image gradient or per-image weights)",
               a.stride);
-  if (a.dx_nchw != nullptr && isx_ctx()->opt_tail_n > 0 && isx_ctx()->opt_c64 < 2 && a.force_bn == 0 &&
-      a.Cin == 64 && a.Cout == 16 && a.ntaps == 9)
-    return conv1_1_tail_n(a.in, a.weight, a.in_mask, a.mask_b, a.dx_nchw, a.xc, a.B, a.H, a.W, stream);
-  if (isx_ctx()->opt_sweep64 > 0 && a.force_bn == 0 && !a.generic_only && conv_sweep_applicable(a)) {
-    const long strips = static_cast<long>(a.B) * ((std::max(a.H, a.W) + 127) / 128) * std::min(a.H, a.W);
-    if (isx_ctx()->opt_sweep64 >= 2 ||
-        (conv_sweep_efficiency(a) >= 0.85 && strips >= 64L * kNumSMs && std::min(a.H, a.W) >= 16))
-      return conv_sweep(a, stream);
-  }
-  if (isx_ctx()->opt_c64 > 0 && a.force_bn == 0 && !a.generic_only && conv_c64_applicable(a) &&
-      (isx_ctx()->opt_c64 >= 2 || (a.dx_nchw == nullptr && static_cast<long>(a.B) * ((a.H + 15) / 16) * ((a.W + 7) / 8) >= kNumSMs)))
-    return conv_c64(a, stream);
-  if (isx_ctx()->opt_halo2 > 0 && a.force_bn == 0 && !a.generic_only && conv_halo_applicable(a)) {
-    const long items = static_cast<long>(a.B) * ((a.H + 15) / 16) * ((a.W + 15) / 16) * (a.Cout / (a.Cout % 128 == 0 ? 128 : 64));
-    if (isx_ctx()->opt_halo2 >= 2 || (items >= 2 * kNumSMs && conv_halo_efficiency(a) >= 0.85)) return conv_halo(a, stream);
+  if (a.unpool_idx != nullptr) {
+    ISX_REQUIRE(conv_halo_unpool_applicable(a, 2 * a.H, 2 * a.W), "conv_tc: unpool_idx needs a call that conv_halo takes");
+    return conv_halo(a, stream);
+  }
+  switch (conv_path(a)) {
+    case ConvPath::kTailN: return conv1_1_tail_n(a.in, a.weight, a.in_mask, a.mask_b, a.dx_nchw, a.xc, a.B, a.H, a.W, stream);
+    case ConvPath::kSweep: return conv_sweep(a, stream);
+    case ConvPath::kC64: return conv_c64(a, stream);
+    case ConvPath::kHalo: return conv_halo(a, stream);
+    case ConvPath::kGeneric: break;
   }
   if (a.dx_nchw != nullptr) {
     ISX_REQUIRE(a.Cin == 64 && a.Cout == 16 && a.ntaps == 9, "conv_tc: image-gradient mode needs Cin 64, Cout 16 (padded)");
diff --git a/iris-style-transfer_b200/csrc/elementwise.cu b/iris-style-transfer_b200/csrc/elementwise.cu
--- a/iris-style-transfer_b200/csrc/elementwise.cu
+++ b/iris-style-transfer_b200/csrc/elementwise.cu
@@ -309,22 +309,12 @@
     const long po = ((static_cast<long>(b) * Ho + yo) * Wo + xo) * C + c8 * 8;
     const uint4 g = __ldg(reinterpret_cast<const uint4*>(dy + po));
     const uint2 cd = __ldg(reinterpret_cast<const uint2*>(idx + po));
-    const uint32_t gw[4] = {g.x, g.y, g.z, g.w};
-    const uint32_t c16[4] = {__byte_perm(cd.x, 0u, 0x4140), __byte_perm(cd.x, 0u, 0x4342), __byte_perm(cd.y, 0u, 0x4140),
-                             __byte_perm(cd.y, 0u, 0x4342)};
+    uint4 o[4];
+    unpool4_codes(g, cd, o);
     const long base = ((static_cast<long>(b) * H + 2 * yo) * W + 2 * xo) * C + c8 * 8;
     const long offs[4] = {0, C, static_cast<long>(W) * C, static_cast<long>(W) * C + C};
 #pragma unroll
-    for (int k = 0; k < 4; ++k) {
-      uint32_t o[4];
-#pragma unroll
-      for (int e = 0; e < 4; ++e) {
-        const uint32_t d = c16[e] ^ (static_cast<uint32_t>(k) * 0x00010001u);
-        const uint32_t keep = ((d & 0x0000FFFFu) ? 0u : 0x0000FFFFu) | ((d & 0xFFFF0000u) ? 0u : 0xFFFF0000u);
-        o[e] = gw[e] & keep;
-      }
-      *reinterpret_cast<uint4*>(dx + base + offs[k]) = make_uint4(o[0], o[1], o[2], o[3]);
-    }
+    for (int k = 0; k < 4; ++k) *reinterpret_cast<uint4*>(dx + base + offs[k]) = o[k];
   }
 }
 
diff --git a/iris-style-transfer_b200/csrc/isx_common.cuh b/iris-style-transfer_b200/csrc/isx_common.cuh
--- a/iris-style-transfer_b200/csrc/isx_common.cuh
+++ b/iris-style-transfer_b200/csrc/isx_common.cuh
@@ -34,6 +34,7 @@
   int opt_tail_n = 1;
   int opt_smem_reserve_kb = 0;
   int opt_sweep64 = 1;
+  int opt_unpool = 1;
   unsigned long long launches = 0;
   IsxProfiler* prof = nullptr;
 };
@@ -267,6 +268,22 @@
   codes.x = __byte_perm(cw[0], cw[1], 0x6420);
   codes.y = __byte_perm(cw[2], cw[3], 0x6420);
 }
+__device__ __forceinline__ void unpool4_codes(const uint4& g, const uint2& cd, uint4 (&o)[4]) {
+  const uint32_t gw[4] = {g.x, g.y, g.z, g.w};
+  const uint32_t c16[4] = {__byte_perm(cd.x, 0u, 0x4140), __byte_perm(cd.x, 0u, 0x4342), __byte_perm(cd.y, 0u, 0x4140),
+                           __byte_perm(cd.y, 0u, 0x4342)};
+#pragma unroll
+  for (int k = 0; k < 4; ++k) {
+    uint32_t w[4];
+#pragma unroll
+    for (int e = 0; e < 4; ++e) {
+      const uint32_t d = c16[e] ^ (static_cast<uint32_t>(k) * 0x00010001u);
+      const uint32_t keep = ((d & 0x0000FFFFu) ? 0u : 0x0000FFFFu) | ((d & 0xFFFF0000u) ? 0u : 0xFFFF0000u);
+      w[e] = gw[e] & keep;
+    }
+    o[k] = make_uint4(w[0], w[1], w[2], w[3]);
+  }
+}
 
 __device__ __forceinline__ float warp_sum(float v) {
 #pragma unroll
diff --git a/iris-style-transfer_b200/csrc/isx_internal.h b/iris-style-transfer_b200/csrc/isx_internal.h
--- a/iris-style-transfer_b200/csrc/isx_internal.h
+++ b/iris-style-transfer_b200/csrc/isx_internal.h
@@ -17,6 +17,7 @@
   __nv_bfloat16* pool_out = nullptr;
   uint8_t* pool_idx = nullptr;
   bool skip_out = false;
+  const uint8_t* unpool_idx = nullptr;
   const __nv_bfloat16* mask_act = nullptr;
   const __nv_bfloat16* add_buf = nullptr;
   const float* aff_a = nullptr;
@@ -41,6 +42,7 @@
 bool conv_halo_applicable(const ConvArgs& a);
 double conv_halo_efficiency(const ConvArgs& a);
 int conv_halo(const ConvArgs& a, cudaStream_t stream);
+bool conv_halo_unpool_applicable(const ConvArgs& a, int H_pre, int W_pre);
 
 int gram_tc_partial(const __nv_bfloat16* feat, int B, int HW, int C, int splits, float* partial,
                     cudaStream_t stream);
diff --git a/iris-style-transfer_b200/csrc/nst_engine.cu b/iris-style-transfer_b200/csrc/nst_engine.cu
--- a/iris-style-transfer_b200/csrc/nst_engine.cu
+++ b/iris-style-transfer_b200/csrc/nst_engine.cu
@@ -309,11 +309,20 @@
       if (int rc = conv_tc(a, s)) return rc;
       gm = a.out;
     } else {
-      if (int rc = conv_tc(a, s)) return rc;
-      if (pool_src(j))
-        if (int rc = pool_combine(pool_index(j), a.out, a.out)) return rc;
-      if (int rc = pool_bwd(a.out, lvj, j, other)) return rc;
-      gm = other;
+      bf16* unpooled = other;
+      bf16* spare = a.out;
+      if (!pool_src(j) && isx_ctx()->opt_unpool > 0 && conv_halo_unpool_applicable(a, L.H[lvj], L.W[lvj])) {
+        a.unpool_idx = atb(b, L.pidx[lvj]);
+        if (int rc = conv_tc(a, s)) return rc;
+        unpooled = a.out;
+        spare = other;
+      } else {
+        if (int rc = conv_tc(a, s)) return rc;
+        if (pool_src(j))
+          if (int rc = pool_combine(pool_index(j), a.out, a.out)) return rc;
+        if (int rc = pool_bwd(a.out, lvj, j, other)) return rc;
+      }
+      gm = unpooled;
       if (t.any()) {
         const bf16* add2 = t.add;
         if (t.gram_D) {
@@ -323,8 +332,8 @@
           }
           add2 = tapbuf;
         }
-        if (int rc = tap_add_mask(other, add2, t.aa, t.ab, at(b, L.act[j]), a.out, B, HWj, Cj, s)) return rc;
-        gm = a.out;
+        if (int rc = tap_add_mask(unpooled, add2, t.aa, t.ab, at(b, L.act[j]), spare, B, HWj, Cj, s)) return rc;
+        gm = spare;
       }
     }
   }
diff --git a/scratch/unpool_kernels.py b/scratch/unpool_kernels.py
--- /dev/null
+++ b/scratch/unpool_kernels.py
@@ -0,0 +1,77 @@
+import collections
+import json
+import os
+import sys
+import tempfile
+
+import torch
+from torch.profiler import ProfilerActivity, profile
+
+ROOT = os.path.dirname(os.path.dirname(os.path.abspath(__file__)))
+sys.path.insert(0, ROOT)
+import iris_b200
+from iris_b200 import _lib, engine as E
+from oracle import nst_oracle as O
+
+B, H, W, EVALS = 64, 400, 640, 10
+lib = _lib.load()
+dev = torch.device("cuda:0")
+net = iris_b200.VGG19(content_layers=["relu4_2"], style_layers=["relu1_1", "relu2_1", "relu3_1", "relu4_1"],
+                      weights=O.random_vgg19_weights(0))
+g = torch.Generator().manual_seed(5)
+x, c, s = (torch.rand(B, 3, H, W, generator=g).to(dev) for _ in range(3))
+eng = E.NstEngine(net.packed(dev), B, H, W, 3, net.content_convs, net.style_convs, style_mode=0, c_weight=1.0, s_weight=1e6)
+eng.forward(c)
+eng.set_content_targets([eng.tap(i) for i in net.content_convs])
+eng.forward(s)
+eng.set_gram_targets([E.gram_of(eng.tap(i)) for i in net.style_convs])
+grad = torch.empty(B, 3, H, W, device=dev)
+
+kern = {0: collections.defaultdict(list), 1: collections.defaultdict(list)}
+eval_ms = {0: [], 1: []}
+for rnd in range(3):
+    for on in (0, 1):
+        assert lib.isx_set_option(b"unpool", on) == 0
+        for _ in range(3):
+            eng.eval(x, grad)
+        torch.cuda.synchronize()
+        with profile(activities=[ProfilerActivity.CUDA]) as prof:
+            for _ in range(EVALS):
+                eng.eval(x, grad)
+            torch.cuda.synchronize()
+        per = collections.defaultdict(float)
+        for e in prof.key_averages():
+            if e.device_type.name == "CUDA" and e.device_time_total > 0:
+                per[(e.key, e.count // EVALS)] += e.device_time_total / EVALS
+        for k, v in per.items():
+            kern[on][k].append(v)
+        ev0, ev1 = torch.cuda.Event(enable_timing=True), torch.cuda.Event(enable_timing=True)
+        ev0.record()
+        for _ in range(20):
+            eng.eval(x, grad)
+        ev1.record()
+        torch.cuda.synchronize()
+        eval_ms[on].append(ev0.elapsed_time(ev1) / 20)
+
+def short(name):
+    return name.split("(")[0].replace("void ", "")[:70]
+
+out = {"gpu": torch.cuda.get_device_name(0), "B": B, "H": H, "W": W, "eval_ms": eval_ms, "kernels": {}}
+print("closure evaluation ms (CUDA events, 20 evals x 3 rounds): unpool=0 %s  unpool=1 %s" % (
+    ["%.3f" % v for v in eval_ms[0]], ["%.3f" % v for v in eval_ms[1]]))
+print("%-72s %6s %12s %12s" % ("kernel (launches per eval)", "n", "unpool=0 us", "unpool=1 us"))
+keys = sorted(set(kern[0]) | set(kern[1]), key=lambda k: -max(min(kern[0].get(k, [0])), min(kern[1].get(k, [0]))))
+tot = {0: 0.0, 1: 0.0}
+for k in keys:
+    a, b = kern[0].get(k), kern[1].get(k)
+    ma, mb = (min(a) if a else 0.0), (min(b) if b else 0.0)
+    tot[0] += ma
+    tot[1] += mb
+    out["kernels"]["%s x%d" % (short(k[0]), k[1])] = [ma, mb]
+    if max(ma, mb) >= 20 or "halo" in k[0] or "maxpool" in k[0]:
+        print("%-72s %6d %12.1f %12.1f" % (short(k[0]), k[1], ma, mb))
+print("%-72s %6s %12.1f %12.1f" % ("sum of kernel time per evaluation (min over rounds)", "", tot[0], tot[1]))
+out_dir = sys.argv[1] if len(sys.argv) > 1 else tempfile.mkdtemp()
+os.makedirs(out_dir, exist_ok=True)
+json.dump(out, open(os.path.join(out_dir, "unpool_kernels.json"), "w"), indent=1)
+print("wrote", os.path.join(out_dir, "unpool_kernels.json"))
```

Result: faster. 2115, median of 6 (+1.5%).
